# astaka-pe/SeMIGCN

Measured on NVIDIA B200. Metric: sgcn_gcnconv_train_edge_layers_per_s, higher is better.
Workload: dtype f32

## Files before the change

include/semigcn_b200.h:

```cpp
#ifndef SEMIGCN_B200_H
#define SEMIGCN_B200_H

#include <stddef.h>
#include <stdint.h>

#if defined(__GNUC__)
#define SGB_API __attribute__((visibility("default")))
#else
#define SGB_API
#endif

#ifdef __cplusplus
extern "C" {
#endif

#define SGB_VERSION 100

#define SGB_OK 0
#define SGB_EINVAL (-1)
#define SGB_ECUDA (-2)
#define SGB_ENOSPC (-3)
#define SGB_ENOTSUP (-4)

#define SGB_MODE_GCN 0
#define SGB_MODE_CHEB 1
#define SGB_MODE_ADJ 2

typedef struct sgb_edge {
    int32_t col;
    float w;
} sgb_edge_t;

SGB_API int sgb_version(void);
SGB_API const char* sgb_last_error(void);
SGB_API int sgb_num_sms(void);

SGB_API int sgb_fingerprint(const int64_t* values, int64_t count, uint64_t* out , void* stream);
SGB_API size_t sgb_graph_build_workspace_bytes(int64_t nnz, int64_t n);
SGB_API int sgb_graph_build(const int64_t* edge_index, int64_t nnz, int64_t n, int mode, int transpose,
                    int32_t* rowptr , int32_t* colidx , sgb_edge_t* edges ,
                    float* dis , int32_t* perm , int32_t* err_flag ,
                    void* workspace, size_t workspace_bytes, void* stream);

SGB_API int sgb_spmm_stat_rows(int64_t n, int c);
SGB_API int sgb_spmm(const int32_t* rowptr, const sgb_edge_t* edges, const float* dis, int mode,
             const float* x, int64_t ldx, int64_t n, int c,
             const float* in_mean, const float* in_scale, const float* in_shift, float slope,
             float alpha, const float* addend, int64_t ld_addend, float beta,
             const float* bias, float* y, int64_t ldy, float* stat_partials, float* amax_out, void* stream);

SGB_API int sgb_spmm_halo(const int32_t* rowptr, const sgb_edge_t* edges, const float* dis, int mode,
                  const float* x, int64_t ldx, int64_t n, int c, const float* x_ghost, int64_t ld_ghost, int64_t n_split,
                  const float* in_mean, const float* in_scale, const float* in_shift, float slope,
                  float alpha, const float* addend, int64_t ld_addend, float beta,
                  const float* bias, float* y, int64_t ldy, float* stat_partials, float* amax_out, void* stream);
SGB_API int sgb_spmm_range(const int32_t* rowptr, const sgb_edge_t* edges, const float* dis, int mode,
                   const float* x, int64_t ldx, int64_t row_begin, int64_t n, int c, const float* x_ghost, int64_t ld_ghost, int64_t n_split,
                   const float* in_mean, const float* in_scale, const float* in_shift, float slope,
                   float alpha, const float* addend, int64_t ld_addend, float beta,
                   const float* bias, float* y, int64_t ldy, float* stat_partials, float* amax_out, void* stream);
SGB_API int sgb_gather_rows(const float* x, int64_t ldx, const int32_t* idx, int64_t count, int c, float* out, int64_t ldo, void* stream);

SGB_API int sgb_gemm_stat_rows(int64_t m);
SGB_API size_t sgb_gemm_workspace_bytes(int64_t m, int n, int k, int engine);
SGB_API int sgb_gemm(int transb, const float* a, int64_t lda, const float* b, int64_t ldb,
             float* c, int64_t ldc, int64_t m, int n, int k,
             const float* a_mean, const float* a_scale, const float* a_shift, float slope,
             const float* bias, int accumulate, float* stat_partials, const float* a_amax,
             void* workspace, size_t workspace_bytes, int engine, void* stream);
SGB_API size_t sgb_gemm_tn_workspace_bytes(int64_t m, int n, int k);
SGB_API int sgb_gemm_tn(const float* g, int64_t ldg, const float* a, int64_t lda, float* d, int64_t ldd,
                int64_t m, int n, int k, int accumulate, const float* g_amax, const float* a_amax,
                void* workspace, size_t workspace_bytes, int engine, void* stream);
SGB_API size_t sgb_colsum_workspace_bytes(int64_t m, int n);
SGB_API int sgb_colsum(const float* g, int64_t ldg, int64_t m, int n, float* out, int accumulate,
               float* amax_out ,
               void* workspace, size_t workspace_bytes, void* stream);
SGB_API int sgb_amax(const float* x, int64_t ldx, int64_t m, int c, float* amax_out, void* stream);

SGB_API int sgb_col_stat_rows(int64_t m, int c);
SGB_API int sgb_col_stats(const float* y, int64_t ldy, int64_t m, int c, float* partials, void* stream);
SGB_API int sgb_bn_finalize(const float* partials, int rows, int c, int64_t count,
                    const float* gamma, const float* beta, float eps, float momentum,
                    float* running_mean, float* running_var,
                    float* mean, float* invstd, float* scale, float* shift, void* stream);
SGB_API int sgb_moments_merge(const float* partials, int rows, int c, float* merged , void* stream);
SGB_API int sgb_bn_act_apply(const float* y, int64_t ldy, int64_t m, int c, const float* mean, const float* scale,
                     const float* shift, float slope, float* z, int64_t ldz, float* amax_out , void* stream);
SGB_API int sgb_bn_act_bwd_reduce(const float* dz, int64_t lddz, const float* y, int64_t ldy, int64_t m, int c,
                          const float* scale, const float* shift, const float* mean, const float* invstd,
                          float slope, float* partials, void* stream);
SGB_API int sgb_bn_bwd_finalize(const float* partials, int rows, int c, float* sums, float* dgamma,
                        float* dbeta, int accumulate, void* stream);
SGB_API int sgb_bn_act_bwd_apply(const float* dz, int64_t lddz, const float* y, int64_t ldy, int64_t m, int c,
                         const float* scale, const float* shift, const float* mean, const float* invstd,
                         const float* sums, float slope, int training, float* dy, int64_t lddy,
                         float* amax_out , void* stream);

SGB_API int sgb_loss_partial_rows(void);
SGB_API size_t sgb_incidence_build_workspace_bytes(int64_t nf, int64_t n);
SGB_API int sgb_incidence_build(const int64_t* faces, int64_t nf, int64_t n, int32_t* rowptr , int32_t* inc ,
                        int32_t* err_flag, void* workspace, size_t workspace_bytes, void* stream);
SGB_API int sgb_step_loss_fwd(const float* pos, int64_t ldp, int64_t n, const void* target_pos, int target_f64, const uint8_t* vmask,
                      const int64_t* faces, int64_t nf, const void* target_fn, const uint8_t* fmask, float* fn_out,
                      double* partials, double* out , void* stream);
SGB_API int sgb_step_loss_bwd(const float* pos, int64_t ldp, int64_t n, const void* target_pos, int target_f64, const uint8_t* vmask,
                      const int64_t* faces, int64_t nf, const void* target_fn, const uint8_t* fmask,
                      const int32_t* inc_rowptr, const int32_t* inc, const double* out, const double* grads ,
                      float* dpos, int64_t lddpos, void* stream);
SGB_API int sgb_lap_loss_fwd(const float* pos, int64_t ldp, int64_t n, const int32_t* rowptr, const sgb_edge_t* edges, float* diff ,
                     double* partials, double* out , void* stream);
SGB_API int sgb_lap_loss_bwd(const float* diff, int64_t n, const int32_t* rowptr, const int32_t* rowptr_t, const sgb_edge_t* edges_t,
                     const double* out, const double* grad , float* dpos, int64_t lddpos, void* stream);

SGB_API size_t sgb_bnf_work_floats(int64_t nf);
SGB_API int sgb_bnf_partial_rows(void);
SGB_API int sgb_bnf_loss_fwd(const float* pos, int64_t ldp, int64_t n, const int64_t* faces, const int32_t* f2f, int64_t nf,
                     const float* fn, int loop, int ltype, float* work, double* partials, float* new_fn, double* out ,
                     void* stream);
SGB_API int sgb_bnf_loss_bwd(const float* fn, const float* new_fn, int64_t nf, int ltype, const double* out, const double* grad ,
                     float* dfn, void* stream);

SGB_API int sgb_input_prep(const float* z1, int64_t ldz, int64_t n, const float* dm, float* x, float* scratch , void* stream);

#ifdef __cplusplus
}
#endif
#endif
```

semigcn_b200/_lib.py:

```python
from __future__ import annotations

import ctypes as C
import os
import subprocess
from typing import Optional

import torch

_HERE = os.path.dirname(os.path.abspath(__file__))
CSRC = os.path.join(_HERE, "csrc")
LIB_PATH = os.environ.get("SGB_LIB_PATH") or os.path.join(CSRC, "libsemigcn_b200.so")

MODE_GCN, MODE_CHEB, MODE_ADJ = 0, 1, 2
ENGINE_AUTO, ENGINE_SIMT, ENGINE_TC = 0, 1, 2

_i64, _i32, _f32, _vp, _sz = C.c_int64, C.c_int, C.c_float, C.c_void_p, C.c_size_t
_f64 = C.c_double

SIGNATURES = {
    "sgb_version": (_i32, []),
    "sgb_last_error": (C.c_char_p, []),
    "sgb_num_sms": (_i32, []),
    "sgb_fingerprint": (_i32, [_vp, _i64, _vp, _vp]),
    "sgb_graph_build_workspace_bytes": (_sz, [_i64, _i64]),
    "sgb_graph_build": (_i32, [_vp, _i64, _i64, _i32, _i32, _vp, _vp, _vp, _vp, _vp, _vp, _vp, _sz, _vp]),
    "sgb_spmm_stat_rows": (_i32, [_i64, _i32]),
    "sgb_spmm": (_i32, [_vp, _vp, _vp, _i32, _vp, _i64, _i64, _i32, _vp, _vp, _vp, _f32, _f32, _vp, _i64, _f32,
                        _vp, _vp, _i64, _vp, _vp, _vp]),
    "sgb_spmm_halo": (_i32, [_vp, _vp, _vp, _i32, _vp, _i64, _i64, _i32, _vp, _i64, _i64, _vp, _vp, _vp, _f32, _f32, _vp, _i64, _f32,
                             _vp, _vp, _i64, _vp, _vp, _vp]),
    "sgb_spmm_range": (_i32, [_vp, _vp, _vp, _i32, _vp, _i64, _i64, _i64, _i32, _vp, _i64, _i64, _vp, _vp, _vp, _f32, _f32, _vp, _i64, _f32,
                              _vp, _vp, _i64, _vp, _vp, _vp]),
    "sgb_gather_rows": (_i32, [_vp, _i64, _vp, _i64, _i32, _vp, _i64, _vp]),
    "sgb_gemm_stat_rows": (_i32, [_i64]),
    "sgb_gemm_workspace_bytes": (_sz, [_i64, _i32, _i32, _i32]),
    "sgb_gemm": (_i32, [_i32, _vp, _i64, _vp, _i64, _vp, _i64, _i64, _i32, _i32, _vp, _vp, _vp, _f32, _vp, _i32,
                        _vp, _vp, _vp, _sz, _i32, _vp]),
    "sgb_gemm_tn_workspace_bytes": (_sz, [_i64, _i32, _i32]),
    "sgb_gemm_tn": (_i32, [_vp, _i64, _vp, _i64, _vp, _i64, _i64, _i32, _i32, _i32, _vp, _vp, _vp, _sz, _i32, _vp]),
    "sgb_colsum_workspace_bytes": (_sz, [_i64, _i32]),
    "sgb_colsum": (_i32, [_vp, _i64, _i64, _i32, _vp, _i32, _vp, _vp, _sz, _vp]),
    "sgb_amax": (_i32, [_vp, _i64, _i64, _i32, _vp, _vp]),
    "sgb_moments_merge": (_i32, [_vp, _i32, _i32, _vp, _vp]),
    "sgb_col_stat_rows": (_i32, [_i64, _i32]),
    "sgb_col_stats": (_i32, [_vp, _i64, _i64, _i32, _vp, _vp]),
    "sgb_bn_finalize": (_i32, [_vp, _i32, _i32, _i64, _vp, _vp, _f32, _f32, _vp, _vp, _vp, _vp, _vp, _vp, _vp]),
    "sgb_bn_act_apply": (_i32, [_vp, _i64, _i64, _i32, _vp, _vp, _vp, _f32, _vp, _i64, _vp, _vp]),
    "sgb_bn_act_bwd_reduce": (_i32, [_vp, _i64, _vp, _i64, _i64, _i32, _vp, _vp, _vp, _vp, _f32, _vp, _vp]),
    "sgb_bn_bwd_finalize": (_i32, [_vp, _i32, _i32, _vp, _vp, _vp, _i32, _vp]),
    "sgb_bn_act_bwd_apply": (_i32, [_vp, _i64, _vp, _i64, _i64, _i32, _vp, _vp, _vp, _vp, _vp, _f32, _i32,
                                    _vp, _i64, _vp, _vp]),
    "sgb_loss_partial_rows": (_i32, []),
    "sgb_incidence_build_workspace_bytes": (_sz, [_i64, _i64]),
    "sgb_incidence_build": (_i32, [_vp, _i64, _i64, _vp, _vp, _vp, _vp, _sz, _vp]),
    "sgb_step_loss_fwd": (_i32, [_vp, _i64, _i64, _vp, _i32, _vp, _vp, _i64, _vp, _vp, _vp, _vp, _vp, _vp]),
    "sgb_step_loss_bwd": (_i32, [_vp, _i64, _i64, _vp, _i32, _vp, _vp, _i64, _vp, _vp, _vp, _vp, _vp, _vp, _vp, _i64, _vp]),
    "sgb_lap_loss_fwd": (_i32, [_vp, _i64, _i64, _vp, _vp, _vp, _vp, _vp, _vp]),
    "sgb_input_prep": (_i32, [_vp, _i64, _i64, _vp, _vp, _vp, _vp]),
    "sgb_bnf_work_floats": (_sz, [_i64]),
    "sgb_bnf_partial_rows": (_i32, []),
    "sgb_bnf_loss_fwd": (_i32, [_vp, _i64, _i64, _vp, _vp, _i64, _vp, _i32, _i32, _vp, _vp, _vp, _vp, _vp]),
    "sgb_bnf_loss_bwd": (_i32, [_vp, _vp, _i64, _i32, _vp, _vp, _vp, _vp]),
    "sgb_lap_loss_bwd": (_i32, [_vp, _i64, _vp, _vp, _vp, _vp, _vp, _vp, _i64, _vp]),
}

_lib: Optional[C.CDLL] = None


class SgbError(RuntimeError):
    pass


def build_library(verbose: bool = False) -> str:
    out = subprocess.run(["make", "-C", CSRC, "-j", str(os.cpu_count() or 4)], capture_output=True, text=True)
    if verbose or out.returncode != 0:
        print(out.stdout[-4000:])
        print(out.stderr[-4000:])
    if out.returncode != 0:
        raise SgbError("building libsemigcn_b200.so failed")
    return LIB_PATH


def load() -> C.CDLL:
    global _lib
    if _lib is not None:
        return _lib
    if not os.path.exists(LIB_PATH):
        raise SgbError(
            f"{LIB_PATH} not found: the CUDA extension is required (no CPU fallback). "
            "Build it with `python -c 'import __graft_entry__ as g; g.build()'` or `make -C semigcn_b200/csrc`.")
    lib = C.CDLL(LIB_PATH)
    for name, (res, args) in SIGNATURES.items():
        fn = getattr(lib, name)
        fn.restype = res
        fn.argtypes = args
    _lib = lib
    return lib


# ... 27 lines not shown
```

semigcn_b200/csrc/bn.cu:

```cuda
#include "common.cuh"

namespace sgb {

constexpr int kColThreads = 256;

enum ColOp { COL_STATS = 0, COL_BN_BWD = 1, COL_SUM = 2 };

struct ColArgs {
    const float* y; int64_t ldy;
    const float* dz; int64_t lddz;
    int64_t m; int c;
    const float* scale; const float* shift; const float* mean; const float* invstd;
    float slope;
    float* partials;
    float* amax;
};

template <int OP, int VEC>
__global__ void __launch_bounds__(kColThreads) k_col_reduce(const ColArgs a, int tpr ) {
    __shared__ float red[2][kColThreads * VEC];
    __shared__ float redn[kColThreads];
    float amx = 0.f;
    const int cl = threadIdx.x % tpr;
    const int rl = threadIdx.x / tpr;
// ... 87 lines not shown
            }
        }
        __syncthreads();
    }
    if (OP == COL_SUM && a.amax) publish_amax(amx, reinterpret_cast<uint32_t*>(redn), a.amax);
}

static int col_tpr(int c, int vec) {
    int lanes = (c + vec - 1) / vec;
    int p = 1;
    while (p < lanes && p < kColThreads) p <<= 1;
    return p;
}

static int col_rows_cfg(int64_t m, int c, int vec) {
    int tpr = col_tpr(c, vec);
    int rpp = kColThreads / tpr;
    int64_t need = ceil_div(m > 0 ? m : 1, (int64_t)rpp * 4);
    int64_t cap = (int64_t)num_sms() * 4;
    int64_t g = need < cap ? need : cap;
    return (int)(g < 1 ? 1 : g);
}

static int col_rows(int64_t m, int c) {
    int g4 = col_rows_cfg(m, c, 4), g1 = col_rows_cfg(m, c, 1);
    return g4 > g1 ? g4 : g1;
}

template <int OP>
static int col_launch(const ColArgs& a, bool vec_ok, cudaStream_t stream) {
    int vec = (a.c % 4 == 0 && vec_ok) ? 4 : 1;
    int grid = col_rows_cfg(a.m, a.c, vec);
    int rows = col_rows(a.m, a.c);
    const int planes = OP == COL_STATS ? 3 : 2;
    if (rows > grid)
        if (cudaMemsetAsync(a.partials + (size_t)grid * planes * a.c, 0, (size_t)(rows - grid) * planes * a.c * sizeof(float), stream) != cudaSuccess) {
            set_error("col_reduce: memset failed");
            return SGB_ECUDA;
        }
    int tpr = col_tpr(a.c, vec);
    if (vec == 4) k_col_reduce<OP, 4><<<grid, kColThreads, 0, stream>>>(a, tpr);
    else k_col_reduce<OP, 1><<<grid, kColThreads, 0, stream>>>(a, tpr);
    SGB_CHECK_LAUNCH("k_col_reduce");
    return SGB_OK;
}

static bool al16(const void* p) { return (reinterpret_cast<uintptr_t>(p) & 15) == 0; }

struct FinArgs {
    const float* partials; int rows; int c; int64_t count;
    const float* gamma; const float* beta; float eps; float momentum;
    float* running_mean; float* running_var;
    float* mean; float* invstd; float* scale; float* shift;
    float* sums; float* dgamma; float* dbeta; int accumulate;
    int kind;
};

__global__ void __launch_bounds__(1024) k_finalize(const FinArgs f) {
    __shared__ double r1[32][33], r2[32][33], r3[32][33];
    const int ch = blockIdx.x * 32 + threadIdx.x;
    double s1 = 0.0, s2 = 0.0, s3 = 0.0;
    if (ch < f.c) {
        if (f.kind == 0 || f.kind == 3) {
            double p = 0.0;
            bool have = false;
            for (int r = threadIdx.y; r < f.rows; r += 32) {
                const double nb = (double)__ldg(f.partials + ((int64_t)r * 3 + 0) * f.c + ch);
                if (nb == 0.0) continue;
                const double mb = (double)__ldg(f.partials + ((int64_t)r * 3 + 1) * f.c + ch);
                const double qb = (double)__ldg(f.partials + ((int64_t)r * 3 + 2) * f.c + ch);
                if (!have) { p = mb; have = true; }
                const double d = mb - p;
                s1 += nb;
                s2 = fma(nb, d, s2);
                s3 += fma(nb * d, d, qb);
            }
            if (have) {
                const double dm = s2 / s1;
                s3 -= s2 * dm;
                if (s3 < 0.0) s3 = 0.0;
                s2 = p + dm;
            }
        } else {
            for (int r = threadIdx.y; r < f.rows; r += 32) {
                s1 += (double)__ldg(f.partials + ((int64_t)r * 2 + 0) * f.c + ch);
                s2 += (double)__ldg(f.partials + ((int64_t)r * 2 + 1) * f.c + ch);
            }
        }
    }
    r1[threadIdx.y][threadIdx.x] = s1;
    r2[threadIdx.y][threadIdx.x] = s2;
    r3[threadIdx.y][threadIdx.x] = s3;
    __syncthreads();
    if (threadIdx.y == 0 && ch < f.c) {
        if (f.kind == 0 || f.kind == 3) {
            double n = 0.0, mean = 0.0, m2 = 0.0;
            for (int r = 0; r < 32; ++r) {
                const double nb = r1[r][threadIdx.x];
                if (nb == 0.0) continue;
                const double nt = n + nb, d = r2[r][threadIdx.x] - mean;
                m2 += r3[r][threadIdx.x] + d * d * n * nb / nt;
                mean += d * nb / nt;
                n = nt;
            }
            if (f.kind == 3) {
                f.sums[ch] = (float)n;
                f.sums[f.c + ch] = (float)mean;
                f.sums[2 * f.c + ch] = (float)m2;
                return;
            }
            double var = n > 0.0 ? m2 / n : 0.0;
            if (var < 0.0) var = 0.0;
            const double invstd = 1.0 / sqrt(var + (double)f.eps);
            const double g = f.gamma ? (double)f.gamma[ch] : 1.0;
            const double b = f.beta ? (double)f.beta[ch] : 0.0;
            f.mean[ch] = (float)mean;
            f.invstd[ch] = (float)invstd;
            f.scale[ch] = (float)(g * invstd);
            f.shift[ch] = (float)b;
            if (f.running_mean) {
                const double unb = n > 1.0 ? m2 / (n - 1.0) : var;
                f.running_mean[ch] = (float)((1.0 - f.momentum) * (double)f.running_mean[ch] + f.momentum * mean);
                f.running_var[ch] = (float)((1.0 - f.momentum) * (double)f.running_var[ch] + f.momentum * unb);
            }
        } else {
            double t1 = 0.0, t2 = 0.0;
            for (int r = 0; r < 32; ++r) { t1 += r1[r][threadIdx.x]; t2 += r2[r][threadIdx.x]; }
            if (f.kind == 1) {
                f.sums[ch] = (float)t1;
                f.sums[f.c + ch] = (float)t2;
                if (f.dbeta) f.dbeta[ch] = f.accumulate ? f.dbeta[ch] + (float)t1 : (float)t1;
                if (f.dgamma) f.dgamma[ch] = f.accumulate ? f.dgamma[ch] + (float)t2 : (float)t2;
            } else {
                f.sums[ch] = f.accumulate ? f.sums[ch] + (float)t1 : (float)t1;
            }
        }
    }
}

constexpr int kEwThreads = 256;

static int ew_tpr(int c, int vec) {
    int lanes = (c + vec - 1) / vec;
    int p = 1;
    while (p < lanes && p < kEwThreads) p <<= 1;
    return p;
}

template <int VEC>
__global__ void __launch_bounds__(kEwThreads) k_bn_act_apply(const float* __restrict__ y, int64_t ldy, int64_t m, int c, const float* __restrict__ mean,
                                                             const float* __restrict__ scale, const float* __restrict__ shift, float slope,
                                                             float* __restrict__ z, int64_t ldz, float* __restrict__ amax, int tpr) {
    __shared__ uint32_t s_amax[32];
    float amx = 0.f;
    const int cl = threadIdx.x % tpr, rl = threadIdx.x / tpr, rpp = kEwThreads / tpr;
    for (int c0 = 0; c0 < c; c0 += tpr * VEC) {
        const int ch = c0 + cl * VEC;
        if (ch >= c) continue;
        float mu[VEC], sc[VEC], sh[VEC];
#pragma unroll
        for (int q = 0; q < VEC; ++q) { mu[q] = __ldg(mean + ch + q); sc[q] = __ldg(scale + ch + q); sh[q] = __ldg(shift + ch + q); }
        for (int64_t r = (int64_t)blockIdx.x * rpp + rl; r < m; r += (int64_t)gridDim.x * rpp) {
            if (VEC == 4) {
                const float4 v = ldg4(y + r * ldy + ch);
                float4 o;
                o.x = bn_lrelu(v.x, mu[0], sc[0], sh[0], slope); o.y = bn_lrelu(v.y, mu[1], sc[1], sh[1], slope);
                o.z = bn_lrelu(v.z, mu[2], sc[2], sh[2], slope); o.w = bn_lrelu(v.w, mu[3], sc[3], sh[3], slope);
                st4(z + r * ldz + ch, o);
                amx = fmaxf(amx, fmaxf(fmaxf(fabsf(o.x), fabsf(o.y)), fmaxf(fabsf(o.z), fabsf(o.w))));
            } else {
                const float o = bn_lrelu(__ldg(y + r * ldy + ch), mu[0], sc[0], sh[0], slope);
                z[r * ldz + ch] = o;
                amx = fmaxf(amx, fabsf(o));
            }
        }
    }
    if (amax) publish_amax(amx, s_amax, amax);
}

struct BwdArgs {
    const float* dz; int64_t lddz; const float* y; int64_t ldy; int64_t m; int c;
    const float* scale; const float* shift; const float* mean; const float* invstd; const float* sums;
    float slope; int training; float* dy; int64_t lddy; float* amax;
};

template <int VEC>
__global__ void __launch_bounds__(kEwThreads) k_bn_act_bwd_apply(const BwdArgs a, int tpr) {
    __shared__ uint32_t s_amax[32];
    float amx = 0.f;
// ... 19 lines not shown
                float4 t = ldg4(a.y + r * a.ldy + ch), u = ldg4(a.dz + r * a.lddz + ch);
                yv[0] = t.x; yv[1] = t.y; yv[2] = t.z; yv[3] = t.w;
                dv[0] = u.x; dv[1] = u.y; dv[2] = u.z; dv[3] = u.w;
            } else {
                yv[0] = __ldg(a.y + r * a.ldy + ch);
                dv[0] = __ldg(a.dz + r * a.lddz + ch);
            }
#pragma unroll
            for (int q = 0; q < VEC; ++q) {
                const float ctr = yv[q] - mu[q];
                const float pre = fmaf(ctr, sc[q], sh[q]);
                const float da = pre > 0.f ? dv[q] : dv[q] * a.slope;
                if (a.training) {
                    const float xh = ctr * is[q];
                    out[q] = sc[q] * (da - sb[q] - xh * sg[q]);
                } else {
                    out[q] = sc[q] * da;
                }
                amx = fmaxf(amx, fabsf(out[q]));
            }
            if (VEC == 4) st4(a.dy + r * a.lddy + ch, make_float4(out[0], out[1], out[2], out[3]));
            else a.dy[r * a.lddy + ch] = out[0];
        }
    }
    if (a.amax) publish_amax(amx, s_amax, a.amax);
}

static int ew_grid(int64_t m, int tpr) {
    const int rpp = kEwThreads / tpr;
    int64_t g = ceil_div(m > 0 ? m : 1, (int64_t)rpp * 4);
    int64_t cap = (int64_t)num_sms() * 8;
    g = g < cap ? g : cap;
    return (int)(g < 1 ? 1 : g);
}

}

using namespace sgb;

extern "C" int sgb_col_stat_rows(int64_t m, int c) {
    if (m < 0 || c <= 0) return 0;
    return col_rows(m, c);
}

extern "C" int sgb_col_stats(const float* y, int64_t ldy, int64_t m, int c, float* partials, void* stream) {
    SGB_CHECK_ARG(y && partials && m >= 0 && c > 0 && ldy >= c, "sgb_col_stats: bad argument");
    ColArgs a{};
    a.y = y; a.ldy = ldy; a.m = m; a.c = c; a.partials = partials;
    return col_launch<COL_STATS>(a, al16(y) && ldy % 4 == 0, (cudaStream_t)stream);
}

extern "C" int sgb_bn_finalize(const float* partials, int rows, int c, int64_t count, const float* gamma, const float* beta,
                               float eps, float momentum, float* running_mean, float* running_var, float* mean, float* invstd,
                               float* scale, float* shift, void* stream) {
    SGB_CHECK_ARG(partials && rows > 0 && c > 0 && count > 0 && mean && invstd && scale && shift, "sgb_bn_finalize: bad argument");
    SGB_CHECK_ARG((running_mean == nullptr) == (running_var == nullptr), "sgb_bn_finalize: running stats must come together");
    FinArgs f{};
    f.partials = partials; f.rows = rows; f.c = c; f.count = count; f.gamma = gamma; f.beta = beta; f.eps = eps;
    f.momentum = momentum; f.running_mean = running_mean; f.running_var = running_var;
    f.mean = mean; f.invstd = invstd; f.scale = scale; f.shift = shift; f.kind = 0;
    k_finalize<<<(c + 31) / 32, dim3(32, 32), 0, (cudaStream_t)stream>>>(f);
    SGB_CHECK_LAUNCH("k_finalize");
    return SGB_OK;
}

extern "C" int sgb_moments_merge(const float* partials, int rows, int c, float* merged, void* stream) {
    SGB_CHECK_ARG(partials && rows > 0 && c > 0 && merged, "sgb_moments_merge: bad argument");
    FinArgs f{};
    f.partials = partials; f.rows = rows; f.c = c; f.sums = merged; f.kind = 3;
    k_finalize<<<(c + 31) / 32, dim3(32, 32), 0, (cudaStream_t)stream>>>(f);
    SGB_CHECK_LAUNCH("k_finalize");
    return SGB_OK;
}

extern "C" int sgb_bn_act_apply(const float* y, int64_t ldy, int64_t m, int c, const float* mean, const float* scale,
                                const float* shift, float slope, float* z, int64_t ldz, float* amax_out, void* stream) {
    SGB_CHECK_ARG(y && z && mean && scale && shift && m >= 0 && c > 0 && ldy >= c && ldz >= c, "sgb_bn_act_apply: bad argument");
    if (m == 0) return SGB_OK;
    bool vec = c % 4 == 0 && al16(y) && al16(z) && al16(mean) && al16(scale) && al16(shift) && ldy % 4 == 0 && ldz % 4 == 0;
    const int tpr = ew_tpr(c, vec ? 4 : 1);
    if (vec) k_bn_act_apply<4><<<ew_grid(m, tpr), kEwThreads, 0, (cudaStream_t)stream>>>(y, ldy, m, c, mean, scale, shift, slope, z, ldz, amax_out, tpr);
    else k_bn_act_apply<1><<<ew_grid(m, tpr), kEwThreads, 0, (cudaStream_t)stream>>>(y, ldy, m, c, mean, scale, shift, slope, z, ldz, amax_out, tpr);
    SGB_CHECK_LAUNCH("k_bn_act_apply");
    return SGB_OK;
}

extern "C" int sgb_bn_act_bwd_reduce(const float* dz, int64_t lddz, const float* y, int64_t ldy, int64_t m, int c, const float* scale,
                                     const float* shift, const float* mean, const float* invstd, float slope, float* partials,
                                     void* stream) {
    SGB_CHECK_ARG(dz && y && scale && shift && mean && invstd && partials && m >= 0 && c > 0 && ldy >= c && lddz >= c,
                  "sgb_bn_act_bwd_reduce: bad argument");
    ColArgs a{};
    a.y = y; a.ldy = ldy; a.dz = dz; a.lddz = lddz; a.m = m; a.c = c;
    a.scale = scale; a.shift = shift; a.mean = mean; a.invstd = invstd; a.slope = slope; a.partials = partials;
    return col_launch<COL_BN_BWD>(a, al16(y) && al16(dz) && ldy % 4 == 0 && lddz % 4 == 0, (cudaStream_t)stream);
}

extern "C" int sgb_bn_bwd_finalize(const float* partials, int rows, int c, float* sums, float* dgamma, float* dbeta, int accumulate,
                                   void* stream) {
    SGB_CHECK_ARG(partials && rows > 0 && c > 0 && sums, "sgb_bn_bwd_finalize: bad argument");
    FinArgs f{};
    f.partials = partials; f.rows = rows; f.c = c; f.sums = sums; f.dgamma = dgamma; f.dbeta = dbeta; f.accumulate = accumulate;
    f.kind = 1;
    k_finalize<<<(c + 31) / 32, dim3(32, 32), 0, (cudaStream_t)stream>>>(f);
    SGB_CHECK_LAUNCH("k_finalize");
    return SGB_OK;
}

extern "C" int sgb_bn_act_bwd_apply(const float* dz, int64_t lddz, const float* y, int64_t ldy, int64_t m, int c, const float* scale,
                                    const float* shift, const float* mean, const float* invstd, const float* sums, float slope,
                                    int training, float* dy, int64_t lddy, float* amax_out, void* stream) {
    SGB_CHECK_ARG(dz && y && dy && scale && shift && m >= 0 && c > 0 && ldy >= c && lddz >= c && lddy >= c,
                  "sgb_bn_act_bwd_apply: bad argument");
// ... 36 lines not shown
```

semigcn_b200/csrc/common.cuh:

```cuda
#pragma once
#include <cuda_runtime.h>
#include <stdint.h>
#include <stdio.h>
#include <stdarg.h>
#include <atomic>
#include "../../include/semigcn_b200.h"

namespace sgb {

void set_error(const char* fmt, ...);
int num_sms();
int smem_optin(const void* func, int bytes, std::atomic<uint64_t>* done_mask);

#define SGB_CHECK_ARG(cond, ...)                 \
    do {                                         \
        if (!(cond)) {                           \
            sgb::set_error(__VA_ARGS__);         \
            return SGB_EINVAL;                   \
        }                                        \
    } while (0)

#define SGB_CHECK_LAUNCH(name)                                                        \
    do {                                                                              \
        cudaError_t e__ = cudaGetLastError();                                         \
        if (e__ != cudaSuccess) {                                                     \
            sgb::set_error("%s: launch failed: %s", name, cudaGetErrorString(e__));   \
            return SGB_ECUDA;                                                         \
        }                                                                             \
    } while (0)

#define SGB_CUDA(call)                                                                \
    do {                                                                              \
        cudaError_t e__ = (call);                                                     \
        if (e__ != cudaSuccess) {                                                     \
            sgb::set_error("%s failed: %s", #call, cudaGetErrorString(e__));          \
            return SGB_ECUDA;                                                         \
        }                                                                             \
    } while (0)

static inline int64_t ceil_div(int64_t a, int64_t b) { return (a + b - 1) / b; }
__host__ __device__ static inline int64_t min64(int64_t a, int64_t b) { return a < b ? a : b; }
static inline size_t align_up(size_t x, size_t a) { return (x + a - 1) / a * a; }

__device__ __forceinline__ float lrelu(float v, float slope) { return v > 0.f ? v : v * slope; }

__device__ __forceinline__ float bn_lrelu(float x, float mean, float scale, float beta, float slope) {
    return lrelu(fmaf(x - mean, scale, beta), slope);
}

struct Moments {
    float n, mean, m2;
};
__device__ __forceinline__ Moments merge(Moments a, Moments b) {
    if (b.n == 0.f) return a;
    if (a.n == 0.f) return b;
    Moments r;
    r.n = a.n + b.n;
    const float d = b.mean - a.mean;
    const float w = b.n / r.n;
    r.mean = fmaf(d, w, a.mean);
    r.m2 = a.m2 + b.m2 + d * d * a.n * w;
    return r;
}
__device__ __forceinline__ Moments from_shifted(float n, float p, float s1, float s2) {
    Moments r;
    r.n = n;
    if (n == 0.f) { r.mean = 0.f; r.m2 = 0.f; return r; }
    const float dm = s1 / n;
    r.mean = p + dm;
    r.m2 = fmaxf(s2 - s1 * dm, 0.f);
    return r;
}

__device__ __forceinline__ float4 ldg4(const float* p) { return __ldg(reinterpret_cast<const float4*>(p)); }
__device__ __forceinline__ void st4(float* p, float4 v) { *reinterpret_cast<float4*>(p) = v; }

__device__ __forceinline__ void publish_amax(float mx, uint32_t* scratch, float* slot) {
    uint32_t b = __reduce_max_sync(0xffffffffu, __float_as_uint(mx));
    const int warp = threadIdx.x >> 5, nw = (blockDim.x + 31) >> 5;
    if ((threadIdx.x & 31) == 0) scratch[warp] = b;
    __syncthreads();
    if (threadIdx.x == 0) {
        for (int w = 1; w < nw; ++w) b = max(b, scratch[w]);
        if (b) atomicMax(reinterpret_cast<uint32_t*>(slot), b);
    }
}

int gemm_stat_rows(int64_t m);

struct GemmArgs {
    int transb;
    const float* a; int64_t lda;
    const float* b; int64_t ldb;
    float* c; int64_t ldc;
    int64_t m; int n; int k;
    const float* a_mean; const float* a_scale; const float* a_shift; float slope;
    const float* bias; int accumulate; float* stat_partials;
};

}
```

semigcn_b200/csrc/gemm.cu:

```cuda
#include "common.cuh"

namespace sgb {
int gemm_simt_launch(const GemmArgs& g, cudaStream_t stream);
int gemm_tn_simt_launch(const float* g, int64_t ldg, const float* a, int64_t lda, float* d, int64_t ldd, int64_t m, int n, int k,
                        int accumulate, void* ws, size_t ws_bytes, cudaStream_t stream);
size_t gemm_tn_simt_workspace(int64_t m, int n, int k);
bool gemm_tc_supported(int64_t m, int n, int k, int64_t lda, int64_t ldc, const void* a, const void* c, const void* bias,
                       const void* a_scale);
size_t gemm_tc_workspace(int n, int k);
int gemm_tc_launch(const GemmArgs& g, void* ws, size_t ws_bytes, cudaStream_t stream);
bool gemm_tn_tc_supported(int64_t m, int n, int k, int64_t ldg, int64_t lda, const void* g, const void* a);
size_t gemm_tn_tc_workspace(int64_t m, int n, int k);
int gemm_tn_tc_launch(const float* g, int64_t ldg, const float* a, int64_t lda, float* d, int64_t ldd, int64_t m, int n, int k,
                      int accumulate, void* ws, size_t ws_bytes, cudaStream_t stream);
size_t gemm_f16_workspace(int n, int k);
int gemm_f16_launch(const GemmArgs& g, const float* a_amax, void* ws, size_t ws_bytes, cudaStream_t stream);
size_t gemm_tn_f16_workspace(int64_t m, int n, int k);
int gemm_tn_f16_launch(const float* g, int64_t ldg, const float* a, int64_t lda, const float* g_amax, const float* a_amax, float* d,
                       int64_t ldd, int64_t m, int n, int k, int accumulate, void* ws, size_t ws_bytes, cudaStream_t stream);
bool gemm_tn_pair_ok(int64_t m, int n, int k);
size_t gemm_tn_pair_workspace(int64_t m, int n, int k);
int gemm_tn_pair_launch(const float* g, int64_t ldg, const float* a, int64_t lda, const float* g_amax, const float* a_amax, float* d,
                        int64_t ldd, int64_t m, int n, int k, int accumulate, void* ws, size_t ws_bytes, cudaStream_t stream);
static bool tn_tc_worthwhile(int64_t m, int n, int k) { return n >= 32 && k >= 16 && m >= 4096; }

static bool tc_worthwhile(int64_t m, int n, int k) { return n >= 32 && k >= 16 && m >= 2048; }
}

using namespace sgb;

namespace sgb {
int gemm_stat_rows(int64_t m) {
    if (m <= 0) return 0;
    const int64_t tiles = ceil_div(m, 128);
    return 4 * (int)(tiles < num_sms() ? tiles : num_sms());
}
}

extern "C" int sgb_gemm_stat_rows(int64_t m) { return gemm_stat_rows(m); }

extern "C" size_t sgb_gemm_workspace_bytes(int64_t m, int n, int k, int engine) {
    if (m < 0 || n <= 0 || k <= 0 || engine == 1) return 0;
    if (engine == 0 && !tc_worthwhile(m, n, k)) return 0;
    if (n % 16 != 0 || k % 4 != 0) return 0;
    size_t w2 = gemm_tc_workspace(n, k), w3 = gemm_f16_workspace(n, k);
    return engine == 2 ? w2 : engine == 3 ? w3 : (w2 > w3 ? w2 : w3);
}

extern "C" int sgb_gemm(int transb, const float* a, int64_t lda, const float* b, int64_t ldb, float* c, int64_t ldc, int64_t m,
                        int n, int k, const float* a_mean, const float* a_scale, const float* a_shift, float slope, const float* bias,
                        int accumulate, float* stat_partials, const float* a_amax, void* workspace, size_t workspace_bytes, int engine,
                        void* stream) {
    SGB_CHECK_ARG(a && b && c && m >= 0 && n > 0 && k > 0, "sgb_gemm: bad argument m=%lld n=%d k=%d", (long long)m, n, k);
    SGB_CHECK_ARG(lda >= k && ldc >= n && ldb >= (transb ? k : n), "sgb_gemm: leading dimension too small");
    SGB_CHECK_ARG((a_scale == nullptr) == (a_shift == nullptr) && (a_scale == nullptr) == (a_mean == nullptr),
                  "sgb_gemm: a_mean / a_scale / a_shift must come together");
    SGB_CHECK_ARG(engine >= 0 && engine <= 3, "sgb_gemm: bad engine %d", engine);
    if (m == 0) return SGB_OK;
    GemmArgs g{transb, a, lda, b, ldb, c, ldc, m, n, k, a_mean, a_scale, a_shift, slope, bias, accumulate, stat_partials};
    const bool tc_ok = gemm_tc_supported(m, n, k, lda, ldc, a, c, bias, a_scale);
    if (engine == 2) {
        if (!tc_ok) {
            set_error("sgb_gemm: tcgen05 engine needs n %% 16 == 0, k %% 4 == 0 and 16-byte aligned operands (n=%d k=%d)", n, k);
            return SGB_ENOTSUP;
        }
        return gemm_tc_launch(g, workspace, workspace_bytes, (cudaStream_t)stream);
    }
    if (engine == 3) {
        if (!tc_ok || a_scale) {
            set_error("sgb_gemm: fp16-split engine needs n %% 16 == 0, k %% 4 == 0, 16-byte aligned operands and no A prologue (n=%d k=%d)", n, k);
            return SGB_ENOTSUP;
        }
        return gemm_f16_launch(g, a_amax, workspace, workspace_bytes, (cudaStream_t)stream);
    }
    if (engine == 0 && tc_ok && tc_worthwhile(m, n, k) && workspace) {
        if (!a_scale && workspace_bytes >= gemm_f16_workspace(n, k))
            return gemm_f16_launch(g, a_amax, workspace, workspace_bytes, (cudaStream_t)stream);
        if (workspace_bytes >= gemm_tc_workspace(n, k)) return gemm_tc_launch(g, workspace, workspace_bytes, (cudaStream_t)stream);
    }
    return gemm_simt_launch(g, (cudaStream_t)stream);
}

extern "C" size_t sgb_gemm_tn_workspace_bytes(int64_t m, int n, int k) {
    if (m < 0 || n <= 0 || k <= 0) return 0;
    size_t a = gemm_tn_simt_workspace(m, n, k), b = (n % 4 == 0 && k % 4 == 0) ? gemm_tn_tc_workspace(m, n, k) : 0;
    size_t c = (n % 4 == 0 && k % 4 == 0) ? gemm_tn_f16_workspace(m, n, k) : 0;
    size_t e = gemm_tn_pair_workspace(m, n, k);
    a = a > b ? a : b;
    a = a > c ? a : c;
    return a > e ? a : e;
}

extern "C" int sgb_gemm_tn(const float* g, int64_t ldg, const float* a, int64_t lda, float* d, int64_t ldd, int64_t m, int n, int k,
                           int accumulate, const float* g_amax, const float* a_amax, void* workspace, size_t workspace_bytes, int engine,
                           void* stream) {
    SGB_CHECK_ARG(g && a && d && m >= 0 && n > 0 && k > 0, "sgb_gemm_tn: bad argument");
    SGB_CHECK_ARG(ldg >= n && lda >= k && ldd >= k, "sgb_gemm_tn: leading dimension too small");
    SGB_CHECK_ARG(engine >= 0 && engine <= 4, "sgb_gemm_tn: bad engine %d", engine);
    const bool tc_ok = gemm_tn_tc_supported(m, n, k, ldg, lda, g, a);
    if (engine == 0 && tc_ok && gemm_tn_pair_ok(m, n, k) && m >= 32768) engine = 4;
    if (engine == 4) {
        if (!tc_ok || !gemm_tn_pair_ok(m, n, k)) {
            set_error("sgb_gemm_tn: the pair engine needs n %% 256 == 0, k %% 32 == 0 (k <= 256 or k %% 256 == 0), m >= 4096 and 16-byte aligned operands");
            return SGB_ENOTSUP;
        }
        return gemm_tn_pair_launch(g, ldg, a, lda, g_amax, a_amax, d, ldd, m, n, k, accumulate, workspace, workspace_bytes, (cudaStream_t)stream);
    }
    if (engine == 2) {
        if (!tc_ok) {
            set_error("sgb_gemm_tn: tcgen05 engine needs n %% 4 == 0, k %% 4 == 0 and 16-byte aligned operands");
            return SGB_ENOTSUP;
        }
        return gemm_tn_tc_launch(g, ldg, a, lda, d, ldd, m, n, k, accumulate, workspace, workspace_bytes, (cudaStream_t)stream);
    }
    if (engine == 3 || (engine == 0 && tc_ok && tn_tc_worthwhile(m, n, k))) {
        if (!tc_ok) {
            set_error("sgb_gemm_tn: fp16-split engine needs n %% 4 == 0, k %% 4 == 0 and 16-byte aligned operands");
            return SGB_ENOTSUP;
        }
        return gemm_tn_f16_launch(g, ldg, a, lda, g_amax, a_amax, d, ldd, m, n, k, accumulate, workspace, workspace_bytes, (cudaStream_t)stream);
    }
    if (engine == 0 && tc_ok && tn_tc_worthwhile(m, n, k))
        return gemm_tn_tc_launch(g, ldg, a, lda, d, ldd, m, n, k, accumulate, workspace, workspace_bytes, (cudaStream_t)stream);
    return gemm_tn_simt_launch(g, ldg, a, lda, d, ldd, m, n, k, accumulate, workspace, workspace_bytes, (cudaStream_t)stream);
}
```

semigcn_b200/csrc/gemm_f16.cu:

```cuda
#include "common.cuh"
#include "umma.cuh"
#include <cuda_fp16.h>
#include <stdlib.h>

#ifndef SGB_ABL
#define SGB_ABL 0
#endif
#define SGB_ABL_NO_BCOPY 1
#define SGB_ABL_NO_STORE 2
#define SGB_ABL_NO_EPI 4
#define SGB_ABL_NO_CONV 8
#define SGB_ABL_NO_TMA 16
#define SGB_ABL_NO_MMA 32
#define SGB_ABL_T_NO_MMA 64
#define SGB_ABL_T_NO_CONV 128
#define SGB_ABL_T_NO_DRAIN 256

namespace sgb {

__host__ __device__ __forceinline__ void f16_scale_from_amax(float amax, float& s, float& inv) {
    uint32_t bits;
#ifdef __CUDA_ARCH__
    bits = __float_as_uint(amax);
#else
    union { float f; uint32_t u; } cv; cv.f = amax; bits = cv.u;
#endif
    const int e = (int)((bits >> 23) & 0xff);
    int se = 127 + 14 - (e - 127);
    if (e == 0 || e == 255) se = 127;
    if (se < 2) se = 2;
    if (se > 252) se = 252;
#ifdef __CUDA_ARCH__
    s = __uint_as_float((uint32_t)se << 23);
    inv = __uint_as_float((uint32_t)(254 - se) << 23);
#else
    cv.u = (uint32_t)se << 23; s = cv.f;
    cv.u = (uint32_t)(254 - se) << 23; inv = cv.f;
#endif
}

__global__ void __launch_bounds__(256) k_amax(const float* __restrict__ x, int64_t ldx, int64_t m, int c, uint32_t* __restrict__ slot) {
    const int cv = c >> 2;
    const int64_t total = m * cv;
    float mx = 0.f;
    for (int64_t i = blockIdx.x * (int64_t)blockDim.x + threadIdx.x; i < total; i += (int64_t)gridDim.x * blockDim.x) {
        const int64_t r = i / cv;
        const int ch = (int)(i % cv) * 4;
        const float4 v = ldg4(x + r * ldx + ch);
        mx = fmaxf(mx, fmaxf(fmaxf(fabsf(v.x), fabsf(v.y)), fmaxf(fabsf(v.z), fabsf(v.w))));
    }
    uint32_t b = __float_as_uint(mx);
    b = __reduce_max_sync(0xffffffffu, b);
    __shared__ uint32_t sm[8];
    if ((threadIdx.x & 31) == 0) sm[threadIdx.x >> 5] = b;
    __syncthreads();
    if (threadIdx.x == 0) {
        for (int w = 1; w < 8; ++w) b = max(b, sm[w]);
        if (b) atomicMax(slot, b);
    }
}

int amax_launch(const float* x, int64_t ldx, int64_t m, int c, uint32_t* slot, cudaStream_t stream) {
    SGB_CUDA(cudaMemsetAsync(slot, 0, sizeof(uint32_t), stream));
    const int64_t total = m * (c / 4);
    const int grid = (int)min64(ceil_div(total > 0 ? total : 1, 256 * 8), (int64_t)num_sms() * 8);
    k_amax<<<grid, 256, 0, stream>>>(x, ldx, m, c, slot);
    SGB_CHECK_LAUNCH("k_amax");
    return SGB_OK;
}

__device__ __forceinline__ void split_f16x2(float x0, float x1, uint32_t& hi, uint32_t& lo) {
    const __half2 h = __floats2half2_rn(x0, x1);
    const float2 f = __half22float2(h);
    const __half2 l = __floats2half2_rn(x0 - f.x, x1 - f.y);
    hi = *reinterpret_cast<const uint32_t*>(&h);
    lo = *reinterpret_cast<const uint32_t*>(&l);
}

constexpr int kHBM = 128;
constexpr int kHBK = 32;
constexpr int kHCols = kHBK / 8;
constexpr int kHALbo = 128;
constexpr int kHASbo = kHCols * kHALbo;
constexpr int kHATile = (kHBM / 8) * kHASbo;
constexpr int kHBLbo = 128;
constexpr int kHBSbo = kHCols * kHBLbo;
constexpr int kHConvWarps = 4;
constexpr int kHEpiWarps = 8;
constexpr int kHWarpB = kHConvWarps + kHEpiWarps;
constexpr int kHWarpMma = kHWarpB + 1;
constexpr int kHWarpLoad = kHWarpB + 2;
constexpr int kHThreads = (kHWarpLoad + 1) * 32;
constexpr int kHRawBytes = kHBM * kHBK * 4;
constexpr int kHMaxRawStages = 6;
constexpr int kHBarBytes = 512;
constexpr int kHMaxStages = 6;
constexpr int kHEpiLd = 36;
constexpr int kHEpiBytes = kHEpiWarps * 32 * 32 * 4;
constexpr int kTEpiBytes = 4 * 32 * kHEpiLd * 4;
static const int kHSmemBudget = 227 * 1024;

__host__ __device__ constexpr int h_b_tile_bytes(int bn) { return (bn / 8) * kHBSbo; }
__host__ __device__ constexpr int h_stage_bytes(int bn) { return (2 * kHATile + 2 * h_b_tile_bytes(bn) + 1023) / 1024 * 1024; }
__host__ __device__ constexpr int h_stage_bytes_pair(int bn) { return (2 * kHATile + h_b_tile_bytes(bn) + 1023) / 1024 * 1024; }

struct HArgs {
    CUtensorMap a_map;
    const float* a; int64_t lda;
    const uint8_t* wp;
    const float* wscale;
    const float* a_amax;
    float* c; int64_t ldc;
    int64_t m; int n; int k;
    int bn; int n_tiles; int k_chunks; int stages; int raw_stages;
    const float* bias; int accumulate;
    float* stat_partials;
    uint32_t tmem_cols; int acc_stride;
};

__global__ void __launch_bounds__(256) k_prep_weights_f16(const float* __restrict__ w, int64_t ldw, int transb, int n, int k, int bn,
                                                          int n_tiles, int k_chunks, __half* __restrict__ wp, float* __restrict__ wscale) {
    __shared__ float sm[8];
    const int rows = transb ? n : k, cols = transb ? k : n;
    float mx = 0.f;
    if (ldw == cols && (reinterpret_cast<uintptr_t>(w) & 15) == 0 && ((rows * cols) & 3) == 0) {
        for (int i = threadIdx.x; i < (rows * cols) >> 2; i += blockDim.x) {
            const float4 v = ldg4(w + 4 * i);
            mx = fmaxf(mx, fmaxf(fmaxf(fabsf(v.x), fabsf(v.y)), fmaxf(fabsf(v.z), fabsf(v.w))));
        }
    } else {
        for (int r = 0; r < rows; ++r)
            for (int i = threadIdx.x; i < cols; i += blockDim.x) mx = fmaxf(mx, fabsf(w[(int64_t)r * ldw + i]));
    }
    mx = __uint_as_float(__reduce_max_sync(0xffffffffu, __float_as_uint(mx)));
    if ((threadIdx.x & 31) == 0) sm[threadIdx.x >> 5] = mx;
    __syncthreads();
    mx = sm[0];
    for (int i = 1; i < 8; ++i) mx = fmaxf(mx, sm[i]);
    float s, inv;
    f16_scale_from_amax(mx, s, inv);
    if (blockIdx.x == 0 && threadIdx.x == 0) { wscale[0] = s; wscale[1] = inv; }
    const int tile_halves = h_b_tile_bytes(bn) / 2;
    const int64_t total = (int64_t)n_tiles * k_chunks * tile_halves;
    for (int64_t i = blockIdx.x * (int64_t)blockDim.x + threadIdx.x; i < total; i += (int64_t)gridDim.x * blockDim.x) {
        const int h = (int)(i % tile_halves);
        const int64_t blk = i / tile_halves;
        const int q = (int)(blk % k_chunks), t = (int)(blk / k_chunks);
        const int core_n = h / (kHBSbo / 2);
        const int rem = h % (kHBSbo / 2);
        const int core_k = rem / 64, in_core = rem % 64;
        const int nl = core_n * 8 + in_core / 8, kl = core_k * 8 + in_core % 8;
        const int gn = t * bn + nl, gk = q * kHBK + kl;
        float v = 0.f;
        if (gn < n && gk < k) v = transb ? w[(int64_t)gn * ldw + gk] : w[(int64_t)gk * ldw + gn];
        v *= s;
        const __half hi = __float2half_rn(v);
        const __half lo = __float2half_rn(v - __half2float(hi));
        __half* base = wp + (blk * 2) * tile_halves;
        base[h] = hi;
        base[tile_halves + h] = lo;
    }
}

template <bool FULL>
__device__ __forceinline__ void h_epi_chunk(const HArgs& g, uint32_t taddr, float* __restrict__ stg, float* __restrict__ cp ,
                                            const float* __restrict__ bias_p, int lane, int grp, int cc, int nvalid, bool col_ok, float sc1, float sc2,
                                            bool stats, float inv_nb, float (&blk_mean)[4], float (&blk_m2)[4]) {
    float4 b = make_float4(0.f, 0.f, 0.f, 0.f);
    if (bias_p && (FULL || col_ok)) b = ldg4(bias_p);
    float v[32];
    tmem_ld_32x32(taddr, v);
    if (sc2 == 1.f) {
#pragma unroll
        for (int e = 0; e < 32; e += 4)
            *reinterpret_cast<float4*>(stg + lane * 32 + (((e >> 2) ^ (lane & 7)) << 2)) = make_float4(v[e] * sc1, v[e + 1] * sc1, v[e + 2] * sc1, v[e + 3] * sc1);
    } else {
#pragma unroll
        for (int e = 0; e < 32; e += 4)
            *reinterpret_cast<float4*>(stg + lane * 32 + (((e >> 2) ^ (lane & 7)) << 2)) =
                make_float4((v[e] * sc1) * sc2, (v[e + 1] * sc1) * sc2, (v[e + 2] * sc1) * sc2, (v[e + 3] * sc1) * sc2);
    }
    __syncwarp();
    const int64_t ld4 = 4 * g.ldc;
    float4 o[8];
#pragma unroll
    for (int i = 0; i < 8; ++i) {
        const bool on = FULL || (col_ok && i * 4 + grp < nvalid);
        o[i] = on ? *reinterpret_cast<const float4*>(stg + (i * 4 + grp) * 32 + ((((lane & 7) ^ ((i * 4 + grp) & 7))) << 2)) : make_float4(0.f, 0.f, 0.f, 0.f);
    }
    if (g.accumulate) {
        float4 old[8];
#pragma unroll
        for (int i = 0; i < 8; ++i) {
            const bool on = FULL || (col_ok && i * 4 + grp < nvalid);
            old[i] = on ? *reinterpret_cast<const float4*>(cp + i * ld4) : make_float4(0.f, 0.f, 0.f, 0.f);
        }
#pragma unroll
        for (int i = 0; i < 8; ++i) { o[i].x += old[i].x; o[i].y += old[i].y; o[i].z += old[i].z; o[i].w += old[i].w; }
    }
#pragma unroll
    for (int i = 0; i < 8; ++i) {
        const bool on = FULL || (col_ok && i * 4 + grp < nvalid);
        if (on) {
            o[i].x += b.x; o[i].y += b.y; o[i].z += b.z; o[i].w += b.w;
            if (!(SGB_ABL & SGB_ABL_NO_STORE)) *reinterpret_cast<float4*>(cp + i * ld4) = o[i];
        }
    }
    if (stats) {
        float sm[4] = {0.f, 0.f, 0.f, 0.f};
#pragma unroll
        for (int i = 0; i < 8; ++i) { sm[0] += o[i].x; sm[1] += o[i].y; sm[2] += o[i].z; sm[3] += o[i].w; }
#pragma unroll
        for (int q = 0; q < 4; ++q) {
            sm[q] += __shfl_xor_sync(0xffffffffu, sm[q], 8);
            sm[q] += __shfl_xor_sync(0xffffffffu, sm[q], 16);
            sm[q] *= inv_nb;
        }
        float d2[4] = {0.f, 0.f, 0.f, 0.f};
#pragma unroll
        for (int i = 0; i < 8; ++i) {
            if (FULL || i * 4 + grp < nvalid) {
                const float dx = o[i].x - sm[0], dy = o[i].y - sm[1], dz = o[i].z - sm[2], dw = o[i].w - sm[3];
                d2[0] = fmaf(dx, dx, d2[0]); d2[1] = fmaf(dy, dy, d2[1]); d2[2] = fmaf(dz, dz, d2[2]); d2[3] = fmaf(dw, dw, d2[3]);
            }
        }
#pragma unroll
        for (int q = 0; q < 4; ++q) {
            d2[q] += __shfl_xor_sync(0xffffffffu, d2[q], 8);
            d2[q] += __shfl_xor_sync(0xffffffffu, d2[q], 16);
            blk_mean[q] = sm[q];
            blk_m2[q] = d2[q];
        }
    }
    __syncwarp();
}

template <bool PAIR>
__global__ void __launch_bounds__(kHThreads, 1) k_gemm_f16(const __grid_constant__ HArgs g) {
    extern __shared__ __align__(1024) uint8_t smem[];
    const int warp = threadIdx.x >> 5, lane = threadIdx.x & 31;
    const uint32_t rank = PAIR ? cluster_ctarank() : 0u;
    const int stage_bytes = PAIR ? h_stage_bytes_pair(g.bn) : h_stage_bytes(g.bn);
    const int b_tile_bytes = h_b_tile_bytes(g.bn);
    const int b_smem_bytes = PAIR ? b_tile_bytes / 2 : b_tile_bytes;
    const uint32_t stages = (uint32_t)g.stages;
    uint8_t* const raw_base = smem;
    const uint32_t raw_stages = (uint32_t)g.raw_stages;
    uint8_t* const op_base = smem + raw_stages * kHRawBytes;
    uint64_t* full = reinterpret_cast<uint64_t*>(op_base + (size_t)g.stages * stage_bytes);
    uint64_t* empty = full + kHMaxStages;
    uint64_t* tfull = empty + kHMaxStages;
    uint64_t* tempty = tfull + 2;
    uint64_t* rfull = tempty + 2;
    uint64_t* rempty = rfull + kHMaxRawStages;
    uint64_t* bfull = rempty + kHMaxRawStages;
    uint32_t* tmem_slot = reinterpret_cast<uint32_t*>(bfull + kHMaxStages);

    if (threadIdx.x == 0) {
        for (int s = 0; s < g.stages; ++s) {
            mbar_init(&full[s], PAIR ? 2 * (kHConvWarps / 2) : kHConvWarps * 32 / 2 + 1);
            mbar_init(&empty[s], 1);
            mbar_init(&bfull[s], 1);
        }
        for (int b = 0; b < 2; ++b) {
            mbar_init(&tfull[b], 1);
            mbar_init(&tempty[b], PAIR ? 2 * kHEpiWarps : kHEpiWarps);
        }
        for (uint32_t s = 0; s < raw_stages; ++s) {
            mbar_init(&rfull[s], 1);
            mbar_init(&rempty[s], kHConvWarps * 32 / 2);
        }
        fence_barrier_init();
    }
    if (PAIR) {
        __syncthreads();
        cluster_sync_all();
        if (warp == kHWarpMma) tmem_alloc_pair(tmem_slot, g.tmem_cols);
    } else {
        if (warp == kHWarpMma) tmem_alloc(tmem_slot, g.tmem_cols);
    }
    tc_fence_before();
    __syncthreads();
    tc_fence_after();
    const uint32_t tmem_base = *tmem_slot;

    const uint32_t unit = PAIR ? blockIdx.x >> 1 : blockIdx.x, units = PAIR ? gridDim.x >> 1 : gridDim.x;
    const int64_t m_tiles = (g.m + kHBM - 1) / kHBM;
    const int64_t total_tiles = (PAIR ? (m_tiles + 1) / 2 : m_tiles) * g.n_tiles;
    const uint32_t my_tiles = total_tiles > unit ? (uint32_t)((total_tiles - 1 - unit) / units + 1) : 0u;
    const uint32_t k_chunks = (uint32_t)g.k_chunks;
    const int nt = (int)(unit % (uint32_t)g.n_tiles);
#define SGB_H_M0_OF(tile) ((PAIR ? ((tile) / g.n_tiles) * 2 + (int64_t)rank : (tile) / g.n_tiles) * kHBM)

    if (warp < kHConvWarps) {
        float sa, inva;
        f16_scale_from_amax(__ldg(g.a_amax), sa, inva);
        constexpr int GROUPS = 2, GTHREADS = kHConvWarps * 32 / GROUPS;
        const int grp = warp / (kHConvWarps / GROUPS);
        const int gt = threadIdx.x - grp * GTHREADS;
        const int cq = (gt >> 3) & (kHCols - 1), r0 = (gt & 7) + 8 * (gt >> 5);
        static_assert(kHCols == 4, "converter thread mapping assumes 4 core columns per stage");
        constexpr int RPT = kHBM * kHCols / GTHREADS;
        constexpr int RSTEP = GTHREADS / kHCols;
        constexpr int HALF = RPT / 2;
        const uint32_t total_it = my_tiles * k_chunks;
        uint32_t s = (uint32_t)grp % stages, ph = ((uint32_t)grp / stages) & 1u;
        uint32_t rs = (uint32_t)grp % raw_stages, rph = ((uint32_t)grp / raw_stages) & 1u;
        for (uint32_t it = (uint32_t)grp; it < total_it; it += GROUPS) {
            mbar_wait(&rempty[rs], rph ^ 1);
            mbar_wait(&rfull[rs], rph);
            const uint8_t* raw = raw_base + (size_t)rs * kHRawBytes;
            uint4 h[RPT], l[RPT];
#pragma unroll
            for (int hf = 0; hf < ((SGB_ABL & SGB_ABL_NO_CONV) ? 0 : 2); ++hf) {
                float4 v[HALF][2];
#pragma unroll
                for (int i = 0; i < HALF; ++i) {
                    const int r = r0 + RSTEP * (hf * HALF + i);
                    v[i][0] = *reinterpret_cast<const float4*>(raw + r * 128 + (((2 * cq) ^ (r & 7)) << 4));
                    v[i][1] = *reinterpret_cast<const float4*>(raw + r * 128 + (((2 * cq + 1) ^ (r & 7)) << 4));
                }
#pragma unroll
                for (int i = 0; i < HALF; ++i) {
                    const int k = hf * HALF + i;
                    split_f16x2(v[i][0].x * sa, v[i][0].y * sa, h[k].x, l[k].x);
                    split_f16x2(v[i][0].z * sa, v[i][0].w * sa, h[k].y, l[k].y);
                    split_f16x2(v[i][1].x * sa, v[i][1].y * sa, h[k].z, l[k].z);
                    split_f16x2(v[i][1].z * sa, v[i][1].w * sa, h[k].w, l[k].w);
                }
            }
            fence_proxy_async();
            mbar_arrive(&rempty[rs]);
            mbar_wait(&empty[s], ph ^ 1);
            uint8_t* a_hi = op_base + (size_t)s * stage_bytes;
            uint8_t* a_lo = a_hi + kHATile;
#pragma unroll
            for (int i = 0; i < ((SGB_ABL & SGB_ABL_NO_CONV) ? 0 : RPT); ++i) {
                const int r = r0 + RSTEP * i;
                const uint32_t off = (uint32_t)(r >> 3) * kHASbo + (uint32_t)cq * kHALbo + (uint32_t)(r & 7) * 16;
                *reinterpret_cast<uint4*>(a_hi + off) = h[i];
                *reinterpret_cast<uint4*>(a_lo + off) = l[i];
            }
            fence_proxy_async();
            if (PAIR) {
                __syncwarp();
                if (lane == 0) {
                    mbar_wait(&bfull[s], ph);
                    mbar_arrive_cluster(&full[s], 0);
                }
            } else {
                mbar_arrive(&full[s]);
            }
            s += GROUPS;
            if (s >= stages) { s -= stages; ph ^= 1; }
            rs += GROUPS;
            if (rs >= raw_stages) { rs -= raw_stages; rph ^= 1; }
        }
    } else if (warp == kHWarpLoad) {
        if (lane == 0) {
            tma_prefetch_desc(&g.a_map);
            uint32_t rs = 0, rph = 0;
            int64_t tile = unit;
            for (uint32_t t = 0; t < my_tiles; ++t, tile += units) {
                const int m0 = (int)SGB_H_M0_OF(tile);
                for (uint32_t q = 0; q < k_chunks; ++q) {
                    mbar_wait(&rempty[rs], rph ^ 1);
                    if (SGB_ABL & SGB_ABL_NO_TMA) { mbar_arrive(&rfull[rs]); }
                    else {
                        mbar_arrive_expect_tx(&rfull[rs], kHRawBytes);
                        tma_load_2d(raw_base + (size_t)rs * kHRawBytes, &g.a_map, (int)(q * kHBK), m0, &rfull[rs]);
                    }
                    if (++rs == raw_stages) { rs = 0; rph ^= 1; }
                }
// ... 32 lines not shown
                const uint32_t acc = tcount & 1;
                if (PAIR) mbar_wait_cluster(&tempty[acc], ((tcount >> 1) & 1) ^ 1);
                else mbar_wait(&tempty[acc], ((tcount >> 1) & 1) ^ 1);
                tc_fence_after();
                const uint32_t d_tmem = tmem_base + acc * (uint32_t)g.acc_stride;
                for (uint32_t q = 0; q < k_chunks; ++q) {
                    if (PAIR) mbar_wait_cluster(&full[s], ph);
                    else mbar_wait(&full[s], ph);
                    tc_fence_after();
                    const uint32_t a_hi = smem_u32(op_base + (size_t)s * stage_bytes);
                    const uint32_t a_lo = a_hi + kHATile;
                    const uint32_t b_hi = a_hi + 2 * kHATile;
                    const uint32_t b_lo = b_hi + b_smem_bytes;
#pragma unroll
                    for (int j = 0; j < ((SGB_ABL & SGB_ABL_NO_MMA) ? 0 : kHBK / 16); ++j) {
                        const uint64_t dah = make_desc(a_hi + j * 2 * kHALbo, kHALbo, kHASbo);
                        const uint64_t dal = make_desc(a_lo + j * 2 * kHALbo, kHALbo, kHASbo);
                        const uint64_t dbh = make_desc(b_hi + j * 2 * kHBLbo, kHBLbo, kHBSbo);
                        const uint64_t dbl = make_desc(b_lo + j * 2 * kHBLbo, kHBLbo, kHBSbo);
                        if (PAIR) {
                            umma_f16_pair(d_tmem, dal, dbh, idesc, (q | (uint32_t)j) ? 1u : 0u);
                            umma_f16_pair(d_tmem, dah, dbl, idesc, 1u);
                            umma_f16_pair(d_tmem, dah, dbh, idesc, 1u);
                        } else {
                            umma_f16(d_tmem, dal, dbh, idesc, (q | (uint32_t)j) ? 1u : 0u);
                            umma_f16(d_tmem, dah, dbl, idesc, 1u);
                            umma_f16(d_tmem, dah, dbh, idesc, 1u);
                        }
                    }
                    if (PAIR) umma_commit_pair(&empty[s]);
                    else umma_commit(&empty[s]);
                    if (++s == stages) { s = 0; ph ^= 1; }
                }
                if (PAIR) umma_commit_pair(&tfull[acc]);
                else umma_commit(&tfull[acc]);
            }
        }
    } else {
        float sa, inva;
        f16_scale_from_amax(__ldg(g.a_amax), sa, inva);
        const float invw = __ldg(g.wscale + 1);
        float sc1 = inva * invw, sc2 = 1.f;
        if (!(fabsf(sc1) >= 1.1754944e-38f && fabsf(sc1) <= 3.4028235e38f)) { sc1 = inva; sc2 = invw; }
        const int ew = warp - kHConvWarps;
        const int quarter = warp & 3;
        const int half = ew >> 2;
        float* stg = reinterpret_cast<float*>(op_base + (size_t)g.stages * stage_bytes + kHBarBytes) + ew * 32 * 32;
        const int grp = lane >> 3;
        const int cc = (lane & 7) * 4;
        const bool stats = g.stat_partials != nullptr;
        const int n0 = nt * g.bn;
        const int ncols = min(g.bn, g.n - n0);
        float st_mean[4] = {0.f, 0.f, 0.f, 0.f}, st_m2[4] = {0.f, 0.f, 0.f, 0.f}, st_n = 0.f;
        int64_t tile = unit;
        for (uint32_t tcount = 0; tcount < my_tiles; ++tcount, tile += units) {
            const int64_t m0 = SGB_H_M0_OF(tile);
            const uint32_t acc = tcount & 1;
            mbar_wait(&tfull[acc], (tcount >> 1) & 1);
            tc_fence_after();
            const uint32_t taddr = tmem_base + ((uint32_t)(quarter * 32) << 16) + acc * (uint32_t)g.acc_stride;
            const int64_t rows_left = g.m - (m0 + quarter * 32);
            const int nvalid = rows_left >= 32 ? 32 : (rows_left > 0 ? (int)rows_left : 0);
            const float nb = (float)nvalid;
            const float inv_nb = nvalid ? 1.f / nb : 0.f;
            const float wgt = nvalid ? nb / (st_n + nb) : 0.f;
            float* crow = g.c + (m0 + quarter * 32 + grp) * g.ldc + n0 + cc;
#pragma unroll
            for (int t = 0; t < 4; ++t) {
                const int c0 = (2 * t + half) * 32;
                if (c0 < ncols && !(SGB_ABL & SGB_ABL_NO_EPI)) {
                    float bm[4], bq[4];
                    const bool col_ok = c0 + cc < ncols;
                    const float* bias_p = g.bias ? g.bias + n0 + c0 + cc : nullptr;
                    if (nvalid == 32 && c0 + 32 <= ncols)
                        h_epi_chunk<true>(g, taddr + c0, stg, crow + c0, bias_p, lane, grp, cc, nvalid, col_ok, sc1, sc2, stats, inv_nb, bm, bq);
                    else
                        h_epi_chunk<false>(g, taddr + c0, stg, crow + c0, bias_p, lane, grp, cc, nvalid, col_ok, sc1, sc2, stats && nvalid > 0, inv_nb, bm, bq);
                    if (stats && nvalid > 0 && grp == t) {
#pragma unroll
                        for (int q = 0; q < 4; ++q) {
                            const float delta = bm[q] - st_mean[q];
                            st_mean[q] = fmaf(delta, wgt, st_mean[q]);
                            st_m2[q] += bq[q] + delta * delta * st_n * wgt;
                        }
                    }
                }
            }
            st_n += nb;
            tc_fence_before();
            __syncwarp();
            if (lane == 0) {
                if (PAIR) mbar_arrive_cluster(&tempty[acc], 0);
                else mbar_arrive(&tempty[acc]);
            }
        }
        if (stats) {
            const int64_t group = PAIR ? (int64_t)(unit / (uint32_t)g.n_tiles) * 2 + rank : (int64_t)(blockIdx.x / g.n_tiles);
            float* row = g.stat_partials + (group * 4 + quarter) * 3 * g.n;
            const int c0 = (2 * grp + half) * 32;
            if (c0 + cc < ncols) {
                st4(row + 0 * (int64_t)g.n + n0 + c0 + cc, make_float4(st_n, st_n, st_n, st_n));
                st4(row + 1 * (int64_t)g.n + n0 + c0 + cc, make_float4(st_mean[0], st_mean[1], st_mean[2], st_mean[3]));
                st4(row + 2 * (int64_t)g.n + n0 + c0 + cc, make_float4(st_m2[0], st_m2[1], st_m2[2], st_m2[3]));
            }
        }
    }
    tc_fence_before();
    __syncthreads();
    if (PAIR) cluster_sync_all();
    if (warp == kHWarpMma) {
        tc_fence_after();
        if (PAIR) tmem_dealloc_pair(tmem_base, g.tmem_cols);
        else tmem_dealloc(tmem_base, g.tmem_cols);
    }
#undef SGB_H_M0_OF
}

int reduce_splits_launch(const float* partial, int splits, int n, int k, float* d, int64_t ldd, int accumulate, cudaStream_t stream);

constexpr int kTBM = 128;
constexpr int kTBV = 32;
constexpr int kTCols = kTBV / 8;
constexpr int kTLbo = 128;
constexpr int kTSbo = kTCols * kTLbo + 16;
constexpr int kTGTile = (kTBM / 8) * kTSbo;
constexpr int kTProducerWarps = 12;
constexpr int kTDrainWarps = 4;
constexpr int kTThreads = (kTProducerWarps + 1 + kTDrainWarps + 1) * 32;
constexpr int kTRawStages = 2;
constexpr int kTMaxRawStages = 8;
constexpr int kTBarBytes = 512;
constexpr int kTSegChunks = 16;

__host__ __device__ constexpr int t_a_tile_bytes(int bk) { return (bk / 8) * kTSbo; }
__host__ __device__ constexpr int t_stage_bytes(int bk) { return 2 * kTGTile + 2 * t_a_tile_bytes(bk); }

struct TArgs {
    CUtensorMap g_map, a_map;
    int gbox, abox;
    const float* g; int64_t ldg;
    const float* a; int64_t lda;
    const float* g_amax; const float* a_amax;
    float* partial;
    int64_t m; int n; int k;
    int bk;
    int k_tiles; int stages; int raw_stages;
    int conv_groups;
    int64_t m_per_split;
    uint32_t tmem_cols; int acc_stride;
};

__global__ void __launch_bounds__(kTThreads, 1) k_gemm_tn_f16(const __grid_constant__ TArgs t) {
    extern __shared__ __align__(1024) uint8_t smem[];
    const int warp = threadIdx.x >> 5, lane = threadIdx.x & 31;
    const int stage_bytes = t_stage_bytes(t.bk);
    const int a_tile_bytes = t_a_tile_bytes(t.bk);
    const int raw_g_bytes = kTBV * t.gbox * 4, raw_a_bytes = kTBV * t.abox * 4;
    const int raw_bytes = (raw_g_bytes + raw_a_bytes + 127) / 128 * 128;
    uint8_t* const raw_base = smem;
    const uint32_t raw_stages = (uint32_t)t.raw_stages;
    uint8_t* const op_base = smem + (size_t)raw_stages * raw_bytes;
    uint64_t* full = reinterpret_cast<uint64_t*>(op_base + (size_t)t.stages * stage_bytes);
    uint64_t* empty = full + kHMaxStages;
    uint64_t* tfull = empty + kHMaxStages;
    uint64_t* tempty = tfull + 2;
    uint64_t* rfull = tempty + 2;
    uint64_t* rempty = rfull + kTMaxRawStages;
    uint32_t* tmem_slot = reinterpret_cast<uint32_t*>(rempty + kTMaxRawStages);

    if (threadIdx.x == 0) {
        for (int s = 0; s < t.stages; ++s) {
            mbar_init(&full[s], kTProducerWarps * 32 / t.conv_groups);
            mbar_init(&empty[s], 1);
        }
        for (int b = 0; b < 2; ++b) {
            mbar_init(&tfull[b], 1);
            mbar_init(&tempty[b], kTDrainWarps);
        }
        for (uint32_t s = 0; s < raw_stages; ++s) {
            mbar_init(&rfull[s], 1);
            mbar_init(&rempty[s], kTProducerWarps * 32 / t.conv_groups);
        }
        fence_barrier_init();
    }
    if (warp == kTProducerWarps) tmem_alloc(tmem_slot, t.tmem_cols);
    tc_fence_before();
    __syncthreads();
    tc_fence_after();
    const uint32_t tmem_base = *tmem_slot;

    const int n0 = (blockIdx.x / t.k_tiles) * kTBM;
    const int k0 = (blockIdx.x % t.k_tiles) * t.bk;
    const int64_t ms = (int64_t)blockIdx.y * t.m_per_split;
    const int64_t me = min64(t.m, ms + t.m_per_split);
    const int chunks = me > ms ? (int)((me - ms + kTBV - 1) / kTBV) : 0;
    const int segments = (chunks + kTSegChunks - 1) / kTSegChunks;
    float sg, invg, sa, inva;
    f16_scale_from_amax(__ldg(t.g_amax), sg, invg);
    f16_scale_from_amax(__ldg(t.a_amax), sa, inva);

    if (warp < kTProducerWarps) {
        const int tid = threadIdx.x;
        const int groups = t.conv_groups, gthreads = kTProducerWarps * 32 / groups;
        const int grp = tid / gthreads, lt = tid - grp * gthreads;
        bool is_g, active = true;
        int mg, c4;
        if (groups == 1) {
            is_g = tid < 128;
            const int idx = is_g ? tid : tid - 128;
            const int per_mg = is_g ? 32 : 64;
            mg = idx / per_mg; c4 = idx % per_mg;
        } else {
            const int qg = t.gbox >> 2, qa = t.abox >> 2;
            is_g = lt < 4 * qg;
            const int la = is_g ? lt : lt - 4 * qg;
            const int q = is_g ? qg : qa;
            active = la < 4 * q;
            mg = active ? la / q : 0; c4 = active ? la % q : 0;
        }
        const int box = is_g ? t.gbox : t.abox;
        const bool col_ok = active && c4 * 4 < box;
        const bool in_tile = active && c4 * 4 < (is_g ? kTBM : t.bk);
        const float sc = is_g ? sg : sa;
        const uint32_t raw_off = (is_g ? 0u : (uint32_t)raw_g_bytes) + (uint32_t)(mg * 8) * (uint32_t)box * 4u + (uint32_t)c4 * 16u;
        const uint32_t tile_off = is_g ? 0u : (uint32_t)(2 * kTGTile);
        const uint32_t lo_off = is_g ? (uint32_t)kTGTile : (uint32_t)a_tile_bytes;
        const uint32_t base_off = tile_off + (uint32_t)((c4 * 4) >> 3) * kTSbo + (uint32_t)mg * kTLbo + (uint32_t)((c4 * 4) & 7) * 16;
        const uint32_t ug = (uint32_t)groups, ustages = (uint32_t)t.stages;
        uint32_t s = (uint32_t)grp % ustages, ph = ((uint32_t)grp / ustages) & 1u, rs = (uint32_t)grp % raw_stages, rph = ((uint32_t)grp / raw_stages) & 1u;
        for (int it = grp; it < chunks; it += groups) {
            if (groups == 2) mbar_wait(&rempty[rs], rph ^ 1);
            mbar_wait(&rfull[rs], rph);
            const uint8_t* raw = raw_base + (size_t)rs * raw_bytes + raw_off;
            uint4 h[4], l[4];
            if (SGB_ABL & SGB_ABL_T_NO_CONV) {
#pragma unroll
                for (int q = 0; q < 4; ++q) { h[q] = make_uint4(0u, 0u, 0u, 0u); l[q] = make_uint4(0u, 0u, 0u, 0u); }
            } else if (col_ok) {
                float4 v[8];
#pragma unroll
                for (int r = 0; r < 8; ++r) v[r] = *reinterpret_cast<const float4*>(raw + (size_t)r * box * 4);
#pragma unroll
                for (int q = 0; q < 4; ++q) {
                    const float x0 = (&v[0].x)[q], x1 = (&v[1].x)[q], x2 = (&v[2].x)[q], x3 = (&v[3].x)[q];
                    const float x4 = (&v[4].x)[q], x5 = (&v[5].x)[q], x6 = (&v[6].x)[q], x7 = (&v[7].x)[q];
                    split_f16x2(x0 * sc, x1 * sc, h[q].x, l[q].x);
                    split_f16x2(x2 * sc, x3 * sc, h[q].y, l[q].y);
                    split_f16x2(x4 * sc, x5 * sc, h[q].z, l[q].z);
                    split_f16x2(x6 * sc, x7 * sc, h[q].w, l[q].w);
                }
            } else {
#pragma unroll
                for (int q = 0; q < 4; ++q) { h[q] = make_uint4(0u, 0u, 0u, 0u); l[q] = make_uint4(0u, 0u, 0u, 0u); }
            }
            fence_proxy_async();
            mbar_arrive(&rempty[rs]);
            mbar_wait(&empty[s], ph ^ 1);
            if (in_tile && !(SGB_ABL & SGB_ABL_T_NO_CONV)) {
                uint8_t* st = op_base + (size_t)s * stage_bytes + base_off;
#pragma unroll
                for (int q = 0; q < 4; ++q) {
                    *reinterpret_cast<uint4*>(st + q * 16) = h[q];
                    *reinterpret_cast<uint4*>(st + lo_off + q * 16) = l[q];
                }
            }
            fence_proxy_async();
            mbar_arrive(&full[s]);
            s += ug;
            if (s >= ustages) { s -= ustages; ph ^= 1; }
            rs += ug;
            if (rs >= raw_stages) { rs -= raw_stages; rph ^= 1; }
        }
    } else if (warp == kTProducerWarps + 1 + kTDrainWarps) {
        if (lane == 0) {
            tma_prefetch_desc(&t.g_map);
            tma_prefetch_desc(&t.a_map);
            const uint64_t stream_policy = l2_policy_evict_first();
            uint32_t rs = 0, rph = 0;
            for (int it = 0; it < chunks; ++it) {
                mbar_wait(&rempty[rs], rph ^ 1);
                mbar_arrive_expect_tx(&rfull[rs], (uint32_t)(raw_g_bytes + raw_a_bytes));
                uint8_t* dst = raw_base + (size_t)rs * raw_bytes;
                const int row = (int)(ms + (int64_t)it * kTBV);
                tma_load_2d_hint(dst, &t.g_map, n0, row, &rfull[rs], stream_policy);
                tma_load_2d_hint(dst + raw_g_bytes, &t.a_map, k0, row, &rfull[rs], stream_policy);
                if (++rs == raw_stages) { rs = 0; rph ^= 1; }
            }
        }
    } else if (warp == kTProducerWarps) {
        if (lane == 0) {
            const uint32_t idesc = make_idesc_f16(kTBM, t.bk, 0, 0);
            uint32_t s = 0, ph = 0;
            for (int it = 0; it < chunks; ++it) {
                const int seg = it / kTSegChunks, in_seg = it % kTSegChunks;
// ... 57 lines not shown
                        float4 old[8];
                        if (seg != 0) {
#pragma unroll
                            for (int i = 0; i < 8; ++i)
                                old[i] = (4 * i < nrows) ? ldcg_hint(reinterpret_cast<const float4*>(op0 + (int64_t)(4 * i) * t.k), keep_policy) : make_float4(0.f, 0.f, 0.f, 0.f);
                        }
#pragma unroll
                        for (int i = 0; i < 8; ++i) {
                            if (4 * i < nrows) {
                                float4 o = *reinterpret_cast<const float4*>(stg + (i * 4 + (lane >> 3)) * kHEpiLd + cc);
                                if (seg != 0) { o.x += old[i].x; o.y += old[i].y; o.z += old[i].z; o.w += old[i].w; }
                                stcg_hint(reinterpret_cast<float4*>(op0 + (int64_t)(4 * i) * t.k), o, keep_policy);
                            }
                        }
                    }
                    __syncwarp();
                } else if (gn < t.n) {
                    float* op = out + (int64_t)gn * t.k + k0 + c0;
#pragma unroll
                    for (int e = 0; e < 32; ++e)
                        if (c0 + e < kcols) op[e] = seg == 0 ? v[e] : op[e] + v[e];
                }
            }
            tc_fence_before();
            __syncwarp();
            if (lane == 0) mbar_arrive(&tempty[acc]);
        }
    }
    tc_fence_before();
    __syncthreads();
    if (warp == kTProducerWarps) {
        tc_fence_after();
        tmem_dealloc(tmem_base, t.tmem_cols);
    }
}

constexpr int kPConvWarps = 8;
constexpr int kPWarpMma = kPConvWarps;
constexpr int kPWarpDrain0 = kPConvWarps + 1;
constexpr int kPWarpLoad = kPWarpDrain0 + kTDrainWarps;
constexpr int kPThreads = (kPWarpLoad + 1) * 32;
constexpr int kPMaxRawStages = 4;

struct TPArgs {
    CUtensorMap g_map, a_map;
    int ah;
    const float* g_amax; const float* a_amax;
    float* partial;
    int64_t m; int n; int k;
    int bk;
    int k_tiles; int stages; int raw_stages;
    int64_t m_per_split;
    uint32_t tmem_cols; int acc_stride;
};

__global__ void __cluster_dims__(2, 1, 1) __launch_bounds__(kPThreads, 1) k_gemm_tn_f16_pair(const __grid_constant__ TPArgs t) {
    extern __shared__ __align__(1024) uint8_t smem[];
    const int warp = threadIdx.x >> 5, lane = threadIdx.x & 31;
    const uint32_t rank = cluster_ctarank();
    const int a_tile_bytes = t_a_tile_bytes(t.ah);
    const int stage_bytes = 2 * kTGTile + 2 * a_tile_bytes;
    constexpr int raw_g_bytes = kTBV * kTBM * 4;
    const int raw_a_bytes = kTBV * t.ah * 4;
    const int raw_bytes = (raw_g_bytes + raw_a_bytes + 127) / 128 * 128;
    uint8_t* const raw_base = smem;
    uint8_t* const op_base = smem + (size_t)t.raw_stages * raw_bytes;
    uint64_t* full = reinterpret_cast<uint64_t*>(op_base + (size_t)t.stages * stage_bytes);
    uint64_t* empty = full + kHMaxStages;
    uint64_t* tfull = empty + kHMaxStages;
    uint64_t* tempty = tfull + 2;
    uint64_t* rfull = tempty + 2;
    uint64_t* rempty = rfull + kPMaxRawStages;
    uint32_t* tmem_slot = reinterpret_cast<uint32_t*>(rempty + kPMaxRawStages);

    if (threadIdx.x == 0) {
        for (int s = 0; s < t.stages; ++s) {
            mbar_init(&full[s], 2 * kPConvWarps);
            mbar_init(&empty[s], 1);
        }
        for (int b = 0; b < 2; ++b) {
            mbar_init(&tfull[b], 1);
            mbar_init(&tempty[b], 2 * kTDrainWarps);
        }
        for (int s = 0; s < t.raw_stages; ++s) {
            mbar_init(&rfull[s], 1);
            mbar_init(&rempty[s], kPConvWarps * 32);
        }
        fence_barrier_init();
    }
    __syncthreads();
    cluster_sync_all();
    if (warp == kPWarpMma) tmem_alloc_pair(tmem_slot, t.tmem_cols);
    tc_fence_before();
    __syncthreads();
    tc_fence_after();
    const uint32_t tmem_base = *tmem_slot;

    const int pair = blockIdx.x >> 1;
    const int n0 = (pair / t.k_tiles) * 2 * kTBM + (int)rank * kTBM;
    const int k0 = (pair % t.k_tiles) * t.bk;
    const int ka = k0 + (int)rank * t.ah;
    const int64_t ms = (int64_t)blockIdx.y * t.m_per_split;
    const int64_t me = min64(t.m, ms + t.m_per_split);
    const int chunks = me > ms ? (int)((me - ms + kTBV - 1) / kTBV) : 0;
    const int segments = (chunks + kTSegChunks - 1) / kTSegChunks;
    float sg, invg, sa, inva;
    f16_scale_from_amax(__ldg(t.g_amax), sg, invg);
    f16_scale_from_amax(__ldg(t.a_amax), sa, inva);

    if (warp < kPConvWarps) {
        const int tid = threadIdx.x;
        const bool is_g = tid < 128;
        const int idx = tid & 127;
        const int mg = idx >> 5, c4 = idx & 31;
        const int box = is_g ? kTBM : t.ah;
        const bool in_tile = c4 * 4 < box;
        const float sc = is_g ? sg : sa;
        const uint32_t raw_off = (is_g ? 0u : (uint32_t)raw_g_bytes) + (uint32_t)(mg * 8) * (uint32_t)box * 4u + (uint32_t)c4 * 16u;
        const uint32_t tile_off = is_g ? 0u : (uint32_t)(2 * kTGTile);
        const uint32_t lo_off = is_g ? (uint32_t)kTGTile : (uint32_t)a_tile_bytes;
        const uint32_t base_off = tile_off + (uint32_t)((c4 * 4) >> 3) * kTSbo + (uint32_t)mg * kTLbo + (uint32_t)((c4 * 4) & 7) * 16;
        uint32_t s = 0, ph = 0, rs = 0, rph = 0;
        for (int it = 0; it < chunks; ++it) {
            mbar_wait(&rfull[rs], rph);
            const uint8_t* raw = raw_base + (size_t)rs * raw_bytes + raw_off;
            uint4 h[4], l[4];
            if (SGB_ABL & SGB_ABL_T_NO_CONV) {
#pragma unroll
                for (int q = 0; q < 4; ++q) { h[q] = make_uint4(0u, 0u, 0u, 0u); l[q] = make_uint4(0u, 0u, 0u, 0u); }
            } else if (in_tile) {
                float4 v[8];
#pragma unroll
                for (int r = 0; r < 8; ++r) v[r] = *reinterpret_cast<const float4*>(raw + (size_t)r * box * 4);
#pragma unroll
                for (int q = 0; q < 4; ++q) {
                    const float x0 = (&v[0].x)[q], x1 = (&v[1].x)[q], x2 = (&v[2].x)[q], x3 = (&v[3].x)[q];
                    const float x4 = (&v[4].x)[q], x5 = (&v[5].x)[q], x6 = (&v[6].x)[q], x7 = (&v[7].x)[q];
                    split_f16x2(x0 * sc, x1 * sc, h[q].x, l[q].x);
                    split_f16x2(x2 * sc, x3 * sc, h[q].y, l[q].y);
                    split_f16x2(x4 * sc, x5 * sc, h[q].z, l[q].z);
                    split_f16x2(x6 * sc, x7 * sc, h[q].w, l[q].w);
                }
            }
            fence_proxy_async();
            mbar_arrive(&rempty[rs]);
            mbar_wait(&empty[s], ph ^ 1);
            if (in_tile && !(SGB_ABL & SGB_ABL_T_NO_CONV)) {
                uint8_t* st = op_base + (size_t)s * stage_bytes + base_off;
#pragma unroll
                for (int q = 0; q < 4; ++q) {
                    *reinterpret_cast<uint4*>(st + q * 16) = h[q];
                    *reinterpret_cast<uint4*>(st + lo_off + q * 16) = l[q];
                }
            }
            fence_proxy_async();
            __syncwarp();
            if (lane == 0) mbar_arrive_cluster(&full[s], 0);
            if (++s == (uint32_t)t.stages) { s = 0; ph ^= 1; }
            if (++rs == (uint32_t)t.raw_stages) { rs = 0; rph ^= 1; }
        }
    } else if (warp == kPWarpLoad) {
        if (lane == 0) {
            tma_prefetch_desc(&t.g_map);
            tma_prefetch_desc(&t.a_map);
            const uint64_t stream_policy = l2_policy_evict_first();
            uint32_t rs = 0, rph = 0;
            for (int it = 0; it < chunks; ++it) {
                mbar_wait(&rempty[rs], rph ^ 1);
                mbar_arrive_expect_tx(&rfull[rs], (uint32_t)(raw_g_bytes + raw_a_bytes));
                uint8_t* dst = raw_base + (size_t)rs * raw_bytes;
                const int row = (int)(ms + (int64_t)it * kTBV);
                tma_load_2d_hint(dst, &t.g_map, n0, row, &rfull[rs], stream_policy);
                tma_load_2d_hint(dst + raw_g_bytes, &t.a_map, ka, row, &rfull[rs], stream_policy);
                if (++rs == (uint32_t)t.raw_stages) { rs = 0; rph ^= 1; }
            }
        }
    } else if (warp == kPWarpMma) {
        if (lane == 0 && rank == 0) {
            const uint32_t idesc = make_idesc_f16(2 * kTBM, t.bk, 0, 0);
            uint32_t s = 0, ph = 0;
            for (int it = 0; it < chunks; ++it) {
                const int seg = it / kTSegChunks, in_seg = it % kTSegChunks;
                const int acc = seg & 1;
                if (in_seg == 0) {
                    mbar_wait_cluster(&tempty[acc], ((seg >> 1) & 1) ^ 1);
                    tc_fence_after();
// ... 39 lines not shown
            mbar_wait(&tfull[acc], (seg >> 1) & 1);
            tc_fence_after();
            const uint32_t taddr = tmem_base + ((uint32_t)(quarter * 32) << 16) + (uint32_t)(acc * t.acc_stride);
            for (int c0 = 0; c0 < ((SGB_ABL & SGB_ABL_T_NO_DRAIN) ? 0 : kcols); c0 += 32) {
                float v[32];
                tmem_ld_32x32(taddr + (uint32_t)c0, v);
#pragma unroll
                for (int e = 0; e < 32; e += 4)
                    *reinterpret_cast<float4*>(stg + lane * kHEpiLd + e) =
                        make_float4((v[e] * invg) * inva, (v[e + 1] * invg) * inva, (v[e + 2] * invg) * inva, (v[e + 3] * invg) * inva);
                __syncwarp();
                if (c0 + cc < kcols) {
                    float4 old[8];
                    if (seg != 0) {
#pragma unroll
                        for (int i = 0; i < 8; ++i) old[i] = ldcg_hint(reinterpret_cast<const float4*>(orow + (int64_t)(4 * i) * t.k + c0), keep_policy);
                    }
#pragma unroll
                    for (int i = 0; i < 8; ++i) {
                        float4 o = *reinterpret_cast<const float4*>(stg + (i * 4 + (lane >> 3)) * kHEpiLd + cc);
                        if (seg != 0) { o.x += old[i].x; o.y += old[i].y; o.z += old[i].z; o.w += old[i].w; }
                        stcg_hint(reinterpret_cast<float4*>(orow + (int64_t)(4 * i) * t.k + c0), o, keep_policy);
                    }
                }
                __syncwarp();
            }
            tc_fence_before();
            __syncwarp();
            if (lane == 0) mbar_arrive_cluster(&tempty[acc], 0);
        }
    }
    tc_fence_before();
    __syncthreads();
    cluster_sync_all();
    if (warp == kPWarpMma) {
        tc_fence_after();
        tmem_dealloc_pair(tmem_base, t.tmem_cols);
    }
}

struct HPlan {
    int bn, n_tiles, k_chunks, stages, raw_stages, acc_stride;
    size_t smem_bytes, img_bytes;
    uint32_t tmem_cols;
    bool pair;
};

static bool h_pair_wanted(int64_t m, int n) {
    if (m <= kHBM) return false;
    if (const char* e = getenv("SGB_F16_PAIR")) return atoi(e) != 0 && n % 16 == 0 && n >= 32;
    return n % 32 == 0 && m >= 32768;
}

static HPlan h_plan(int n, int k, bool pair = false) {
    HPlan p;
    p.pair = pair;
    p.bn = n <= 256 ? n : 256;
    p.n_tiles = (n + p.bn - 1) / p.bn;
    p.k_chunks = (k + kHBK - 1) / kHBK;
    int sb = pair ? h_stage_bytes_pair(p.bn) : h_stage_bytes(p.bn);
    p.raw_stages = 3;
    if (const char* e = getenv("SGB_F16_RAW")) { int v = atoi(e); if (v >= 2 && v <= kHMaxRawStages) p.raw_stages = v; }
    int st = (kHSmemBudget - kHBarBytes - kHEpiBytes - p.raw_stages * kHRawBytes - 1024) / sb;
    p.stages = st > kHMaxStages ? kHMaxStages : st;
    if (const char* e = getenv("SGB_F16_STAGES")) { int v = atoi(e); if (v >= 2 && v <= p.stages) p.stages = v; }
    p.smem_bytes = (size_t)p.raw_stages * kHRawBytes + (size_t)p.stages * sb + kHBarBytes + kHEpiBytes;
    p.img_bytes = (size_t)p.n_tiles * p.k_chunks * 2 * h_b_tile_bytes(p.bn);
    p.acc_stride = (p.bn + 31) / 32 * 32;
    uint32_t cols = 32;
    while (cols < (uint32_t)(2 * p.acc_stride)) cols <<= 1;
    p.tmem_cols = cols;
    return p;
}

size_t gemm_f16_workspace(int n, int k) { return h_plan(n, k).img_bytes + 512; }

int gemm_f16_launch(const GemmArgs& g, const float* a_amax, void* ws, size_t ws_bytes, cudaStream_t stream) {
    HPlan p = h_plan(g.n, g.k, h_pair_wanted(g.m, g.n));
    if (!ws || ws_bytes < p.img_bytes + 512) {
        set_error("sgb_gemm: fp16-split engine needs %zu bytes of workspace, got %zu", p.img_bytes + 512, ws_bytes);
        return SGB_ENOSPC;
    }
    if (p.stages < 2) {
        set_error("sgb_gemm: tile does not fit shared memory");
        return SGB_ENOTSUP;
    }
    uint8_t* base = reinterpret_cast<uint8_t*>((reinterpret_cast<uintptr_t>(ws) + 255) & ~(uintptr_t)255);
    float* hdr = reinterpret_cast<float*>(base);
    uint8_t* img = base + 256;
    if (!a_amax) {
        int rc = amax_launch(g.a, g.lda, g.m, g.k, reinterpret_cast<uint32_t*>(hdr + 2), stream);
        if (rc != SGB_OK) return rc;
        a_amax = hdr + 2;
    }
    k_prep_weights_f16<<<num_sms(), 256, 0, stream>>>(g.b, g.ldb, g.transb, g.n, g.k, p.bn, p.n_tiles, p.k_chunks, reinterpret_cast<__half*>(img), hdr);
    SGB_CHECK_LAUNCH("k_prep_weights_f16");
    {
        static std::atomic<uint64_t> optin{0}, optin_pair{0};
        int rc = p.pair ? smem_optin(reinterpret_cast<const void*>(k_gemm_f16<true>), kHSmemBudget, &optin_pair)
                        : smem_optin(reinterpret_cast<const void*>(k_gemm_f16<false>), kHSmemBudget, &optin);
        if (rc != SGB_OK) return rc;
    }
    HArgs t{};
    {
        int rc = make_tmap_2d(&t.a_map, g.a, g.m, g.k, g.lda, kHBK, kHBM, true);
        if (rc != SGB_OK) return rc;
    }
    t.a = g.a; t.lda = g.lda; t.wp = img; t.wscale = hdr; t.a_amax = a_amax; t.c = g.c; t.ldc = g.ldc; t.m = g.m; t.n = g.n; t.k = g.k;
    t.bn = p.bn; t.n_tiles = p.n_tiles; t.k_chunks = p.k_chunks; t.stages = p.stages; t.raw_stages = p.raw_stages;
    t.bias = g.bias; t.accumulate = g.accumulate; t.stat_partials = g.stat_partials; t.tmem_cols = p.tmem_cols; t.acc_stride = p.acc_stride;
    const int64_t m_tiles = ceil_div(g.m, kHBM);
    int groups = num_sms() / p.n_tiles;
    if (groups < 1) groups = 1;
    if (groups > m_tiles) groups = (int)m_tiles;
    if (p.pair) groups = groups / 2 * 2;
    if (p.pair && groups < 2) {
        set_error("sgb_gemm: too few rows for CTA pairs");
        return SGB_ENOTSUP;
    }
    const int grid = groups * p.n_tiles;
    if (g.stat_partials) {
        SGB_CHECK_ARG((reinterpret_cast<uintptr_t>(g.stat_partials) & 15) == 0, "sgb_gemm: stat_partials must be 16-byte aligned");
        const int rows = gemm_stat_rows(g.m), written = 4 * groups;
        if (rows > written)
            SGB_CUDA(cudaMemsetAsync(g.stat_partials + (size_t)written * 3 * g.n, 0, (size_t)(rows - written) * 3 * g.n * sizeof(float), stream));
    }
    if (p.pair) {
        cudaLaunchConfig_t cfg{};
        cfg.gridDim = dim3((unsigned)grid);
        cfg.blockDim = dim3(kHThreads);
        cfg.dynamicSmemBytes = p.smem_bytes;
        cfg.stream = stream;
        cudaLaunchAttribute attr[1];
        attr[0].id = cudaLaunchAttributeClusterDimension;
        attr[0].val.clusterDim.x = 2; attr[0].val.clusterDim.y = 1; attr[0].val.clusterDim.z = 1;
        cfg.attrs = attr;
        cfg.numAttrs = 1;
        SGB_CUDA(cudaLaunchKernelEx(&cfg, k_gemm_f16<true>, t));
    } else {
        k_gemm_f16<false><<<grid, kHThreads, p.smem_bytes, stream>>>(t);
    }
    SGB_CHECK_LAUNCH("k_gemm_f16");
    return SGB_OK;
}

struct TPlan {
    int bk, k_tiles, n_tiles, stages, raw_stages, conv_groups, splits, acc_stride, gbox, abox;
    int64_t m_per_split;
    size_t smem_bytes, ws_bytes;
    uint32_t tmem_cols;
};

static TPlan t_plan(int64_t m, int n, int k) {
    TPlan p;
    int kpad = (k + 15) / 16 * 16;
    p.bk = kpad <= 256 ? kpad : 256;
    p.k_tiles = (k + p.bk - 1) / p.bk;
    p.n_tiles = (n + kTBM - 1) / kTBM;
    int sb = t_stage_bytes(p.bk);
    p.gbox = n < kTBM ? n : kTBM;
    p.abox = k < p.bk ? k : p.bk;
    int raw = (kTBV * (p.gbox + p.abox) * 4 + 127) / 128 * 128;
    int st = (kHSmemBudget - kTBarBytes - kTEpiBytes - kTRawStages * raw) / sb;
    p.stages = st > 4 ? 4 : st;
    int rs = (kHSmemBudget - kTBarBytes - kTEpiBytes - p.stages * sb) / raw;
    p.raw_stages = rs > kTMaxRawStages ? kTMaxRawStages : (rs < kTRawStages ? kTRawStages : rs);
    if (const char* e = getenv("SGB_TN_RAW")) { int v = atoi(e); if (v >= 2 && v <= p.raw_stages) p.raw_stages = v; }
    p.conv_groups = (p.gbox + p.abox <= kTProducerWarps * 32 / 2 && p.stages >= 2 && p.raw_stages >= 2) ? 2 : 1;
    if (const char* e = getenv("SGB_TN_GROUPS")) { if (atoi(e) == 1) p.conv_groups = 1; }
    p.smem_bytes = (size_t)p.raw_stages * raw + (size_t)p.stages * sb + kTBarBytes + kTEpiBytes;
    int tiles = p.k_tiles * p.n_tiles;
    int64_t want = num_sms() / tiles;
    if (want < 1) want = 1;
    int64_t maxs = ceil_div(m > 0 ? m : 1, 1024);
    p.splits = (int)(want < maxs ? want : maxs);
    p.m_per_split = ceil_div(ceil_div(m, p.splits), kTBV) * kTBV;
    p.ws_bytes = (size_t)p.splits * n * k * sizeof(float) + 512;
    p.acc_stride = (p.bk + 31) / 32 * 32;
    uint32_t cols = 32;
    while (cols < (uint32_t)(2 * p.acc_stride)) cols <<= 1;
    p.tmem_cols = cols;
    return p;
}

size_t gemm_tn_f16_workspace(int64_t m, int n, int k) { return t_plan(m, n, k).ws_bytes; }

int gemm_tn_f16_launch(const float* g, int64_t ldg, const float* a, int64_t lda, const float* g_amax, const float* a_amax, float* d,
                       int64_t ldd, int64_t m, int n, int k, int accumulate, void* ws, size_t ws_bytes, cudaStream_t stream) {
    TPlan p = t_plan(m, n, k);
    if (!ws || ws_bytes < p.ws_bytes) {
        set_error("sgb_gemm_tn: fp16-split engine needs %zu bytes of workspace, got %zu", p.ws_bytes, ws_bytes);
        return SGB_ENOSPC;
    }
    if (p.stages < 2) {
        set_error("sgb_gemm_tn: tile does not fit shared memory");
        return SGB_ENOTSUP;
    }
    uint8_t* base = reinterpret_cast<uint8_t*>((reinterpret_cast<uintptr_t>(ws) + 255) & ~(uintptr_t)255);
    float* hdr = reinterpret_cast<float*>(base);
    float* partial = reinterpret_cast<float*>(base + 256);
    if (!g_amax) {
        int rc = amax_launch(g, ldg, m, n, reinterpret_cast<uint32_t*>(hdr + 0), stream);
        if (rc != SGB_OK) return rc;
        g_amax = hdr + 0;
    }
    if (!a_amax) {
        int rc = amax_launch(a, lda, m, k, reinterpret_cast<uint32_t*>(hdr + 1), stream);
        if (rc != SGB_OK) return rc;
        a_amax = hdr + 1;
    }
    {
        static std::atomic<uint64_t> optin{0};
        int rc = smem_optin(reinterpret_cast<const void*>(k_gemm_tn_f16), kHSmemBudget, &optin);
        if (rc != SGB_OK) return rc;
    }
    TArgs t{};
    {
        int rc = make_tmap_2d(&t.g_map, g, m, n, ldg, p.gbox, kTBV, false);
        if (rc == SGB_OK) rc = make_tmap_2d(&t.a_map, a, m, k, lda, p.abox, kTBV, false);
        if (rc != SGB_OK) return rc;
        t.gbox = p.gbox; t.abox = p.abox;
    }
    t.g = g; t.ldg = ldg; t.a = a; t.lda = lda; t.g_amax = g_amax; t.a_amax = a_amax; t.partial = partial; t.m = m; t.n = n; t.k = k;
    t.bk = p.bk; t.k_tiles = p.k_tiles; t.stages = p.stages; t.raw_stages = p.raw_stages; t.conv_groups = p.conv_groups; t.m_per_split = p.m_per_split; t.tmem_cols = p.tmem_cols; t.acc_stride = p.acc_stride;
    dim3 grid((unsigned)(p.n_tiles * p.k_tiles), (unsigned)p.splits);
    k_gemm_tn_f16<<<grid, kTThreads, p.smem_bytes, stream>>>(t);
    SGB_CHECK_LAUNCH("k_gemm_tn_f16");
    return reduce_splits_launch(partial, p.splits, n, k, d, ldd, accumulate, stream);
}

bool gemm_tn_pair_ok(int64_t m, int n, int k) { return n % 256 == 0 && k % 32 == 0 && (k <= 256 || k % 256 == 0) && m >= 4096; }

struct PPlan {
    int bk, ah, k_tiles, pairs, stages, raw_stages, splits, acc_stride;
    int64_t m_per_split;
    size_t smem_bytes, ws_bytes;
    uint32_t tmem_cols;
};

static PPlan p_plan(int64_t m, int n, int k) {
    PPlan p;
    p.bk = k <= 256 ? k : 256;
    p.ah = p.bk / 2;
    p.k_tiles = k / p.bk;
    p.pairs = (n / 256) * p.k_tiles;
    const int sb = 2 * kTGTile + 2 * t_a_tile_bytes(p.ah);
    const int raw = (kTBV * (kTBM + p.ah) * 4 + 127) / 128 * 128;
    p.raw_stages = 3;
    if (const char* e = getenv("SGB_PAIR_RAW")) { int v = atoi(e); if (v >= 2 && v <= kPMaxRawStages) p.raw_stages = v; }
    int st = (kHSmemBudget - 256 - kTEpiBytes - p.raw_stages * raw) / sb;
    p.stages = st > kHMaxStages ? kHMaxStages : st;
    p.smem_bytes = (size_t)p.raw_stages * raw + (size_t)p.stages * sb + 256 + kTEpiBytes;
    int64_t want = num_sms() / (2 * p.pairs);
    if (want < 1) want = 1;
    const int64_t maxs = ceil_div(m > 0 ? m : 1, 1024);
    p.splits = (int)(want < maxs ? want : maxs);
    p.m_per_split = ceil_div(ceil_div(m, p.splits), kTBV) * kTBV;
    p.ws_bytes = (size_t)p.splits * n * k * sizeof(float) + 512;
    p.acc_stride = (p.bk + 31) / 32 * 32;
    uint32_t cols = 32;
    while (cols < (uint32_t)(2 * p.acc_stride)) cols <<= 1;
    p.tmem_cols = cols;
    return p;
}

size_t gemm_tn_pair_workspace(int64_t m, int n, int k) { return gemm_tn_pair_ok(m, n, k) ? p_plan(m, n, k).ws_bytes : 0; }

int gemm_tn_pair_launch(const float* g, int64_t ldg, const float* a, int64_t lda, const float* g_amax, const float* a_amax, float* d,
                        int64_t ldd, int64_t m, int n, int k, int accumulate, void* ws, size_t ws_bytes, cudaStream_t stream) {
    PPlan p = p_plan(m, n, k);
    if (!ws || ws_bytes < p.ws_bytes) {
        set_error("sgb_gemm_tn: pair engine needs %zu bytes of workspace, got %zu", p.ws_bytes, ws_bytes);
        return SGB_ENOSPC;
    }
    if (p.stages < 2) {
        set_error("sgb_gemm_tn: pair tile does not fit shared memory");
        return SGB_ENOTSUP;
    }
    uint8_t* base = reinterpret_cast<uint8_t*>((reinterpret_cast<uintptr_t>(ws) + 255) & ~(uintptr_t)255);
    float* hdr = reinterpret_cast<float*>(base);
    float* partial = reinterpret_cast<float*>(base + 256);
    if (!g_amax) {
        int rc = amax_launch(g, ldg, m, n, reinterpret_cast<uint32_t*>(hdr + 0), stream);
        if (rc != SGB_OK) return rc;
        g_amax = hdr + 0;
    }
    if (!a_amax) {
        int rc = amax_launch(a, lda, m, k, reinterpret_cast<uint32_t*>(hdr + 1), stream);
        if (rc != SGB_OK) return rc;
        a_amax = hdr + 1;
    }
    {
        static std::atomic<uint64_t> optin{0};
        int rc = smem_optin(reinterpret_cast<const void*>(k_gemm_tn_f16_pair), kHSmemBudget, &optin);
        if (rc != SGB_OK) return rc;
    }
    TPArgs t{};
    {
        int rc = make_tmap_2d(&t.g_map, g, m, n, ldg, kTBM, kTBV, false);
        if (rc == SGB_OK) rc = make_tmap_2d(&t.a_map, a, m, k, lda, p.ah, kTBV, false);
        if (rc != SGB_OK) return rc;
    }
    t.ah = p.ah; t.g_amax = g_amax; t.a_amax = a_amax; t.partial = partial; t.m = m; t.n = n; t.k = k;
    t.bk = p.bk; t.k_tiles = p.k_tiles; t.stages = p.stages; t.raw_stages = p.raw_stages; t.m_per_split = p.m_per_split; t.tmem_cols = p.tmem_cols; t.acc_stride = p.acc_stride;
    dim3 grid((unsigned)(2 * p.pairs), (unsigned)p.splits);
    k_gemm_tn_f16_pair<<<grid, kPThreads, p.smem_bytes, stream>>>(t);
    SGB_CHECK_LAUNCH("k_gemm_tn_f16_pair");
    return reduce_splits_launch(partial, p.splits, n, k, d, ldd, accumulate, stream);
}

}

extern "C" int sgb_amax(const float* x, int64_t ldx, int64_t m, int c, float* amax_out, void* stream) {
    SGB_CHECK_ARG(x && amax_out && m >= 0 && c > 0 && ldx >= c, "sgb_amax: bad argument");
    SGB_CHECK_ARG(c % 4 == 0 && ldx % 4 == 0 && (reinterpret_cast<uintptr_t>(x) & 15) == 0, "sgb_amax: needs c %% 4 == 0 and 16-byte aligned rows");
    return sgb::amax_launch(x, ldx, m, c, reinterpret_cast<uint32_t*>(amax_out), (cudaStream_t)stream);
}
```

semigcn_b200/networks.py:

```python
from __future__ import annotations

import numpy as np
import torch
import torch.nn as nn

from . import ops
from . import profile as _prof
from .nn import ChebConv, GCNConv, Sequential

SGCN_WIDTHS = [4, 16, 32, 64, 128, 256, 256, 512, 256, 256, 128, 64, 32, 16, 3]


class SingleScaleGCN(nn.Module):
    def __init__(self, device, activation: str = "lrelu", skip: bool = False, conv: str = "chebconv", widths=None):
        super().__init__()
        self.device, self.skip = device, skip
        self.comm = None
        h = list(widths) if widths is not None else list(SGCN_WIDTHS)
        self.h = h
        act = {"relu": nn.ReLU(), "lrelu": nn.LeakyReLU()}[activation]

        def mk(i):
            if conv == "gcnconv":
                return GCNConv(h[i], h[i + 1])
            if conv == "chebconv":
                return ChebConv(h[i], h[i + 1], K=3)
            raise ValueError(conv)

        nb = len(h) - 2
        blocks = []
        for i in range(nb - 1):
            blocks.append(Sequential("x, edge_index", [(mk(i), "x, edge_index -> x"), nn.BatchNorm1d(h[i + 1]), act]))
        blocks.append(Sequential("x, edge_index", [(mk(nb - 1), "x, edge_index -> x"), nn.BatchNorm1d(h[nb]), act,
                                                   (nn.Linear(h[nb], h[nb + 1]), "x -> x")]))
        self.blocks = nn.ModuleList(blocks)
        self.skip_blocks = nn.ModuleList([nn.Linear(h[i + 1] * 2, h[i + 1]) for i in range(min(6, nb))])

    def forward(self, data, dm=None):
        z1, x_pos, edge_index = data.z1.to(self.device), data.x_pos.to(self.device), data.edge_index.to(self.device)
        if type(dm) == np.ndarray:
            dm = torch.from_numpy(dm)
        elif type(dm) != torch.Tensor:
            dm = torch.ones([z1.shape[0], 1])
        dm = dm.to(self.device)
        if self.comm is None and z1.is_cuda and not z1.requires_grad and dm.numel() == z1.shape[0]:
            x = ops.input_prep(z1, dm)
        else:
            prep = _prof.span("input_prep", 4.0 * 11 * z1.shape[0]) if _prof.ACTIVE is not None else None
            z_min, z_max = torch.min(z1, dim=0, keepdim=True)[0], torch.max(z1, dim=0, keepdim=True)[0]
            if self.comm is not None:
                z_min, z_max = self.comm.all_reduce_min(z_min.clone()), self.comm.all_reduce_max(z_max.clone())
            z_sc = torch.max(z_max - z_min)
            zc = (z_min + z_max) * 0.5
            z1 = (z1 - zc) / z_sc
            z1 = dm * z1
            x = torch.cat([z1, dm], dim=1)
            if prep is not None:
                prep.close()
        skip_in = []
        nblk = len(self.blocks)
        for i, b in enumerate(self.blocks):
            if i <= 5:
                x = b(x, edge_index)
                skip_in.append(x)
            elif i <= 7:
                x = b(x, edge_index)
            else:
                if self.skip:
                    lin = self.skip_blocks[nblk - i]
                    x = ops.linear(torch.cat([skip_in[nblk - i], x], dim=1), lin.weight, lin.bias)
                x = b(x, edge_index)
        return x_pos + x
```

semigcn_b200/nn.py:

```python
from __future__ import annotations

import math
from typing import List, Optional, Tuple

import torch
import torch.nn as nn
from torch import Tensor

from . import ops
from ._lib import MODE_CHEB, MODE_GCN, SgbError, require_cuda


def _glorot_(w: Tensor) -> None:
    a = math.sqrt(6.0 / (w.size(-2) + w.size(-1)))
    w.data.uniform_(-a, a)


class _PygLinear(nn.Module):

    def __init__(self, in_channels: int, out_channels: int):
        super().__init__()
        self.in_channels, self.out_channels = in_channels, out_channels
        self.weight = nn.Parameter(torch.empty(out_channels, in_channels))
        self.register_parameter("bias", None)
        self.reset_parameters()

    def reset_parameters(self) -> None:
        _glorot_(self.weight)

    def forward(self, x: Tensor) -> Tensor:
        return ops.linear(x, self.weight, None)


def _check_inputs(x: Tensor, edge_index: Tensor, in_channels: int) -> None:
    require_cuda(x, edge_index)
    if x.dim() != 2 or x.shape[1] != in_channels:
        raise SgbError(f"expected x of shape [N, {in_channels}], got {tuple(x.shape)}")
    if x.dtype != torch.float32:
        raise SgbError("x must be float32")


class GCNConv(nn.Module):

    def __init__(self, in_channels: int, out_channels: int, improved: bool = False, cached: bool = False,
                 add_self_loops: bool = True, normalize: bool = True, bias: bool = True, **kwargs):
        super().__init__()
        if improved or not add_self_loops or not normalize:
            raise SgbError("GCNConv: only improved=False, add_self_loops=True, normalize=True are supported")
        if kwargs:
            raise SgbError(f"GCNConv: unsupported arguments {sorted(kwargs)}")
        self.in_channels, self.out_channels = in_channels, out_channels
        self.improved, self.cached, self.add_self_loops, self.normalize = improved, cached, add_self_loops, normalize
        self.lin = _PygLinear(in_channels, out_channels)
        if bias:
            self.bias = nn.Parameter(torch.empty(out_channels))
        else:
            self.register_parameter("bias", None)
        self.reset_parameters()

    def reset_parameters(self) -> None:
        self.lin.reset_parameters()
        if self.bias is not None:
            self.bias.data.zero_()

    def forward(self, x: Tensor, edge_index: Tensor, edge_weight: Optional[Tensor] = None) -> Tensor:
        if edge_weight is not None:
            raise SgbError("GCNConv: edge_weight is not supported (the reference never passes one)")
        _check_inputs(x, edge_index, self.in_channels)
        g = ops.graph_for(edge_index, x.shape[0], MODE_GCN)
        return ConvBlockFn.apply(x, g, _BlockCfg("gcn", None, 1.0), self.bias, None, None, self.lin.weight)

    def __repr__(self) -> str:
        return f"GCNConv({self.in_channels}, {self.out_channels})"


class ChebConv(nn.Module):

    def __init__(self, in_channels: int, out_channels: int, K: int, normalization: Optional[str] = "sym",
                 bias: bool = True, **kwargs):
        super().__init__()
        if K <= 0:
            raise SgbError("ChebConv: K must be positive")
        if normalization != "sym":
            raise SgbError("ChebConv: only normalization='sym' is supported")
        if kwargs:
            raise SgbError(f"ChebConv: unsupported arguments {sorted(kwargs)}")
        self.in_channels, self.out_channels, self.normalization = in_channels, out_channels, normalization
        self.lins = nn.ModuleList([_PygLinear(in_channels, out_channels) for _ in range(K)])
        if bias:
            self.bias = nn.Parameter(torch.empty(out_channels))
        else:
            self.register_parameter("bias", None)
        self.reset_parameters()

    def reset_parameters(self) -> None:
        for lin in self.lins:
            lin.reset_parameters()
        if self.bias is not None:
            self.bias.data.zero_()

    def forward(self, x: Tensor, edge_index: Tensor, edge_weight: Optional[Tensor] = None,
                batch: Optional[Tensor] = None, lambda_max: Optional[Tensor] = None) -> Tensor:
        if edge_weight is not None or batch is not None or lambda_max is not None:
            raise SgbError("ChebConv: edge_weight / batch / lambda_max are not supported (lambda_max is 2.0 for 'sym')")
        _check_inputs(x, edge_index, self.in_channels)
        g = ops.graph_for(edge_index, x.shape[0], MODE_CHEB)
        return ConvBlockFn.apply(x, g, _BlockCfg("cheb", None, 1.0), self.bias, None, None, *[l.weight for l in self.lins])

    def __repr__(self) -> str:
        return f"ChebConv({self.in_channels}, {self.out_channels}, K={len(self.lins)}, normalization={self.normalization})"


class _BlockCfg:
    def __init__(self, kind: str, bn: Optional[nn.BatchNorm1d], slope: float, x_amax: Optional[Tensor] = None):
        self.kind, self.bn, self.slope = kind, bn, slope
        self.x_amax = x_amax
        self.out_amax = None


class ConvBlockFn(torch.autograd.Function):

    @staticmethod
    def forward(ctx, x, graph, cfg, bias, gamma, beta, *weights):
        x = ops._f32c(x, "x")
        bn = cfg.bn
        training = bn is not None and (bn.training or bn.running_mean is None)
        want_stats = training
        saved_ops: List[Tensor] = []
        am = ops.new_amax(x.device, 4)
        x_amax = cfg.x_amax
        if cfg.kind == "gcn":
            (w,) = weights
            cout, cin = w.shape
            agg_first = cin <= cout
            if agg_first:
                p = ops.spmm(graph, x, amax_out=am[0:1])
                r = ops.gemm(p, w, transb=True, bias=bias, want_stats=want_stats, a_amax=am[0:1])
                saved_ops = [p]
                ctx.op_amax = [am[0:1]]
            else:
                h = ops.gemm(x, w, transb=True, a_amax=x_amax)
                r = ops.spmm(graph, h, bias=bias, want_stats=want_stats)
                saved_ops = [x]
                ctx.op_amax = [x_amax]
            ctx.agg_first = agg_first
        else:
            nw = len(weights)
            cin = x.shape[1]
            tcat = None
            if nw > 1:
                tcat = torch.empty((x.shape[0], (nw - 1) * cin), dtype=torch.float32, device=x.device)
                tk = [x] + [tcat[:, (k - 1) * cin:k * cin] for k in range(1, nw)]
                ops.spmm(graph, x, out=tk[1], amax_out=am[0:1])
                for k in range(2, nw):
                    ops.spmm(graph, tk[k - 1], alpha=2.0, addend=tk[k - 2], beta=-1.0, out=tk[k], amax_out=am[0:1])
            one = nw == 1
            r = ops.gemm(x, weights[0], transb=True, bias=bias if one else None, want_stats=want_stats and one, a_amax=x_amax)
            if not one:
                wcat = weights[1] if nw == 2 else torch.cat(list(weights[1:]), dim=1)
                r = ops.gemm(tcat, wcat, transb=True, bias=bias, out=r, accumulate=True, want_stats=want_stats, a_amax=am[0:1])
            saved_ops = [x] if one else [x, tcat]
            ctx.op_amax = [x_amax, am[0:1]]
        y, partials = r if want_stats else (r, None)

        ctx.graph, ctx.cfg, ctx.nw, ctx.has_bias = graph, cfg, len(weights), bias is not None
        if bn is None:
            ctx.bn_mode = 0
            ctx.save_for_backward(*weights, *saved_ops)
            return y
        if training:
            momentum = 0.1 if bn.momentum is None else bn.momentum
            if bn.track_running_stats and bn.num_batches_tracked is not None:
                bn.num_batches_tracked.add_(1)
                if bn.momentum is None:
                    momentum = 1.0 / float(bn.num_batches_tracked)
            rm = bn.running_mean if bn.track_running_stats else None
            rv = bn.running_var if bn.track_running_stats else None
            mean, invstd, scale, shift = ops.bn_finalize(partials, graph.n_global, gamma, beta, bn.eps, momentum, rm, rv,
                                                         comm=graph.comm)
        else:
            mean, invstd, scale, shift = ops.eval_affine(bn.running_mean, bn.running_var, gamma, beta, bn.eps)
        z = ops.bn_act_apply(y, mean, scale, shift, cfg.slope, amax_out=am[3:4])
        cfg.out_amax = am[3:4]
        ctx.bn_mode = 2 if training else 1
        ctx.has_affine = gamma is not None
        ctx.save_for_backward(*weights, *saved_ops, y, scale, shift, mean, invstd)
        return z

    @staticmethod
    def backward(ctx, dz):
        cfg, graph, nw = ctx.cfg, ctx.graph, ctx.nw
        saved = ctx.saved_tensors
        weights = saved[:nw]
        dgamma = dbeta = None
        dz = dz.contiguous()
        am = ops.new_amax(dz.device, 2)
        dy_amax = None
        if ctx.bn_mode == 0:
            saved_ops = saved[nw:]
            dy = dz
        else:
            saved_ops = saved[nw:-5]
            y, scale, shift, mean, invstd = saved[-5:]
            dy_amax = am[0:1]
            dy, dgamma, dbeta = ops.bn_act_bwd(dz, y, scale, shift, mean, invstd, cfg.slope, ctx.bn_mode == 2,
                                               comm=graph.comm, n_global=graph.n_global, amax_out=dy_amax)
            if not ctx.has_affine:
                dgamma = dbeta = None
        need_x = ctx.needs_input_grad[0]
        db = None
        want_db = ctx.has_bias and ctx.needs_input_grad[3]
        dy_used_by_gemm = cfg.kind != "gcn" or ctx.agg_first
        if dy_amax is None and dy_used_by_gemm:
            if want_db and ctx.bn_mode != 2:
                dy_amax = am[0:1]
                db = ops.colsum(dy, amax_out=dy_amax)
                want_db = False
            elif ops.tensor_core_likely(dy.shape[0], weights[0].shape[1], dy.shape[1]):
                dy_amax = ops.amax(dy)
        if want_db:
            if ctx.bn_mode == 2:
                db = torch.zeros(dy.shape[1], dtype=dy.dtype, device=dy.device)
            else:
                db = ops.colsum(dy)
        dws: List[Optional[Tensor]] = [None] * nw
        dx = None
        if cfg.kind == "gcn":
            (w,) = weights
            if ctx.agg_first:
                (p,) = saved_ops
                dws[0] = ops.gemm_tn(dy, p, g_amax=dy_amax, a_amax=ctx.op_amax[0])
                if need_x:
                    dp = ops.gemm(dy, w, transb=False, a_amax=dy_amax)
                    dx = ops.spmm(graph, dp, transpose=True)
            else:
                (x,) = saved_ops
                dh = ops.spmm(graph, dy, transpose=True, amax_out=am[1:2])
                dws[0] = ops.gemm_tn(dh, x, g_amax=am[1:2], a_amax=ctx.op_amax[0])
                if need_x:
                    dx = ops.gemm(dh, w, transb=False, a_amax=am[1:2])
        else:
            x = saved_ops[0]
            cin = x.shape[1]
            dws[0] = ops.gemm_tn(dy, x, g_amax=dy_amax, a_amax=ctx.op_amax[0])
            if nw > 1:
                tcat = saved_ops[1]
                dwcat = ops.gemm_tn(dy, tcat, g_amax=dy_amax, a_amax=ctx.op_amax[1])
                for k in range(1, nw):
                    dws[k] = dwcat[:, (k - 1) * cin:k * cin]
            if need_x:
                ds: List[Optional[Tensor]] = [ops.gemm(dy, weights[0], transb=False, a_amax=dy_amax)]
                if nw > 1:
                    wcat = weights[1] if nw == 2 else torch.cat(list(weights[1:]), dim=1)
                    dcat = ops.gemm(dy, wcat, transb=False, a_amax=dy_amax)
                    ds += [dcat[:, (k - 1) * cin:k * cin] for k in range(1, nw)]
                gs: List[Optional[Tensor]] = [None] * nw
                for k in range(nw - 1, -1, -1):
                    d = ds[k]
                    if k + 2 <= nw - 1:
                        d = torch.sub(d, gs[k + 2], out=d)
                    if k + 1 <= nw - 1:
                        d = ops.spmm(graph, gs[k + 1], transpose=True, alpha=2.0 if k >= 1 else 1.0, addend=d, beta=1.0)
                    gs[k] = d
                dx = gs[0]
        return (dx, None, None, db, dgamma, dbeta, *dws)


class _SparseHashModule(nn.Module):

    _buffer_name = "hash"

    def __init__(self, hash_matrix: Tensor):
        super().__init__()
        self.register_buffer(self._buffer_name, hash_matrix)
        self._op = None
        self._op_key = None

    def _row_scale(self, mat: Tensor) -> Optional[Tensor]:
        return None

    def _operator(self, device) -> "ops.SparseOp":
        mat = getattr(self, self._buffer_name)
        key = (str(device), mat._version if not mat.is_sparse else id(mat))
        if self._op is None or self._op_key != key:
            m = mat.to(device)
            self._op = ops.SparseOp(m, self._row_scale(m))
            self._op_key = key
        return self._op

    def forward(self, input: Tensor) -> Tensor:
        require_cuda(input)
        if input.dtype != torch.float32 or input.dim() != 2:
            raise SgbError(f"{type(self).__name__}: expected a float32 [N, C] tensor")
        return ops.sparse_mm(self._operator(input.device), input)


class MeshPool(_SparseHashModule):

    _buffer_name = "pool_hash"

    def __init__(self, pool_hash: Tensor):
        super().__init__(pool_hash)

    def _row_scale(self, mat: Tensor) -> Tensor:
        m = mat if mat.is_sparse else mat.to_sparse()
        v_sum = torch.sparse.sum(m, dim=1).to_dense().to(torch.float32)
        return torch.where(v_sum != 0, 1.0 / v_sum, torch.zeros_like(v_sum))


class MeshUnpool(_SparseHashModule):

    _buffer_name = "unpool_hash"

    def __init__(self, unpool_hash: Tensor):
        super().__init__(unpool_hash)


class Sequential(nn.Module):

    def __init__(self, input_args: str, modules: list):
        super().__init__()
        self._in_names = [a.strip() for a in input_args.split(",")]
        self._descs: List[Tuple[List[str], List[str]]] = []
        for i, entry in enumerate(modules):
            if isinstance(entry, (tuple, list)):
                mod, desc = entry
                lhs, rhs = desc.split("->")
                ins = [a.strip() for a in lhs.split(",")]
                outs = [a.strip() for a in rhs.split(",")]
            else:
                mod = entry
                prev = self._descs[-1][1] if self._descs else self._in_names[:1]
                ins, outs = list(prev), list(prev)
            if isinstance(mod, nn.Module):
                setattr(self, f"module_{i}", mod)
            else:
                object.__setattr__(self, f"module_{i}", mod)
            self._descs.append((ins, outs))

    def __len__(self) -> int:
        return len(self._descs)

    def __getitem__(self, i: int):
        return getattr(self, f"module_{i}")

    def _fusable(self, i: int) -> Optional[Tuple[int, float]]:
        conv = self[i]
        if not isinstance(conv, (GCNConv, ChebConv)) or i + 1 >= len(self):
            return None
        ins, outs = self._descs[i]
        if len(ins) != 2 or len(outs) != 1:
            return None
        bn = self[i + 1]
        if type(bn) is not nn.BatchNorm1d or self._descs[i + 1][0] != outs:
            return None
        if i + 2 < len(self) and self._descs[i + 2][0] == outs:
            act = self[i + 2]
            if type(act) is nn.LeakyReLU:
                return 3, float(act.negative_slope)
            if type(act) is nn.ReLU:
                return 3, 0.0
        return 2, 1.0

    def forward(self, *args):
        env = dict(zip(self._in_names, args))
        out = None
        i = 0
        while i < len(self):
            ins, outs = self._descs[i]
            mod = self[i]
            fuse = self._fusable(i)
            if fuse is not None:
                consumed, slope = fuse
                x, edge_index = env[ins[0]], env[ins[1]]
                bn = self[i + 1]
                _check_inputs(x, edge_index, mod.in_channels)
                if isinstance(mod, GCNConv):
                    g = ops.graph_for(edge_index, x.shape[0], MODE_GCN)
                    cfg = _BlockCfg("gcn", bn, slope, ops.amax_of(x))
                    out = ConvBlockFn.apply(x, g, cfg, mod.bias, bn.weight, bn.bias, mod.lin.weight)
                else:
                    g = ops.graph_for(edge_index, x.shape[0], MODE_CHEB)
                    cfg = _BlockCfg("cheb", bn, slope, ops.amax_of(x))
                    out = ConvBlockFn.apply(x, g, cfg, mod.bias, bn.weight, bn.bias, *[l.weight for l in mod.lins])
                if cfg.out_amax is not None:
                    ops.tag_amax(out, cfg.out_amax)
                env[outs[0]] = out
                i += consumed
                continue
            vals = [env[k] for k in ins]
            if type(mod) is nn.Linear and len(vals) == 1 and vals[0].is_cuda and vals[0].dim() == 2:
                out = ops.linear(vals[0], mod.weight, mod.bias)
            elif (type(mod) is nn.BatchNorm1d and len(vals) == 1 and vals[0].is_cuda and vals[0].dim() == 2
                  and vals[0].dtype == torch.float32 and len(outs) == 1):
                slope, consumed = 1.0, 1
                if i + 1 < len(self) and self._descs[i + 1][0] == outs:
                    act = self[i + 1]
                    if type(act) is nn.LeakyReLU:
                        slope, consumed = float(act.negative_slope), 2
                    elif type(act) is nn.ReLU:
                        slope, consumed = 0.0, 2
                out = ops.bn_act(vals[0], mod, slope)
                env[outs[0]] = out
                i += consumed
                continue
            else:
                out = mod(*vals)
            if len(outs) == 1:
                env[outs[0]] = out
            else:
                for k, v in zip(outs, out):
                    env[k] = v
            i += 1
        return out
```

semigcn_b200/ops.py:

```python
from __future__ import annotations

import os
import weakref
from collections import OrderedDict
from typing import Optional, Tuple

import torch
from torch import Tensor

from . import _lib as L
from . import profile as _prof
from ._lib import MODE_ADJ, MODE_CHEB, MODE_GCN, SgbError, check, ptr, require_cuda, stream_ptr

Affine = Optional[Tuple[Tensor, Tensor, Tensor, float]]


def _f32c(t: Tensor, name: str) -> Tensor:
    if t.dtype != torch.float32:
        raise SgbError(f"{name}: expected float32, got {t.dtype}")
    if t.dim() == 2 and t.stride(1) != 1:
        t = t.contiguous()
    elif t.dim() != 2 and not t.is_contiguous():
        t = t.contiguous()
    return t
# ... 126 lines not shown

def clear_graph_cache() -> None:
    _GRAPH_CACHE.clear()
    _GRAPH_CACHE_PINNED.clear()
    _GRAPH_BY_CONTENT.clear()
    _GRAPH_ALIAS.clear()


def spmm(g: MeshGraph, x: Tensor, transpose: bool = False, in_affine: Affine = None, alpha: float = 1.0,
         addend: Optional[Tensor] = None, beta: float = 0.0, bias: Optional[Tensor] = None,
         want_stats: bool = False, out: Optional[Tensor] = None, amax_out: Optional[Tensor] = None):
    lib = L.load()
    require_cuda(x, addend, bias)
    x = _f32c(x, "x")
    n, c = x.shape
    if n != g.n:
        raise SgbError(f"x has {n} rows but the graph has {g.n} vertices")
    y = out if out is not None else torch.empty((n, c), dtype=torch.float32, device=x.device)
    if addend is not None:
        addend = _f32c(addend, "addend")
    rowptr, edges = g.csr(transpose)
    mu, sc, sh, slope = (in_affine if in_affine is not None else (None, None, None, 0.0))
    nnz_eff = int(g.nnz) + (n if g.mode == MODE_GCN else 0)
    sp = _prof.span(f"spmm_c{c}", 4.0 * (2 * n * c + nnz_eff + 2 * n + 1 + (n * c if addend is not None else 0)),
                    2.0 * nnz_eff * c) if _prof.ACTIVE is not None else None
    n_int = int(getattr(g, "n_interior", 0)) if g.halo is not None else 0
    ranges = [(0, n, True)] if not (0 < n_int < n) else [(0, n_int, False), (n_int, n - n_int, True)]
    pending = g.halo.start(x) if g.halo is not None else None
    partials, row_off = None, 0
    if want_stats:
        rows = sum(lib.sgb_spmm_stat_rows(cnt, c) for (_, cnt, _) in ranges)
        partials = torch.empty((rows, 3, c), dtype=torch.float32, device=x.device)
    xg = None
    with torch.cuda.device(x.device):
        for (r0, cnt, needs_ghosts) in ranges:
            if needs_ghosts and pending is not None:
                xg = g.halo.finish(pending)
            part = partials[row_off:] if partials is not None else None
            check(lib.sgb_spmm_range(ptr(rowptr), ptr(edges), ptr(g.dis), g.mode, ptr(x), x.stride(0), r0, cnt, c,
                                     ptr(xg) if needs_ghosts else None, xg.stride(0) if (needs_ghosts and xg is not None) else 0, n,
                                     ptr(mu), ptr(sc), ptr(sh), float(slope), float(alpha), ptr(addend),
                                     addend.stride(0) if addend is not None else 0, float(beta), ptr(bias),
                                     ptr(y), y.stride(0), ptr(part), ptr(amax_out), stream_ptr(x.device)), "sgb_spmm")
            if partials is not None:
                row_off += lib.sgb_spmm_stat_rows(cnt, c)
            L.count(1)
    if sp is not None:
        sp.close()
    return (y, partials) if want_stats else y


def gemm(a: Tensor, b: Tensor, transb: bool = True, a_affine: Affine = None, bias: Optional[Tensor] = None,
         out: Optional[Tensor] = None, accumulate: bool = False, want_stats: bool = False, engine: int = 0,
         a_amax: Optional[Tensor] = None):
    lib = L.load()
    require_cuda(a, b, bias)
    a, b = _f32c(a, "a"), _f32c(b, "b")
    m, k = a.shape
    n = b.shape[0] if transb else b.shape[1]
    if (b.shape[1] if transb else b.shape[0]) != k:
        raise SgbError(f"gemm: inner dimensions differ ({a.shape} x {b.shape}, transb={transb})")
    c = out if out is not None else torch.empty((m, n), dtype=torch.float32, device=a.device)
    partials = None
    if want_stats:
        partials = torch.empty((lib.sgb_gemm_stat_rows(m), 3, n), dtype=torch.float32, device=a.device)
    mu, sc, sh, slope = (a_affine if a_affine is not None else (None, None, None, 0.0))
    sp = _prof.span(f"gemm_n{n}_k{k}", 4.0 * (m * (k + n) + k * n + (m * n if accumulate else 0)), 2.0 * m * n * k) \
        if _prof.ACTIVE is not None else None
    wsb = lib.sgb_gemm_workspace_bytes(m, n, k, engine)
    ws = _ws(wsb, a.device) if wsb else None
    with torch.cuda.device(a.device):
        check(lib.sgb_gemm(1 if transb else 0, ptr(a), a.stride(0), ptr(b), b.stride(0), ptr(c), c.stride(0), m, n, k,
                           ptr(mu), ptr(sc), ptr(sh), float(slope), ptr(bias), 1 if accumulate else 0, ptr(partials),
                           ptr(a_amax), ptr(ws), wsb, engine, stream_ptr(a.device)), "sgb_gemm")
    if sp is not None:
        sp.close()
    L.count(1)
    return (c, partials) if want_stats else c


def gemm_tn(gmat: Tensor, a: Tensor, out: Optional[Tensor] = None, accumulate: bool = False, engine: int = 0,
            g_amax: Optional[Tensor] = None, a_amax: Optional[Tensor] = None) -> Tensor:
    lib = L.load()
    require_cuda(gmat, a)
    gmat, a = _f32c(gmat, "g"), _f32c(a, "a")
    m, n = gmat.shape
    k = a.shape[1]
    if a.shape[0] != m:
        raise SgbError("gemm_tn: row counts differ")
    d = out if out is not None else torch.empty((n, k), dtype=torch.float32, device=a.device)
    wsb = lib.sgb_gemm_tn_workspace_bytes(m, n, k)
    ws = _ws(wsb, a.device)
    sp = _prof.span(f"gemm_tn_n{n}_k{k}", 4.0 * (m * (k + n) + k * n), 2.0 * m * n * k) if _prof.ACTIVE is not None else None
    with torch.cuda.device(a.device):
        check(lib.sgb_gemm_tn(ptr(gmat), gmat.stride(0), ptr(a), a.stride(0), ptr(d), d.stride(0), m, n, k,
                              1 if accumulate else 0, ptr(g_amax), ptr(a_amax), ptr(ws), wsb, engine, stream_ptr(a.device)), "sgb_gemm_tn")
    if sp is not None:
        sp.close()
    L.count(2)
    return d


def colsum(gmat: Tensor, out: Optional[Tensor] = None, accumulate: bool = False, amax_out: Optional[Tensor] = None) -> Tensor:
    lib = L.load()
    require_cuda(gmat)
    gmat = _f32c(gmat, "g")
    m, n = gmat.shape
    o = out if out is not None else torch.empty(n, dtype=torch.float32, device=gmat.device)
    wsb = lib.sgb_colsum_workspace_bytes(m, n)
    ws = _ws(wsb, gmat.device)
    sp = _prof.span(f"colsum_c{n}", 4.0 * m * n) if _prof.ACTIVE is not None else None
    with torch.cuda.device(gmat.device):
        check(lib.sgb_colsum(ptr(gmat), gmat.stride(0), m, n, ptr(o), 1 if accumulate else 0, ptr(amax_out), ptr(ws), wsb,
                             stream_ptr(gmat.device)), "sgb_colsum")
    if sp is not None:
        sp.close()
    L.count(2)
    return o


def tensor_core_likely(m: int, cin: int, cout: int) -> bool:
    return m >= 2048 and ((cin >= 32 and cout >= 16) or (cout >= 32 and cin >= 16))


def amax(x: Tensor) -> Optional[Tensor]:
    lib = L.load()
    require_cuda(x)
    x = _f32c(x, "x")
    m, c = x.shape
    if c % 4 != 0 or x.stride(0) % 4 != 0 or x.data_ptr() % 16 != 0:
        return None
    out = torch.empty(1, dtype=torch.float32, device=x.device)
    with torch.cuda.device(x.device):
        check(lib.sgb_amax(ptr(x), x.stride(0), m, c, ptr(out), stream_ptr(x.device)), "sgb_amax")
    L.count(1)
    return out


def input_prep(z1: Tensor, dm: Optional[Tensor]) -> Tensor:
    lib = L.load()
    require_cuda(z1, dm)
    z1 = _f32c(z1.detach(), "z1")
    n = int(z1.shape[0])
    if z1.dim() != 2 or z1.shape[1] != 3:
        raise SgbError("input_prep: z1 must be [N, 3]")
    if dm is not None:
        dm = dm.detach().to(torch.float32).reshape(-1).contiguous()
        if dm.numel() != n:
            raise SgbError("input_prep: mask must have one entry per vertex")
    x = torch.empty((n, 4), dtype=torch.float32, device=z1.device)
    scratch = torch.empty(16, dtype=torch.float32, device=z1.device)
    sp = _prof.span("input_prep", 4.0 * 11 * n) if _prof.ACTIVE is not None else None
    with torch.cuda.device(z1.device):
        check(lib.sgb_input_prep(ptr(z1), z1.stride(0), n, ptr(dm), ptr(x), ptr(scratch), stream_ptr(z1.device)), "sgb_input_prep")
    if sp is not None:
        sp.close()
    L.count(3)
    return x


def col_stats(y: Tensor) -> Tensor:
    lib = L.load()
    y = _f32c(y, "y")
    m, c = y.shape
    partials = torch.empty((lib.sgb_col_stat_rows(m, c), 3, c), dtype=torch.float32, device=y.device)
    sp = _prof.span(f"col_stats_c{c}", 4.0 * m * c) if _prof.ACTIVE is not None else None
    with torch.cuda.device(y.device):
        check(lib.sgb_col_stats(ptr(y), y.stride(0), m, c, ptr(partials), stream_ptr(y.device)), "sgb_col_stats")
    if sp is not None:
        sp.close()
    L.count(1)
    return partials


def gather_rows(x: Tensor, idx: Tensor, out: Optional[Tensor] = None) -> Tensor:
    lib = L.load()
    require_cuda(x, idx)
    x = _f32c(x, "x")
    count, c = int(idx.numel()), int(x.shape[1])
    o = out if out is not None else torch.empty((count, c), dtype=torch.float32, device=x.device)
    with torch.cuda.device(x.device):
        check(lib.sgb_gather_rows(ptr(x), x.stride(0), ptr(idx), count, c, ptr(o), o.stride(0), stream_ptr(x.device)), "sgb_gather_rows")
    L.count(1)
    return o


def merge_moment_rows(partials: Tensor) -> Tensor:
    if partials.is_cuda:
        lib = L.load()
        partials = partials.contiguous()
        rows, _, c = partials.shape
        out = torch.empty((1, 3, c), dtype=torch.float32, device=partials.device)
        with torch.cuda.device(partials.device):
            check(lib.sgb_moments_merge(ptr(partials), rows, c, ptr(out), stream_ptr(partials.device)), "sgb_moments_merge")
        L.count(1)
        return out
    p = partials.to(torch.float64)
    n_r, mean_r, m2_r = p[:, 0, :], p[:, 1, :], p[:, 2, :]
    n = n_r.sum(dim=0)
    safe = torch.where(n > 0, n, torch.ones_like(n))
    mean = (n_r * mean_r).sum(dim=0) / safe
    d = mean_r - mean.unsqueeze(0)
    m2 = (m2_r + n_r * d * d).sum(dim=0)
    return torch.stack([n, mean, m2]).unsqueeze(0).to(torch.float32).contiguous()


def bn_finalize(partials: Tensor, count: int, gamma: Optional[Tensor], beta: Optional[Tensor], eps: float,
                momentum: float, running_mean: Optional[Tensor], running_var: Optional[Tensor], comm=None):
    lib = L.load()
    if comm is not None:
        partials = comm.all_gather_cat(merge_moment_rows(partials).contiguous())
    rows, _, c = partials.shape
    dev = partials.device
    sp = _prof.span("bn_finalize", 12.0 * rows * c) if _prof.ACTIVE is not None else None
    st = torch.empty((4, c), dtype=torch.float32, device=dev)
    with torch.cuda.device(dev):
        check(lib.sgb_bn_finalize(ptr(partials), rows, c, count, ptr(gamma), ptr(beta), float(eps), float(momentum),
                                  ptr(running_mean), ptr(running_var), ptr(st[0]), ptr(st[1]), ptr(st[2]), ptr(st[3]),
                                  stream_ptr(dev)), "sgb_bn_finalize")
    if sp is not None:
        sp.close()
    L.count(1)
    return st[0], st[1], st[2], st[3]


def bn_act_apply(y: Tensor, mean: Tensor, scale: Tensor, shift: Tensor, slope: float, out: Optional[Tensor] = None,
                 amax_out: Optional[Tensor] = None) -> Tensor:
    lib = L.load()
    y = _f32c(y, "y")
    m, c = y.shape
    z = out if out is not None else torch.empty_like(y)
    sp = _prof.span(f"bn_act_apply_c{c}", 8.0 * m * c) if _prof.ACTIVE is not None else None
    with torch.cuda.device(y.device):
        check(lib.sgb_bn_act_apply(ptr(y), y.stride(0), m, c, ptr(mean), ptr(scale), ptr(shift), float(slope), ptr(z), z.stride(0),
                                   ptr(amax_out), stream_ptr(y.device)), "sgb_bn_act_apply")
    if sp is not None:
        sp.close()
    L.count(1)
    return z


def bn_act_bwd(dz: Tensor, y: Tensor, scale: Tensor, shift: Tensor, mean: Optional[Tensor], invstd: Optional[Tensor],
               slope: float, training: bool, want_param_grads: bool = True, comm=None, n_global: Optional[int] = None,
               amax_out: Optional[Tensor] = None):
    lib = L.load()
    dz, y = _f32c(dz, "dz"), _f32c(y, "y")
    m, c = y.shape
    dev = y.device
    dy = torch.empty_like(y)
    dgamma = dbeta = sums = None
    sp = _prof.span(f"bn_act_bwd_c{c}", 4.0 * m * c * (5 if training else 3)) if _prof.ACTIVE is not None else None
    with torch.cuda.device(dev):
        if training or want_param_grads:
            if mean is None:
                raise SgbError("bn_act_bwd: mean/invstd required")
            rows = lib.sgb_col_stat_rows(m, c)
            partials = torch.empty((rows, 2, c), dtype=torch.float32, device=dev)
            check(lib.sgb_bn_act_bwd_reduce(ptr(dz), dz.stride(0), ptr(y), y.stride(0), m, c, ptr(scale), ptr(shift),
                                            ptr(mean), ptr(invstd), float(slope), ptr(partials), stream_ptr(dev)),
                  "sgb_bn_act_bwd_reduce")
            sums = torch.empty((2, c), dtype=torch.float32, device=dev)
            dgamma = torch.empty(c, dtype=torch.float32, device=dev)
            dbeta = torch.empty(c, dtype=torch.float32, device=dev)
            check(lib.sgb_bn_bwd_finalize(ptr(partials), rows, c, ptr(sums), ptr(dgamma), ptr(dbeta), 0, stream_ptr(dev)),
                  "sgb_bn_bwd_finalize")
            L.count(2)
            if comm is not None and training:
                sums = comm.all_reduce_sum(sums.clone()) * (float(m) / float(n_global))
        check(lib.sgb_bn_act_bwd_apply(ptr(dz), dz.stride(0), ptr(y), y.stride(0), m, c, ptr(scale), ptr(shift), ptr(mean),
                                       ptr(invstd), ptr(sums), float(slope), 1 if training else 0, ptr(dy), dy.stride(0),
                                       ptr(amax_out), stream_ptr(dev)), "sgb_bn_act_bwd_apply")
        L.count(1)
# ... 166 lines not shown
```

Measured before the change: 2.559 billion.

## Defer BatchNorm+LeakyReLU into next GCN block's tensor-core GEMM prologue

Instead of materialising the BN+activation output between blocks, the producing block returns a deferred object, and the next GCNConv applies the affine+LeakyReLU inside its fp16-split GEMM prologue, forward and backward (gemm_tn). The GEMM epilogue records per-column min/max order keys, so bn_finalize can bound the post-activation amax without a separate amax pass. This removes one full elementwise read/write pass and an amax kernel per deferred layer. In exchange it adds API surface, engine restrictions and more complex autograd plumbing, and relies on monotonic-bound reasoning for the fp16 scaling.

After: 2.592 billion, median of 6. 1.3% higher.

```diff
diff --git a/include/semigcn_b200.h b/include/semigcn_b200.h
--- a/include/semigcn_b200.h
+++ b/include/semigcn_b200.h
@@ -66,11 +66,13 @@
 SGB_API int sgb_gemm(int transb, const float* a, int64_t lda, const float* b, int64_t ldb,
              float* c, int64_t ldc, int64_t m, int n, int k,
              const float* a_mean, const float* a_scale, const float* a_shift, float slope,
-             const float* bias, int accumulate, float* stat_partials, const float* a_amax,
-             void* workspace, size_t workspace_bytes, int engine, void* stream);
+             const float* bias, int accumulate, float* stat_partials,
+             int32_t* stat_extremes ,
+             const float* a_amax, void* workspace, size_t workspace_bytes, int engine, void* stream);
 SGB_API size_t sgb_gemm_tn_workspace_bytes(int64_t m, int n, int k);
 SGB_API int sgb_gemm_tn(const float* g, int64_t ldg, const float* a, int64_t lda, float* d, int64_t ldd,
                 int64_t m, int n, int k, int accumulate, const float* g_amax, const float* a_amax,
+                const float* a_mean, const float* a_scale, const float* a_shift, float slope,
                 void* workspace, size_t workspace_bytes, int engine, void* stream);
 SGB_API size_t sgb_colsum_workspace_bytes(int64_t m, int n);
 SGB_API int sgb_colsum(const float* g, int64_t ldg, int64_t m, int n, float* out, int accumulate,
@@ -83,7 +85,10 @@
 SGB_API int sgb_bn_finalize(const float* partials, int rows, int c, int64_t count,
                     const float* gamma, const float* beta, float eps, float momentum,
                     float* running_mean, float* running_var,
-                    float* mean, float* invstd, float* scale, float* shift, void* stream);
+                    float* mean, float* invstd, float* scale, float* shift,
+                    const int32_t* extremes, float slope,
+                    float* amax_out ,
+                    void* stream);
 SGB_API int sgb_moments_merge(const float* partials, int rows, int c, float* merged , void* stream);
 SGB_API int sgb_bn_act_apply(const float* y, int64_t ldy, int64_t m, int c, const float* mean, const float* scale,
                      const float* shift, float slope, float* z, int64_t ldz, float* amax_out , void* stream);
diff --git a/semigcn_b200/_lib.py b/semigcn_b200/_lib.py
--- a/semigcn_b200/_lib.py
+++ b/semigcn_b200/_lib.py
@@ -35,16 +35,16 @@
     "sgb_gemm_stat_rows": (_i32, [_i64]),
     "sgb_gemm_workspace_bytes": (_sz, [_i64, _i32, _i32, _i32]),
     "sgb_gemm": (_i32, [_i32, _vp, _i64, _vp, _i64, _vp, _i64, _i64, _i32, _i32, _vp, _vp, _vp, _f32, _vp, _i32,
-                        _vp, _vp, _vp, _sz, _i32, _vp]),
+                        _vp, _vp, _vp, _vp, _sz, _i32, _vp]),
     "sgb_gemm_tn_workspace_bytes": (_sz, [_i64, _i32, _i32]),
-    "sgb_gemm_tn": (_i32, [_vp, _i64, _vp, _i64, _vp, _i64, _i64, _i32, _i32, _i32, _vp, _vp, _vp, _sz, _i32, _vp]),
+    "sgb_gemm_tn": (_i32, [_vp, _i64, _vp, _i64, _vp, _i64, _i64, _i32, _i32, _i32, _vp, _vp, _vp, _vp, _vp, _f32, _vp, _sz, _i32, _vp]),
     "sgb_colsum_workspace_bytes": (_sz, [_i64, _i32]),
     "sgb_colsum": (_i32, [_vp, _i64, _i64, _i32, _vp, _i32, _vp, _vp, _sz, _vp]),
     "sgb_amax": (_i32, [_vp, _i64, _i64, _i32, _vp, _vp]),
     "sgb_moments_merge": (_i32, [_vp, _i32, _i32, _vp, _vp]),
     "sgb_col_stat_rows": (_i32, [_i64, _i32]),
     "sgb_col_stats": (_i32, [_vp, _i64, _i64, _i32, _vp, _vp]),
-    "sgb_bn_finalize": (_i32, [_vp, _i32, _i32, _i64, _vp, _vp, _f32, _f32, _vp, _vp, _vp, _vp, _vp, _vp, _vp]),
+    "sgb_bn_finalize": (_i32, [_vp, _i32, _i32, _i64, _vp, _vp, _f32, _f32, _vp, _vp, _vp, _vp, _vp, _vp, _vp, _f32, _vp, _vp]),
     "sgb_bn_act_apply": (_i32, [_vp, _i64, _i64, _i32, _vp, _vp, _vp, _f32, _vp, _i64, _vp, _vp]),
     "sgb_bn_act_bwd_reduce": (_i32, [_vp, _i64, _vp, _i64, _i64, _i32, _vp, _vp, _vp, _vp, _f32, _vp, _vp]),
     "sgb_bn_bwd_finalize": (_i32, [_vp, _i32, _i32, _vp, _vp, _vp, _i32, _vp]),
diff --git a/semigcn_b200/csrc/bn.cu b/semigcn_b200/csrc/bn.cu
--- a/semigcn_b200/csrc/bn.cu
+++ b/semigcn_b200/csrc/bn.cu
@@ -163,6 +163,8 @@
     const float* gamma; const float* beta; float eps; float momentum;
     float* running_mean; float* running_var;
     float* mean; float* invstd; float* scale; float* shift;
+    const int32_t* ext; float slope;
+    float* amax;
     float* sums; float* dgamma; float* dbeta; int accumulate;
     int kind;
 };
@@ -203,6 +205,7 @@
     r2[threadIdx.y][threadIdx.x] = s2;
     r3[threadIdx.y][threadIdx.x] = s3;
     __syncthreads();
+    float bound = 0.f;
     if (threadIdx.y == 0 && ch < f.c) {
         if (f.kind == 0 || f.kind == 3) {
             double n = 0.0, mean = 0.0, m2 = 0.0;
@@ -229,6 +232,11 @@
             f.invstd[ch] = (float)invstd;
             f.scale[ch] = (float)(g * invstd);
             f.shift[ch] = (float)b;
+            if (f.amax) {
+                const float mu = f.mean[ch], sc = f.scale[ch], sh = f.shift[ch];
+                const float hi = float_from_order_key(f.ext[ch]), lo = -float_from_order_key(f.ext[f.c + ch]);
+                bound = fmaxf(fabsf(bn_lrelu(hi, mu, sc, sh, f.slope)), fabsf(bn_lrelu(lo, mu, sc, sh, f.slope)));
+            }
             if (f.running_mean) {
                 const double unb = n > 1.0 ? m2 / (n - 1.0) : var;
                 f.running_mean[ch] = (float)((1.0 - f.momentum) * (double)f.running_mean[ch] + f.momentum * mean);
@@ -246,6 +254,10 @@
                 f.sums[ch] = f.accumulate ? f.sums[ch] + (float)t1 : (float)t1;
             }
         }
+    }
+    if (f.amax && threadIdx.y == 0) {
+        const uint32_t b = __reduce_max_sync(0xffffffffu, __float_as_uint(bound));
+        if (threadIdx.x == 0 && b) atomicMax(reinterpret_cast<uint32_t*>(f.amax), b);
     }
 }
 
@@ -371,13 +383,14 @@
 
 extern "C" int sgb_bn_finalize(const float* partials, int rows, int c, int64_t count, const float* gamma, const float* beta,
                                float eps, float momentum, float* running_mean, float* running_var, float* mean, float* invstd,
-                               float* scale, float* shift, void* stream) {
+                               float* scale, float* shift, const int32_t* extremes, float slope, float* amax_out, void* stream) {
     SGB_CHECK_ARG(partials && rows > 0 && c > 0 && count > 0 && mean && invstd && scale && shift, "sgb_bn_finalize: bad argument");
     SGB_CHECK_ARG((running_mean == nullptr) == (running_var == nullptr), "sgb_bn_finalize: running stats must come together");
     FinArgs f{};
     f.partials = partials; f.rows = rows; f.c = c; f.count = count; f.gamma = gamma; f.beta = beta; f.eps = eps;
     f.momentum = momentum; f.running_mean = running_mean; f.running_var = running_var;
-    f.mean = mean; f.invstd = invstd; f.scale = scale; f.shift = shift; f.kind = 0;
+    SGB_CHECK_ARG(!amax_out || (extremes && slope >= 0.f), "sgb_bn_finalize: amax_out needs the column extremes and slope >= 0");
+    f.mean = mean; f.invstd = invstd; f.scale = scale; f.shift = shift; f.ext = extremes; f.slope = slope; f.amax = amax_out; f.kind = 0;
     k_finalize<<<(c + 31) / 32, dim3(32, 32), 0, (cudaStream_t)stream>>>(f);
     SGB_CHECK_LAUNCH("k_finalize");
     return SGB_OK;
diff --git a/semigcn_b200/csrc/common.cuh b/semigcn_b200/csrc/common.cuh
--- a/semigcn_b200/csrc/common.cuh
+++ b/semigcn_b200/csrc/common.cuh
@@ -3,6 +3,7 @@
 #include <stdint.h>
 #include <stdio.h>
 #include <stdarg.h>
+#include <string.h>
 #include <atomic>
 #include "../../include/semigcn_b200.h"
 
@@ -96,6 +97,23 @@
     int64_t m; int n; int k;
     const float* a_mean; const float* a_scale; const float* a_shift; float slope;
     const float* bias; int accumulate; float* stat_partials;
+    int32_t* stat_ext;
+};
+
+__host__ __device__ __forceinline__ int32_t float_order_key(float v) {
+    int32_t b;
+    memcpy(&b, &v, 4);
+    return b >= 0 ? b : b ^ 0x7fffffff;
+}
+__host__ __device__ __forceinline__ float float_from_order_key(int32_t k) {
+    const int32_t b = k >= 0 ? k : k ^ 0x7fffffff;
+    float v;
+    memcpy(&v, &b, 4);
+    return v;
+}
+
+struct AffinePrologue {
+    const float* mean = nullptr; const float* scale = nullptr; const float* shift = nullptr; float slope = 0.f;
 };
 
 }
diff --git a/semigcn_b200/csrc/gemm.cu b/semigcn_b200/csrc/gemm.cu
--- a/semigcn_b200/csrc/gemm.cu
+++ b/semigcn_b200/csrc/gemm.cu
@@ -14,14 +14,15 @@
 int gemm_tn_tc_launch(const float* g, int64_t ldg, const float* a, int64_t lda, float* d, int64_t ldd, int64_t m, int n, int k,
                       int accumulate, void* ws, size_t ws_bytes, cudaStream_t stream);
 size_t gemm_f16_workspace(int n, int k);
+bool gemm_f16_prologue_ok(int k);
 int gemm_f16_launch(const GemmArgs& g, const float* a_amax, void* ws, size_t ws_bytes, cudaStream_t stream);
 size_t gemm_tn_f16_workspace(int64_t m, int n, int k);
-int gemm_tn_f16_launch(const float* g, int64_t ldg, const float* a, int64_t lda, const float* g_amax, const float* a_amax, float* d,
-                       int64_t ldd, int64_t m, int n, int k, int accumulate, void* ws, size_t ws_bytes, cudaStream_t stream);
+int gemm_tn_f16_launch(const float* g, int64_t ldg, const float* a, int64_t lda, const float* g_amax, const float* a_amax, const AffinePrologue& pro,
+                       float* d, int64_t ldd, int64_t m, int n, int k, int accumulate, void* ws, size_t ws_bytes, cudaStream_t stream);
 bool gemm_tn_pair_ok(int64_t m, int n, int k);
 size_t gemm_tn_pair_workspace(int64_t m, int n, int k);
-int gemm_tn_pair_launch(const float* g, int64_t ldg, const float* a, int64_t lda, const float* g_amax, const float* a_amax, float* d,
-                        int64_t ldd, int64_t m, int n, int k, int accumulate, void* ws, size_t ws_bytes, cudaStream_t stream);
+int gemm_tn_pair_launch(const float* g, int64_t ldg, const float* a, int64_t lda, const float* g_amax, const float* a_amax, const AffinePrologue& pro,
+                        float* d, int64_t ldd, int64_t m, int n, int k, int accumulate, void* ws, size_t ws_bytes, cudaStream_t stream);
 static bool tn_tc_worthwhile(int64_t m, int n, int k) { return n >= 32 && k >= 16 && m >= 4096; }
 
 static bool tc_worthwhile(int64_t m, int n, int k) { return n >= 32 && k >= 16 && m >= 2048; }
@@ -49,16 +50,23 @@
 
 extern "C" int sgb_gemm(int transb, const float* a, int64_t lda, const float* b, int64_t ldb, float* c, int64_t ldc, int64_t m,
                         int n, int k, const float* a_mean, const float* a_scale, const float* a_shift, float slope, const float* bias,
-                        int accumulate, float* stat_partials, const float* a_amax, void* workspace, size_t workspace_bytes, int engine,
-                        void* stream) {
+                        int accumulate, float* stat_partials, int32_t* stat_extremes, const float* a_amax, void* workspace,
+                        size_t workspace_bytes, int engine, void* stream) {
     SGB_CHECK_ARG(a && b && c && m >= 0 && n > 0 && k > 0, "sgb_gemm: bad argument m=%lld n=%d k=%d", (long long)m, n, k);
     SGB_CHECK_ARG(lda >= k && ldc >= n && ldb >= (transb ? k : n), "sgb_gemm: leading dimension too small");
     SGB_CHECK_ARG((a_scale == nullptr) == (a_shift == nullptr) && (a_scale == nullptr) == (a_mean == nullptr),
                   "sgb_gemm: a_mean / a_scale / a_shift must come together");
     SGB_CHECK_ARG(engine >= 0 && engine <= 3, "sgb_gemm: bad engine %d", engine);
     if (m == 0) return SGB_OK;
-    GemmArgs g{transb, a, lda, b, ldb, c, ldc, m, n, k, a_mean, a_scale, a_shift, slope, bias, accumulate, stat_partials};
+    SGB_CHECK_ARG(!stat_extremes || stat_partials, "sgb_gemm: stat_extremes come with stat_partials");
+    GemmArgs g{transb, a, lda, b, ldb, c, ldc, m, n, k, a_mean, a_scale, a_shift, slope, bias, accumulate, stat_partials, stat_extremes};
     const bool tc_ok = gemm_tc_supported(m, n, k, lda, ldc, a, c, bias, a_scale);
+    const bool f16_auto = engine == 0 && tc_ok && tc_worthwhile(m, n, k) && workspace && (!a_scale || gemm_f16_prologue_ok(k)) &&
+                          workspace_bytes >= gemm_f16_workspace(n, k);
+    if (stat_extremes && !((engine == 3 && tc_ok) || f16_auto)) {
+        set_error("sgb_gemm: stat_extremes are written by the fp16-split engine only (n=%d k=%d)", n, k);
+        return SGB_ENOTSUP;
+    }
     if (engine == 2) {
         if (!tc_ok) {
             set_error("sgb_gemm: tcgen05 engine needs n %% 16 == 0, k %% 4 == 0 and 16-byte aligned operands (n=%d k=%d)", n, k);
@@ -67,14 +75,14 @@
         return gemm_tc_launch(g, workspace, workspace_bytes, (cudaStream_t)stream);
     }
     if (engine == 3) {
-        if (!tc_ok || a_scale) {
-            set_error("sgb_gemm: fp16-split engine needs n %% 16 == 0, k %% 4 == 0, 16-byte aligned operands and no A prologue (n=%d k=%d)", n, k);
+        if (!tc_ok) {
+            set_error("sgb_gemm: fp16-split engine needs n %% 16 == 0, k %% 4 == 0 and 16-byte aligned operands (n=%d k=%d)", n, k);
             return SGB_ENOTSUP;
         }
         return gemm_f16_launch(g, a_amax, workspace, workspace_bytes, (cudaStream_t)stream);
     }
     if (engine == 0 && tc_ok && tc_worthwhile(m, n, k) && workspace) {
-        if (!a_scale && workspace_bytes >= gemm_f16_workspace(n, k))
+        if (f16_auto)
             return gemm_f16_launch(g, a_amax, workspace, workspace_bytes, (cudaStream_t)stream);
         if (workspace_bytes >= gemm_tc_workspace(n, k)) return gemm_tc_launch(g, workspace, workspace_bytes, (cudaStream_t)stream);
     }
@@ -92,11 +100,16 @@
 }
 
 extern "C" int sgb_gemm_tn(const float* g, int64_t ldg, const float* a, int64_t lda, float* d, int64_t ldd, int64_t m, int n, int k,
-                           int accumulate, const float* g_amax, const float* a_amax, void* workspace, size_t workspace_bytes, int engine,
-                           void* stream) {
+                           int accumulate, const float* g_amax, const float* a_amax, const float* a_mean, const float* a_scale,
+                           const float* a_shift, float slope, void* workspace, size_t workspace_bytes, int engine, void* stream) {
     SGB_CHECK_ARG(g && a && d && m >= 0 && n > 0 && k > 0, "sgb_gemm_tn: bad argument");
     SGB_CHECK_ARG(ldg >= n && lda >= k && ldd >= k, "sgb_gemm_tn: leading dimension too small");
     SGB_CHECK_ARG(engine >= 0 && engine <= 4, "sgb_gemm_tn: bad engine %d", engine);
+    SGB_CHECK_ARG((a_scale == nullptr) == (a_shift == nullptr) && (a_scale == nullptr) == (a_mean == nullptr),
+                  "sgb_gemm_tn: a_mean / a_scale / a_shift must come together");
+    SGB_CHECK_ARG(!a_scale || ((reinterpret_cast<uintptr_t>(a_mean) | reinterpret_cast<uintptr_t>(a_scale) | reinterpret_cast<uintptr_t>(a_shift)) & 15) == 0,
+                  "sgb_gemm_tn: a_mean / a_scale / a_shift must be 16-byte aligned");
+    const AffinePrologue pro{a_mean, a_scale, a_shift, slope};
     const bool tc_ok = gemm_tn_tc_supported(m, n, k, ldg, lda, g, a);
     if (engine == 0 && tc_ok && gemm_tn_pair_ok(m, n, k) && m >= 32768) engine = 4;
     if (engine == 4) {
@@ -104,7 +117,12 @@
             set_error("sgb_gemm_tn: the pair engine needs n %% 256 == 0, k %% 32 == 0 (k <= 256 or k %% 256 == 0), m >= 4096 and 16-byte aligned operands");
             return SGB_ENOTSUP;
         }
-        return gemm_tn_pair_launch(g, ldg, a, lda, g_amax, a_amax, d, ldd, m, n, k, accumulate, workspace, workspace_bytes, (cudaStream_t)stream);
+        return gemm_tn_pair_launch(g, ldg, a, lda, g_amax, a_amax, pro, d, ldd, m, n, k, accumulate, workspace, workspace_bytes, (cudaStream_t)stream);
+    }
+    if (a_scale && engine != 3 && !(engine == 0 && tc_ok && tn_tc_worthwhile(m, n, k))) {
+        set_error("sgb_gemm_tn: the BatchNorm prologue runs on the fp16-split engines (3, 4) only: n >= 32, k >= 16, m >= 4096, "
+                  "n %% 4 == 0, k %% 4 == 0 and 16-byte aligned operands for engine 0");
+        return SGB_ENOTSUP;
     }
     if (engine == 2) {
         if (!tc_ok) {
@@ -118,7 +136,7 @@
             set_error("sgb_gemm_tn: fp16-split engine needs n %% 4 == 0, k %% 4 == 0 and 16-byte aligned operands");
             return SGB_ENOTSUP;
         }
-        return gemm_tn_f16_launch(g, ldg, a, lda, g_amax, a_amax, d, ldd, m, n, k, accumulate, workspace, workspace_bytes, (cudaStream_t)stream);
+        return gemm_tn_f16_launch(g, ldg, a, lda, g_amax, a_amax, pro, d, ldd, m, n, k, accumulate, workspace, workspace_bytes, (cudaStream_t)stream);
     }
     if (engine == 0 && tc_ok && tn_tc_worthwhile(m, n, k))
         return gemm_tn_tc_launch(g, ldg, a, lda, d, ldd, m, n, k, accumulate, workspace, workspace_bytes, (cudaStream_t)stream);
diff --git a/semigcn_b200/csrc/gemm_f16.cu b/semigcn_b200/csrc/gemm_f16.cu
--- a/semigcn_b200/csrc/gemm_f16.cu
+++ b/semigcn_b200/csrc/gemm_f16.cu
@@ -39,14 +39,22 @@
 #endif
 }
 
-__global__ void __launch_bounds__(256) k_amax(const float* __restrict__ x, int64_t ldx, int64_t m, int c, uint32_t* __restrict__ slot) {
+__global__ void __launch_bounds__(256) k_amax(const float* __restrict__ x, int64_t ldx, int64_t m, int c, const float* __restrict__ mean,
+                                              const float* __restrict__ scale, const float* __restrict__ shift, float slope,
+                                              uint32_t* __restrict__ slot) {
     const int cv = c >> 2;
     const int64_t total = m * cv;
     float mx = 0.f;
     for (int64_t i = blockIdx.x * (int64_t)blockDim.x + threadIdx.x; i < total; i += (int64_t)gridDim.x * blockDim.x) {
         const int64_t r = i / cv;
         const int ch = (int)(i % cv) * 4;
-        const float4 v = ldg4(x + r * ldx + ch);
+        float4 v = ldg4(x + r * ldx + ch);
+        if (mean) {
+            v.x = bn_lrelu(v.x, __ldg(mean + ch), __ldg(scale + ch), __ldg(shift + ch), slope);
+            v.y = bn_lrelu(v.y, __ldg(mean + ch + 1), __ldg(scale + ch + 1), __ldg(shift + ch + 1), slope);
+            v.z = bn_lrelu(v.z, __ldg(mean + ch + 2), __ldg(scale + ch + 2), __ldg(shift + ch + 2), slope);
+            v.w = bn_lrelu(v.w, __ldg(mean + ch + 3), __ldg(scale + ch + 3), __ldg(shift + ch + 3), slope);
+        }
         mx = fmaxf(mx, fmaxf(fmaxf(fabsf(v.x), fabsf(v.y)), fmaxf(fabsf(v.z), fabsf(v.w))));
     }
     uint32_t b = __float_as_uint(mx);
@@ -60,13 +68,18 @@
     }
 }
 
-int amax_launch(const float* x, int64_t ldx, int64_t m, int c, uint32_t* slot, cudaStream_t stream) {
+int amax_launch(const float* x, int64_t ldx, int64_t m, int c, uint32_t* slot, cudaStream_t stream, const AffinePrologue& pro = AffinePrologue{}) {
     SGB_CUDA(cudaMemsetAsync(slot, 0, sizeof(uint32_t), stream));
     const int64_t total = m * (c / 4);
     const int grid = (int)min64(ceil_div(total > 0 ? total : 1, 256 * 8), (int64_t)num_sms() * 8);
-    k_amax<<<grid, 256, 0, stream>>>(x, ldx, m, c, slot);
+    k_amax<<<grid, 256, 0, stream>>>(x, ldx, m, c, pro.mean, pro.scale, pro.shift, pro.slope, slot);
     SGB_CHECK_LAUNCH("k_amax");
     return SGB_OK;
+}
+
+__device__ __forceinline__ float4 bn_lrelu4(float4 v, float4 mu, float4 sc, float4 sh, float slope) {
+    return make_float4(bn_lrelu(v.x, mu.x, sc.x, sh.x, slope), bn_lrelu(v.y, mu.y, sc.y, sh.y, slope), bn_lrelu(v.z, mu.z, sc.z, sh.z, slope),
+                       bn_lrelu(v.w, mu.w, sc.w, sh.w, slope));
 }
 
 __device__ __forceinline__ void split_f16x2(float x0, float x1, uint32_t& hi, uint32_t& lo) {
@@ -99,6 +112,7 @@
 constexpr int kHEpiBytes = kHEpiWarps * 32 * 32 * 4;
 constexpr int kTEpiBytes = 4 * 32 * kHEpiLd * 4;
 static const int kHSmemBudget = 227 * 1024;
+constexpr int kHMaxAffK = 512;
 
 __host__ __device__ constexpr int h_b_tile_bytes(int bn) { return (bn / 8) * kHBSbo; }
 __host__ __device__ constexpr int h_stage_bytes(int bn) { return (2 * kHATile + 2 * h_b_tile_bytes(bn) + 1023) / 1024 * 1024; }
@@ -115,7 +129,9 @@
     int bn; int n_tiles; int k_chunks; int stages; int raw_stages;
     const float* bias; int accumulate;
     float* stat_partials;
+    int32_t* stat_ext;
     uint32_t tmem_cols; int acc_stride;
+    AffinePrologue pro;
 };
 
 __global__ void __launch_bounds__(256) k_prep_weights_f16(const float* __restrict__ w, int64_t ldw, int transb, int n, int k, int bn,
@@ -165,7 +181,8 @@
 template <bool FULL>
 __device__ __forceinline__ void h_epi_chunk(const HArgs& g, uint32_t taddr, float* __restrict__ stg, float* __restrict__ cp ,
                                             const float* __restrict__ bias_p, int lane, int grp, int cc, int nvalid, bool col_ok, float sc1, float sc2,
-                                            bool stats, float inv_nb, float (&blk_mean)[4], float (&blk_m2)[4]) {
+                                            bool stats, float inv_nb, float (&blk_mean)[4], float (&blk_m2)[4], float (&blk_max)[4],
+                                            float (&blk_nmax)[4]) {
     float4 b = make_float4(0.f, 0.f, 0.f, 0.f);
     if (bias_p && (FULL || col_ok)) b = ldg4(bias_p);
     float v[32];
@@ -231,11 +248,30 @@
             blk_mean[q] = sm[q];
             blk_m2[q] = d2[q];
         }
+        if (g.stat_ext) {
+            float mx[4] = {-INFINITY, -INFINITY, -INFINITY, -INFINITY}, nx[4] = {-INFINITY, -INFINITY, -INFINITY, -INFINITY};
+#pragma unroll
+            for (int i = 0; i < 8; ++i) {
+                if (FULL || i * 4 + grp < nvalid) {
+                    mx[0] = fmaxf(mx[0], o[i].x); mx[1] = fmaxf(mx[1], o[i].y); mx[2] = fmaxf(mx[2], o[i].z); mx[3] = fmaxf(mx[3], o[i].w);
+                    nx[0] = fmaxf(nx[0], -o[i].x); nx[1] = fmaxf(nx[1], -o[i].y); nx[2] = fmaxf(nx[2], -o[i].z); nx[3] = fmaxf(nx[3], -o[i].w);
+                }
+            }
+#pragma unroll
+            for (int q = 0; q < 4; ++q) {
+                mx[q] = fmaxf(mx[q], __shfl_xor_sync(0xffffffffu, mx[q], 8));
+                mx[q] = fmaxf(mx[q], __shfl_xor_sync(0xffffffffu, mx[q], 16));
+                nx[q] = fmaxf(nx[q], __shfl_xor_sync(0xffffffffu, nx[q], 8));
+                nx[q] = fmaxf(nx[q], __shfl_xor_sync(0xffffffffu, nx[q], 16));
+                blk_max[q] = mx[q];
+                blk_nmax[q] = nx[q];
+            }
+        }
     }
     __syncwarp();
 }
 
-template <bool PAIR>
+template <bool PAIR, bool AFF>
 __global__ void __launch_bounds__(kHThreads, 1) k_gemm_f16(const __grid_constant__ HArgs g) {
     extern __shared__ __align__(1024) uint8_t smem[];
     const int warp = threadIdx.x >> 5, lane = threadIdx.x & 31;
@@ -255,6 +291,16 @@
     uint64_t* rempty = rfull + kHMaxRawStages;
     uint64_t* bfull = rempty + kHMaxRawStages;
     uint32_t* tmem_slot = reinterpret_cast<uint32_t*>(bfull + kHMaxStages);
+    float* const aff = reinterpret_cast<float*>(op_base + (size_t)g.stages * stage_bytes + kHBarBytes + kHEpiBytes);
+    const int aff_ld = g.k_chunks * kHBK;
+    if (AFF) {
+        for (int i = threadIdx.x; i < aff_ld; i += blockDim.x) {
+            const bool in = i < g.k;
+            aff[i] = in ? __ldg(g.pro.mean + i) : 0.f;
+            aff[aff_ld + i] = in ? __ldg(g.pro.scale + i) : 0.f;
+            aff[2 * aff_ld + i] = in ? __ldg(g.pro.shift + i) : 0.f;
+        }
+    }
 
     if (threadIdx.x == 0) {
         for (int s = 0; s < g.stages; ++s) {
@@ -308,6 +354,12 @@
         uint32_t rs = (uint32_t)grp % raw_stages, rph = ((uint32_t)grp / raw_stages) & 1u;
         for (uint32_t it = (uint32_t)grp; it < total_it; it += GROUPS) {
             mbar_wait(&rempty[rs], rph ^ 1);
+            int aff_col = 0, rows_left = kHBM;
+            if (AFF) {
+                const uint32_t tl = it / k_chunks, q = it - tl * k_chunks;
+                aff_col = (int)q * kHBK + cq * 8;
+                rows_left = (int)min64(g.m - SGB_H_M0_OF((int64_t)unit + (int64_t)tl * units), (int64_t)kHBM);
+            }
             mbar_wait(&rfull[rs], rph);
             const uint8_t* raw = raw_base + (size_t)rs * kHRawBytes;
             uint4 h[RPT], l[RPT];
@@ -319,6 +371,21 @@
                     const int r = r0 + RSTEP * (hf * HALF + i);
                     v[i][0] = *reinterpret_cast<const float4*>(raw + r * 128 + (((2 * cq) ^ (r & 7)) << 4));
                     v[i][1] = *reinterpret_cast<const float4*>(raw + r * 128 + (((2 * cq + 1) ^ (r & 7)) << 4));
+                }
+                if (AFF) {
+                    const float4 mu0 = *reinterpret_cast<const float4*>(aff + aff_col), mu1 = *reinterpret_cast<const float4*>(aff + aff_col + 4);
+                    const float4 sc0 = *reinterpret_cast<const float4*>(aff + aff_ld + aff_col), sc1 = *reinterpret_cast<const float4*>(aff + aff_ld + aff_col + 4);
+                    const float4 sh0 = *reinterpret_cast<const float4*>(aff + 2 * aff_ld + aff_col), sh1 = *reinterpret_cast<const float4*>(aff + 2 * aff_ld + aff_col + 4);
+#pragma unroll
+                    for (int i = 0; i < HALF; ++i) {
+                        v[i][0] = bn_lrelu4(v[i][0], mu0, sc0, sh0, g.pro.slope);
+                        v[i][1] = bn_lrelu4(v[i][1], mu1, sc1, sh1, g.pro.slope);
+                    }
+                    if (rows_left < kHBM) {
+#pragma unroll
+                        for (int i = 0; i < HALF; ++i)
+                            if (r0 + RSTEP * (hf * HALF + i) >= rows_left) v[i][0] = v[i][1] = make_float4(0.f, 0.f, 0.f, 0.f);
+                    }
                 }
 #pragma unroll
                 for (int i = 0; i < HALF; ++i) {
@@ -457,6 +524,7 @@
         const int n0 = nt * g.bn;
         const int ncols = min(g.bn, g.n - n0);
         float st_mean[4] = {0.f, 0.f, 0.f, 0.f}, st_m2[4] = {0.f, 0.f, 0.f, 0.f}, st_n = 0.f;
+        float st_max[4] = {-INFINITY, -INFINITY, -INFINITY, -INFINITY}, st_nmax[4] = {-INFINITY, -INFINITY, -INFINITY, -INFINITY};
         int64_t tile = unit;
         for (uint32_t tcount = 0; tcount < my_tiles; ++tcount, tile += units) {
             const int64_t m0 = SGB_H_M0_OF(tile);
@@ -474,19 +542,20 @@
             for (int t = 0; t < 4; ++t) {
                 const int c0 = (2 * t + half) * 32;
                 if (c0 < ncols && !(SGB_ABL & SGB_ABL_NO_EPI)) {
-                    float bm[4], bq[4];
+                    float bm[4], bq[4], bx[4], bnx[4];
                     const bool col_ok = c0 + cc < ncols;
                     const float* bias_p = g.bias ? g.bias + n0 + c0 + cc : nullptr;
                     if (nvalid == 32 && c0 + 32 <= ncols)
-                        h_epi_chunk<true>(g, taddr + c0, stg, crow + c0, bias_p, lane, grp, cc, nvalid, col_ok, sc1, sc2, stats, inv_nb, bm, bq);
+                        h_epi_chunk<true>(g, taddr + c0, stg, crow + c0, bias_p, lane, grp, cc, nvalid, col_ok, sc1, sc2, stats, inv_nb, bm, bq, bx, bnx);
                     else
-                        h_epi_chunk<false>(g, taddr + c0, stg, crow + c0, bias_p, lane, grp, cc, nvalid, col_ok, sc1, sc2, stats && nvalid > 0, inv_nb, bm, bq);
+                        h_epi_chunk<false>(g, taddr + c0, stg, crow + c0, bias_p, lane, grp, cc, nvalid, col_ok, sc1, sc2, stats && nvalid > 0, inv_nb, bm, bq, bx, bnx);
                     if (stats && nvalid > 0 && grp == t) {
 #pragma unroll
                         for (int q = 0; q < 4; ++q) {
                             const float delta = bm[q] - st_mean[q];
                             st_mean[q] = fmaf(delta, wgt, st_mean[q]);
                             st_m2[q] += bq[q] + delta * delta * st_n * wgt;
+                            if (g.stat_ext) { st_max[q] = fmaxf(st_max[q], bx[q]); st_nmax[q] = fmaxf(st_nmax[q], bnx[q]); }
                         }
                     }
                 }
@@ -507,6 +576,13 @@
                 st4(row + 0 * (int64_t)g.n + n0 + c0 + cc, make_float4(st_n, st_n, st_n, st_n));
                 st4(row + 1 * (int64_t)g.n + n0 + c0 + cc, make_float4(st_mean[0], st_mean[1], st_mean[2], st_mean[3]));
                 st4(row + 2 * (int64_t)g.n + n0 + c0 + cc, make_float4(st_m2[0], st_m2[1], st_m2[2], st_m2[3]));
+                if (g.stat_ext && st_n > 0.f) {
+#pragma unroll
+                    for (int q = 0; q < 4; ++q) {
+                        atomicMax(g.stat_ext + n0 + c0 + cc + q, float_order_key(st_max[q]));
+                        atomicMax(g.stat_ext + g.n + n0 + c0 + cc + q, float_order_key(st_nmax[q]));
+                    }
+                }
             }
         }
     }
@@ -553,8 +629,25 @@
     int conv_groups;
     int64_t m_per_split;
     uint32_t tmem_cols; int acc_stride;
+    AffinePrologue pro;
 };
 
+__device__ __forceinline__ void tn_load_affine(const AffinePrologue& pro, int col, int k, float4& mu, float4& sc, float4& sh) {
+    mu = sc = sh = make_float4(0.f, 0.f, 0.f, 0.f);
+    if (col < k) { mu = ldg4(pro.mean + col); sc = ldg4(pro.scale + col); sh = ldg4(pro.shift + col); }
+}
+
+__device__ __forceinline__ void tn_apply_affine(float4 (&v)[8], float4 mu, float4 sc, float4 sh, float slope, int64_t row0, int64_t m) {
+#pragma unroll
+    for (int r = 0; r < 8; ++r) v[r] = bn_lrelu4(v[r], mu, sc, sh, slope);
+    if (row0 + 8 > m) {
+#pragma unroll
+        for (int r = 0; r < 8; ++r)
+            if (row0 + r >= m) v[r] = make_float4(0.f, 0.f, 0.f, 0.f);
+    }
+}
+
+template <bool AFF>
 __global__ void __launch_bounds__(kTThreads, 1) k_gemm_tn_f16(const __grid_constant__ TArgs t) {
     extern __shared__ __align__(1024) uint8_t smem[];
     const int warp = threadIdx.x >> 5, lane = threadIdx.x & 31;
@@ -631,6 +724,8 @@
         const uint32_t tile_off = is_g ? 0u : (uint32_t)(2 * kTGTile);
         const uint32_t lo_off = is_g ? (uint32_t)kTGTile : (uint32_t)a_tile_bytes;
         const uint32_t base_off = tile_off + (uint32_t)((c4 * 4) >> 3) * kTSbo + (uint32_t)mg * kTLbo + (uint32_t)((c4 * 4) & 7) * 16;
+        float4 pmu, psc, psh;
+        if (AFF) tn_load_affine(t.pro, k0 + c4 * 4, t.k, pmu, psc, psh);
         const uint32_t ug = (uint32_t)groups, ustages = (uint32_t)t.stages;
         uint32_t s = (uint32_t)grp % ustages, ph = ((uint32_t)grp / ustages) & 1u, rs = (uint32_t)grp % raw_stages, rph = ((uint32_t)grp / raw_stages) & 1u;
         for (int it = grp; it < chunks; it += groups) {
@@ -645,6 +740,7 @@
                 float4 v[8];
 #pragma unroll
                 for (int r = 0; r < 8; ++r) v[r] = *reinterpret_cast<const float4*>(raw + (size_t)r * box * 4);
+                if (AFF && !is_g) tn_apply_affine(v, pmu, psc, psh, t.pro.slope, ms + (int64_t)it * kTBV + mg * 8, t.m);
 #pragma unroll
                 for (int q = 0; q < 4; ++q) {
                     const float x0 = (&v[0].x)[q], x1 = (&v[1].x)[q], x2 = (&v[2].x)[q], x3 = (&v[3].x)[q];
@@ -808,8 +904,10 @@
     int k_tiles; int stages; int raw_stages;
     int64_t m_per_split;
     uint32_t tmem_cols; int acc_stride;
+    AffinePrologue pro;
 };
 
+template <bool AFF>
 __global__ void __cluster_dims__(2, 1, 1) __launch_bounds__(kPThreads, 1) k_gemm_tn_f16_pair(const __grid_constant__ TPArgs t) {
     extern __shared__ __align__(1024) uint8_t smem[];
     const int warp = threadIdx.x >> 5, lane = threadIdx.x & 31;
@@ -876,6 +974,8 @@
         const uint32_t tile_off = is_g ? 0u : (uint32_t)(2 * kTGTile);
         const uint32_t lo_off = is_g ? (uint32_t)kTGTile : (uint32_t)a_tile_bytes;
         const uint32_t base_off = tile_off + (uint32_t)((c4 * 4) >> 3) * kTSbo + (uint32_t)mg * kTLbo + (uint32_t)((c4 * 4) & 7) * 16;
+        float4 pmu, psc, psh;
+        if (AFF) tn_load_affine(t.pro, ka + c4 * 4, t.k, pmu, psc, psh);
         uint32_t s = 0, ph = 0, rs = 0, rph = 0;
         for (int it = 0; it < chunks; ++it) {
             mbar_wait(&rfull[rs], rph);
@@ -888,6 +988,7 @@
                 float4 v[8];
 #pragma unroll
                 for (int r = 0; r < 8; ++r) v[r] = *reinterpret_cast<const float4*>(raw + (size_t)r * box * 4);
+                if (AFF && !is_g) tn_apply_affine(v, pmu, psc, psh, t.pro.slope, ms + (int64_t)it * kTBV + mg * 8, t.m);
 #pragma unroll
                 for (int q = 0; q < 4; ++q) {
                     const float x0 = (&v[0].x)[q], x1 = (&v[1].x)[q], x2 = (&v[2].x)[q], x3 = (&v[3].x)[q];
@@ -1033,7 +1134,7 @@
     return n % 32 == 0 && m >= 32768;
 }
 
-static HPlan h_plan(int n, int k, bool pair = false) {
+static HPlan h_plan(int n, int k, bool pair = false, bool aff = false) {
     HPlan p;
     p.pair = pair;
     p.bn = n <= 256 ? n : 256;
@@ -1042,10 +1143,11 @@
     int sb = pair ? h_stage_bytes_pair(p.bn) : h_stage_bytes(p.bn);
     p.raw_stages = 3;
     if (const char* e = getenv("SGB_F16_RAW")) { int v = atoi(e); if (v >= 2 && v <= kHMaxRawStages) p.raw_stages = v; }
-    int st = (kHSmemBudget - kHBarBytes - kHEpiBytes - p.raw_stages * kHRawBytes - 1024) / sb;
+    const int aff_bytes = aff ? 3 * p.k_chunks * kHBK * 4 : 0;
+    int st = (kHSmemBudget - kHBarBytes - kHEpiBytes - aff_bytes - p.raw_stages * kHRawBytes - 1024) / sb;
     p.stages = st > kHMaxStages ? kHMaxStages : st;
     if (const char* e = getenv("SGB_F16_STAGES")) { int v = atoi(e); if (v >= 2 && v <= p.stages) p.stages = v; }
-    p.smem_bytes = (size_t)p.raw_stages * kHRawBytes + (size_t)p.stages * sb + kHBarBytes + kHEpiBytes;
+    p.smem_bytes = (size_t)p.raw_stages * kHRawBytes + (size_t)p.stages * sb + kHBarBytes + kHEpiBytes + aff_bytes;
     p.img_bytes = (size_t)p.n_tiles * p.k_chunks * 2 * h_b_tile_bytes(p.bn);
     p.acc_stride = (p.bn + 31) / 32 * 32;
     uint32_t cols = 32;
@@ -1056,8 +1158,16 @@
 
 size_t gemm_f16_workspace(int n, int k) { return h_plan(n, k).img_bytes + 512; }
 
+bool gemm_f16_prologue_ok(int k) { return k <= kHMaxAffK; }
+
 int gemm_f16_launch(const GemmArgs& g, const float* a_amax, void* ws, size_t ws_bytes, cudaStream_t stream) {
-    HPlan p = h_plan(g.n, g.k, h_pair_wanted(g.m, g.n));
+    const bool aff = g.a_scale != nullptr;
+    if (aff && !gemm_f16_prologue_ok(g.k)) {
+        set_error("sgb_gemm: the fp16-split engine applies the BatchNorm prologue for k <= %d (k=%d)", kHMaxAffK, g.k);
+        return SGB_ENOTSUP;
+    }
+    const AffinePrologue pro{g.a_mean, g.a_scale, g.a_shift, g.slope};
+    HPlan p = h_plan(g.n, g.k, h_pair_wanted(g.m, g.n), aff);
     if (!ws || ws_bytes < p.img_bytes + 512) {
         set_error("sgb_gemm: fp16-split engine needs %zu bytes of workspace, got %zu", p.img_bytes + 512, ws_bytes);
         return SGB_ENOSPC;
@@ -1070,16 +1180,16 @@
     float* hdr = reinterpret_cast<float*>(base);
     uint8_t* img = base + 256;
     if (!a_amax) {
-        int rc = amax_launch(g.a, g.lda, g.m, g.k, reinterpret_cast<uint32_t*>(hdr + 2), stream);
+        int rc = amax_launch(g.a, g.lda, g.m, g.k, reinterpret_cast<uint32_t*>(hdr + 2), stream, pro);
         if (rc != SGB_OK) return rc;
         a_amax = hdr + 2;
     }
     k_prep_weights_f16<<<num_sms(), 256, 0, stream>>>(g.b, g.ldb, g.transb, g.n, g.k, p.bn, p.n_tiles, p.k_chunks, reinterpret_cast<__half*>(img), hdr);
     SGB_CHECK_LAUNCH("k_prep_weights_f16");
+    void (*kern)(HArgs) = p.pair ? (aff ? k_gemm_f16<true, true> : k_gemm_f16<true, false>) : (aff ? k_gemm_f16<false, true> : k_gemm_f16<false, false>);
     {
-        static std::atomic<uint64_t> optin{0}, optin_pair{0};
-        int rc = p.pair ? smem_optin(reinterpret_cast<const void*>(k_gemm_f16<true>), kHSmemBudget, &optin_pair)
-                        : smem_optin(reinterpret_cast<const void*>(k_gemm_f16<false>), kHSmemBudget, &optin);
+        static std::atomic<uint64_t> optin[4];
+        int rc = smem_optin(reinterpret_cast<const void*>(kern), kHSmemBudget, &optin[(p.pair ? 2 : 0) + (aff ? 1 : 0)]);
         if (rc != SGB_OK) return rc;
     }
     HArgs t{};
@@ -1089,7 +1199,8 @@
     }
     t.a = g.a; t.lda = g.lda; t.wp = img; t.wscale = hdr; t.a_amax = a_amax; t.c = g.c; t.ldc = g.ldc; t.m = g.m; t.n = g.n; t.k = g.k;
     t.bn = p.bn; t.n_tiles = p.n_tiles; t.k_chunks = p.k_chunks; t.stages = p.stages; t.raw_stages = p.raw_stages;
-    t.bias = g.bias; t.accumulate = g.accumulate; t.stat_partials = g.stat_partials; t.tmem_cols = p.tmem_cols; t.acc_stride = p.acc_stride;
+    t.bias = g.bias; t.accumulate = g.accumulate; t.stat_partials = g.stat_partials; t.stat_ext = g.stat_ext; t.tmem_cols = p.tmem_cols; t.acc_stride = p.acc_stride;
+    t.pro = pro;
     const int64_t m_tiles = ceil_div(g.m, kHBM);
     int groups = num_sms() / p.n_tiles;
     if (groups < 1) groups = 1;
@@ -1105,6 +1216,7 @@
         const int rows = gemm_stat_rows(g.m), written = 4 * groups;
         if (rows > written)
             SGB_CUDA(cudaMemsetAsync(g.stat_partials + (size_t)written * 3 * g.n, 0, (size_t)(rows - written) * 3 * g.n * sizeof(float), stream));
+        if (g.stat_ext) SGB_CUDA(cudaMemsetAsync(g.stat_ext, 0x80, 2 * (size_t)g.n * sizeof(int32_t), stream));
     }
     if (p.pair) {
         cudaLaunchConfig_t cfg{};
@@ -1117,9 +1229,9 @@
         attr[0].val.clusterDim.x = 2; attr[0].val.clusterDim.y = 1; attr[0].val.clusterDim.z = 1;
         cfg.attrs = attr;
         cfg.numAttrs = 1;
-        SGB_CUDA(cudaLaunchKernelEx(&cfg, k_gemm_f16<true>, t));
+        SGB_CUDA(cudaLaunchKernelEx(&cfg, kern, t));
     } else {
-        k_gemm_f16<false><<<grid, kHThreads, p.smem_bytes, stream>>>(t);
+        kern<<<grid, kHThreads, p.smem_bytes, stream>>>(t);
     }
     SGB_CHECK_LAUNCH("k_gemm_f16");
     return SGB_OK;
@@ -1166,8 +1278,9 @@
 
 size_t gemm_tn_f16_workspace(int64_t m, int n, int k) { return t_plan(m, n, k).ws_bytes; }
 
-int gemm_tn_f16_launch(const float* g, int64_t ldg, const float* a, int64_t lda, const float* g_amax, const float* a_amax, float* d,
-                       int64_t ldd, int64_t m, int n, int k, int accumulate, void* ws, size_t ws_bytes, cudaStream_t stream) {
+int gemm_tn_f16_launch(const float* g, int64_t ldg, const float* a, int64_t lda, const float* g_amax, const float* a_amax, const AffinePrologue& pro,
+                       float* d, int64_t ldd, int64_t m, int n, int k, int accumulate, void* ws, size_t ws_bytes, cudaStream_t stream) {
+    const bool aff = pro.mean != nullptr;
     TPlan p = t_plan(m, n, k);
     if (!ws || ws_bytes < p.ws_bytes) {
         set_error("sgb_gemm_tn: fp16-split engine needs %zu bytes of workspace, got %zu", p.ws_bytes, ws_bytes);
@@ -1186,13 +1299,14 @@
         g_amax = hdr + 0;
     }
     if (!a_amax) {
-        int rc = amax_launch(a, lda, m, k, reinterpret_cast<uint32_t*>(hdr + 1), stream);
+        int rc = amax_launch(a, lda, m, k, reinterpret_cast<uint32_t*>(hdr + 1), stream, pro);
         if (rc != SGB_OK) return rc;
         a_amax = hdr + 1;
     }
+    void (*kern)(TArgs) = aff ? k_gemm_tn_f16<true> : k_gemm_tn_f16<false>;
     {
-        static std::atomic<uint64_t> optin{0};
-        int rc = smem_optin(reinterpret_cast<const void*>(k_gemm_tn_f16), kHSmemBudget, &optin);
+        static std::atomic<uint64_t> optin[2];
+        int rc = smem_optin(reinterpret_cast<const void*>(kern), kHSmemBudget, &optin[aff ? 1 : 0]);
         if (rc != SGB_OK) return rc;
     }
     TArgs t{};
@@ -1204,8 +1318,9 @@
     }
     t.g = g; t.ldg = ldg; t.a = a; t.lda = lda; t.g_amax = g_amax; t.a_amax = a_amax; t.partial = partial; t.m = m; t.n = n; t.k = k;
     t.bk = p.bk; t.k_tiles = p.k_tiles; t.stages = p.stages; t.raw_stages = p.raw_stages; t.conv_groups = p.conv_groups; t.m_per_split = p.m_per_split; t.tmem_cols = p.tmem_cols; t.acc_stride = p.acc_stride;
+    t.pro = pro;
     dim3 grid((unsigned)(p.n_tiles * p.k_tiles), (unsigned)p.splits);
-    k_gemm_tn_f16<<<grid, kTThreads, p.smem_bytes, stream>>>(t);
+    kern<<<grid, kTThreads, p.smem_bytes, stream>>>(t);
     SGB_CHECK_LAUNCH("k_gemm_tn_f16");
     return reduce_splits_launch(partial, p.splits, n, k, d, ldd, accumulate, stream);
 }
@@ -1247,8 +1362,9 @@
 
 size_t gemm_tn_pair_workspace(int64_t m, int n, int k) { return gemm_tn_pair_ok(m, n, k) ? p_plan(m, n, k).ws_bytes : 0; }
 
-int gemm_tn_pair_launch(const float* g, int64_t ldg, const float* a, int64_t lda, const float* g_amax, const float* a_amax, float* d,
-                        int64_t ldd, int64_t m, int n, int k, int accumulate, void* ws, size_t ws_bytes, cudaStream_t stream) {
+int gemm_tn_pair_launch(const float* g, int64_t ldg, const float* a, int64_t lda, const float* g_amax, const float* a_amax, const AffinePrologue& pro,
+                        float* d, int64_t ldd, int64_t m, int n, int k, int accumulate, void* ws, size_t ws_bytes, cudaStream_t stream) {
+    const bool aff = pro.mean != nullptr;
     PPlan p = p_plan(m, n, k);
     if (!ws || ws_bytes < p.ws_bytes) {
         set_error("sgb_gemm_tn: pair engine needs %zu bytes of workspace, got %zu", p.ws_bytes, ws_bytes);
@@ -1267,13 +1383,14 @@
         g_amax = hdr + 0;
     }
     if (!a_amax) {
-        int rc = amax_launch(a, lda, m, k, reinterpret_cast<uint32_t*>(hdr + 1), stream);
+        int rc = amax_launch(a, lda, m, k, reinterpret_cast<uint32_t*>(hdr + 1), stream, pro);
         if (rc != SGB_OK) return rc;
         a_amax = hdr + 1;
     }
+    void (*kern)(TPArgs) = aff ? k_gemm_tn_f16_pair<true> : k_gemm_tn_f16_pair<false>;
     {
-        static std::atomic<uint64_t> optin{0};
-        int rc = smem_optin(reinterpret_cast<const void*>(k_gemm_tn_f16_pair), kHSmemBudget, &optin);
+        static std::atomic<uint64_t> optin[2];
+        int rc = smem_optin(reinterpret_cast<const void*>(kern), kHSmemBudget, &optin[aff ? 1 : 0]);
         if (rc != SGB_OK) return rc;
     }
     TPArgs t{};
@@ -1284,8 +1401,9 @@
     }
     t.ah = p.ah; t.g_amax = g_amax; t.a_amax = a_amax; t.partial = partial; t.m = m; t.n = n; t.k = k;
     t.bk = p.bk; t.k_tiles = p.k_tiles; t.stages = p.stages; t.raw_stages = p.raw_stages; t.m_per_split = p.m_per_split; t.tmem_cols = p.tmem_cols; t.acc_stride = p.acc_stride;
+    t.pro = pro;
     dim3 grid((unsigned)(2 * p.pairs), (unsigned)p.splits);
-    k_gemm_tn_f16_pair<<<grid, kPThreads, p.smem_bytes, stream>>>(t);
+    kern<<<grid, kPThreads, p.smem_bytes, stream>>>(t);
     SGB_CHECK_LAUNCH("k_gemm_tn_f16_pair");
     return reduce_splits_launch(partial, p.splits, n, k, d, ldd, accumulate, stream);
 }
diff --git a/semigcn_b200/networks.py b/semigcn_b200/networks.py
--- a/semigcn_b200/networks.py
+++ b/semigcn_b200/networks.py
@@ -59,15 +59,18 @@
                 prep.close()
         skip_in = []
         nblk = len(self.blocks)
+        defer = self.comm is None and not self.skip and ops.defer_bn_enabled()
+        n = x.shape[0]
         for i, b in enumerate(self.blocks):
+            d = defer and i + 1 < nblk and self.blocks[i + 1].takes_deferred_input(n)
             if i <= 5:
-                x = b(x, edge_index)
+                x = b(x, edge_index, defer_out=d)
                 skip_in.append(x)
             elif i <= 7:
-                x = b(x, edge_index)
+                x = b(x, edge_index, defer_out=d)
             else:
                 if self.skip:
                     lin = self.skip_blocks[nblk - i]
                     x = ops.linear(torch.cat([skip_in[nblk - i], x], dim=1), lin.weight, lin.bias)
-                x = b(x, edge_index)
+                x = b(x, edge_index, defer_out=d)
         return x_pos + x
diff --git a/semigcn_b200/nn.py b/semigcn_b200/nn.py
--- a/semigcn_b200/nn.py
+++ b/semigcn_b200/nn.py
@@ -68,7 +68,7 @@
             raise SgbError("GCNConv: edge_weight is not supported (the reference never passes one)")
         _check_inputs(x, edge_index, self.in_channels)
         g = ops.graph_for(edge_index, x.shape[0], MODE_GCN)
-        return ConvBlockFn.apply(x, g, _BlockCfg("gcn", None, 1.0), self.bias, None, None, self.lin.weight)
+        return ConvBlockFn.apply(x, g, _BlockCfg("gcn", None, 1.0), self.bias, None, None, None, None, self.lin.weight)
 
     def __repr__(self) -> str:
         return f"GCNConv({self.in_channels}, {self.out_channels})"
@@ -105,23 +105,33 @@
             raise SgbError("ChebConv: edge_weight / batch / lambda_max are not supported (lambda_max is 2.0 for 'sym')")
         _check_inputs(x, edge_index, self.in_channels)
         g = ops.graph_for(edge_index, x.shape[0], MODE_CHEB)
-        return ConvBlockFn.apply(x, g, _BlockCfg("cheb", None, 1.0), self.bias, None, None, *[l.weight for l in self.lins])
+        return ConvBlockFn.apply(x, g, _BlockCfg("cheb", None, 1.0), self.bias, None, None, None, None, *[l.weight for l in self.lins])
 
     def __repr__(self) -> str:
         return f"ChebConv({self.in_channels}, {self.out_channels}, K={len(self.lins)}, normalization={self.normalization})"
 
 
 class _BlockCfg:
-    def __init__(self, kind: str, bn: Optional[nn.BatchNorm1d], slope: float, x_amax: Optional[Tensor] = None):
+    def __init__(self, kind: str, bn: Optional[nn.BatchNorm1d], slope: float, x_amax: Optional[Tensor] = None,
+                 defer_out: bool = False, x_src: Optional["_BlockCfg"] = None):
         self.kind, self.bn, self.slope = kind, bn, slope
         self.x_amax = x_amax
         self.out_amax = None
+        self.defer_out, self.x_src = defer_out, x_src
+        self.out_affine: Optional[Tuple[Tensor, Tensor, Tensor, Tensor]] = None
+        self.dy_amax: Optional[Tensor] = None
+
+
+class DeferredBnAct:
+
+    def __init__(self, y: Tensor, cfg: _BlockCfg, bn: nn.BatchNorm1d):
+        self.y, self.cfg, self.bn = y, cfg, bn
 
 
 class ConvBlockFn(torch.autograd.Function):
 
     @staticmethod
-    def forward(ctx, x, graph, cfg, bias, gamma, beta, *weights):
+    def forward(ctx, x, graph, cfg, bias, gamma, beta, x_gamma, x_beta, *weights):
         x = ops._f32c(x, "x")
         bn = cfg.bn
         training = bn is not None and (bn.training or bn.running_mean is None)
@@ -129,22 +139,36 @@
         saved_ops: List[Tensor] = []
         am = ops.new_amax(x.device, 4)
         x_amax = cfg.x_amax
+        x_aff = None
+        if cfg.x_src is not None:
+            mean_p, _, scale_p, shift_p = cfg.x_src.out_affine
+            x_aff = (mean_p, scale_p, shift_p, cfg.x_src.slope)
+            x_amax = cfg.x_src.out_amax
+        ctx.x_aff = x_aff
+        ext = None
         if cfg.kind == "gcn":
             (w,) = weights
             cout, cin = w.shape
             agg_first = cin <= cout
+            if x_aff is not None and agg_first:
+                raise SgbError("ConvBlockFn: a deferred input needs a transform-first GCN block")
             if agg_first:
                 p = ops.spmm(graph, x, amax_out=am[0:1])
-                r = ops.gemm(p, w, transb=True, bias=bias, want_stats=want_stats, a_amax=am[0:1])
+                if (cfg.defer_out and want_stats and graph.comm is None and cfg.slope >= 0.0
+                        and ops.gemm_on_f16_engine(p.shape[0], cout, cin)):
+                    ext = torch.empty((2, cout), dtype=torch.int32, device=x.device)
+                r = ops.gemm(p, w, transb=True, bias=bias, want_stats=want_stats, a_amax=am[0:1], extremes_out=ext)
                 saved_ops = [p]
                 ctx.op_amax = [am[0:1]]
             else:
-                h = ops.gemm(x, w, transb=True, a_amax=x_amax)
+                h = ops.gemm(x, w, transb=True, a_affine=x_aff, a_amax=x_amax)
                 r = ops.spmm(graph, h, bias=bias, want_stats=want_stats)
                 saved_ops = [x]
                 ctx.op_amax = [x_amax]
             ctx.agg_first = agg_first
         else:
+            if x_aff is not None:
+                raise SgbError("ConvBlockFn: a deferred input needs a transform-first GCN block")
             nw = len(weights)
             cin = x.shape[1]
             tcat = None
@@ -164,6 +188,7 @@
         y, partials = r if want_stats else (r, None)
 
         ctx.graph, ctx.cfg, ctx.nw, ctx.has_bias = graph, cfg, len(weights), bias is not None
+        ctx.deferred = False
         if bn is None:
             ctx.bn_mode = 0
             ctx.save_for_backward(*weights, *saved_ops)
@@ -176,10 +201,19 @@
                     momentum = 1.0 / float(bn.num_batches_tracked)
             rm = bn.running_mean if bn.track_running_stats else None
             rv = bn.running_var if bn.track_running_stats else None
+            defer = ext is not None
             mean, invstd, scale, shift = ops.bn_finalize(partials, graph.n_global, gamma, beta, bn.eps, momentum, rm, rv,
-                                                         comm=graph.comm)
+                                                         comm=graph.comm, extremes=ext, slope=cfg.slope,
+                                                         amax_out=am[2:3] if defer else None)
+            if defer:
+                cfg.out_affine = (mean, invstd, scale, shift)
+                cfg.out_amax = am[2:3]
+                ctx.bn_mode, ctx.deferred, ctx.has_affine = 2, True, gamma is not None
+                ctx.save_for_backward(*weights, *saved_ops)
+                return y
         else:
             mean, invstd, scale, shift = ops.eval_affine(bn.running_mean, bn.running_var, gamma, beta, bn.eps)
+        cfg.defer_out = False
         z = ops.bn_act_apply(y, mean, scale, shift, cfg.slope, amax_out=am[3:4])
         cfg.out_amax = am[3:4]
         ctx.bn_mode = 2 if training else 1
@@ -192,13 +226,15 @@
         cfg, graph, nw = ctx.cfg, ctx.graph, ctx.nw
         saved = ctx.saved_tensors
         weights = saved[:nw]
-        dgamma = dbeta = None
+        dgamma = dbeta = dxg = dxb = None
         dz = dz.contiguous()
-        am = ops.new_amax(dz.device, 2)
+        am = ops.new_amax(dz.device, 3)
         dy_amax = None
-        if ctx.bn_mode == 0:
+        if ctx.bn_mode == 0 or ctx.deferred:
             saved_ops = saved[nw:]
             dy = dz
+            if ctx.deferred:
+                dy_amax = cfg.dy_amax
         else:
             saved_ops = saved[nw:-5]
             y, scale, shift, mean, invstd = saved[-5:]
@@ -236,9 +272,15 @@
             else:
                 (x,) = saved_ops
                 dh = ops.spmm(graph, dy, transpose=True, amax_out=am[1:2])
-                dws[0] = ops.gemm_tn(dh, x, g_amax=am[1:2], a_amax=ctx.op_amax[0])
+                dws[0] = ops.gemm_tn(dh, x, g_amax=am[1:2], a_amax=ctx.op_amax[0], a_affine=ctx.x_aff)
                 if need_x:
                     dx = ops.gemm(dh, w, transb=False, a_amax=am[1:2])
+                    if ctx.x_aff is not None:
+                        src = cfg.x_src
+                        mean_p, invstd_p, scale_p, shift_p = src.out_affine
+                        src.dy_amax = am[2:3]
+                        dx, dxg, dxb = ops.bn_act_bwd(dx, x, scale_p, shift_p, mean_p, invstd_p, src.slope, True,
+                                                      amax_out=src.dy_amax)
         else:
             x = saved_ops[0]
             cin = x.shape[1]
@@ -263,7 +305,8 @@
                         d = ops.spmm(graph, gs[k + 1], transpose=True, alpha=2.0 if k >= 1 else 1.0, addend=d, beta=1.0)
                     gs[k] = d
                 dx = gs[0]
-        return (dx, None, None, db, dgamma, dbeta, *dws)
+        return (dx, None, None, db, dgamma, dbeta, dxg if ctx.needs_input_grad[6] else None,
+                dxb if ctx.needs_input_grad[7] else None, *dws)
 
 
 class _SparseHashModule(nn.Module):
@@ -362,7 +405,13 @@
                 return 3, 0.0
         return 2, 1.0
 
-    def forward(self, *args):
+    def takes_deferred_input(self, m: int) -> bool:
+        conv = self[0]
+        return (isinstance(conv, GCNConv) and self._fusable(0) is not None and self._descs[0][0][0] == self._in_names[0]
+                and conv.in_channels > conv.out_channels
+                and ops.bn_prologue_on_tensor_cores(m, conv.in_channels, conv.out_channels))
+
+    def forward(self, *args, defer_out: bool = False):
         env = dict(zip(self._in_names, args))
         out = None
         i = 0
@@ -374,16 +423,26 @@
                 consumed, slope = fuse
                 x, edge_index = env[ins[0]], env[ins[1]]
                 bn = self[i + 1]
+                src = None
+                if isinstance(x, DeferredBnAct):
+                    if not (i == 0 and self.takes_deferred_input(x.y.shape[0])):
+                        raise SgbError("Sequential: a deferred BatchNorm output reached a block that cannot apply it")
+                    src, x = x, x.y
                 _check_inputs(x, edge_index, mod.in_channels)
+                defer = defer_out and i + consumed == len(self)
                 if isinstance(mod, GCNConv):
                     g = ops.graph_for(edge_index, x.shape[0], MODE_GCN)
-                    cfg = _BlockCfg("gcn", bn, slope, ops.amax_of(x))
-                    out = ConvBlockFn.apply(x, g, cfg, mod.bias, bn.weight, bn.bias, mod.lin.weight)
+                    cfg = _BlockCfg("gcn", bn, slope, ops.amax_of(x) if src is None else None, defer_out=defer,
+                                    x_src=src.cfg if src is not None else None)
+                    out = ConvBlockFn.apply(x, g, cfg, mod.bias, bn.weight, bn.bias, src.bn.weight if src is not None else None,
+                                            src.bn.bias if src is not None else None, mod.lin.weight)
                 else:
                     g = ops.graph_for(edge_index, x.shape[0], MODE_CHEB)
-                    cfg = _BlockCfg("cheb", bn, slope, ops.amax_of(x))
-                    out = ConvBlockFn.apply(x, g, cfg, mod.bias, bn.weight, bn.bias, *[l.weight for l in mod.lins])
-                if cfg.out_amax is not None:
+                    cfg = _BlockCfg("cheb", bn, slope, ops.amax_of(x), defer_out=defer)
+                    out = ConvBlockFn.apply(x, g, cfg, mod.bias, bn.weight, bn.bias, None, None, *[l.weight for l in mod.lins])
+                if cfg.defer_out:
+                    out = DeferredBnAct(out, cfg, bn)
+                elif cfg.out_amax is not None:
                     ops.tag_amax(out, cfg.out_amax)
                 env[outs[0]] = out
                 i += consumed
diff --git a/semigcn_b200/ops.py b/semigcn_b200/ops.py
--- a/semigcn_b200/ops.py
+++ b/semigcn_b200/ops.py
@@ -202,7 +202,7 @@
 
 def gemm(a: Tensor, b: Tensor, transb: bool = True, a_affine: Affine = None, bias: Optional[Tensor] = None,
          out: Optional[Tensor] = None, accumulate: bool = False, want_stats: bool = False, engine: int = 0,
-         a_amax: Optional[Tensor] = None):
+         a_amax: Optional[Tensor] = None, extremes_out: Optional[Tensor] = None):
     lib = L.load()
     require_cuda(a, b, bias)
     a, b = _f32c(a, "a"), _f32c(b, "b")
@@ -222,7 +222,7 @@
     with torch.cuda.device(a.device):
         check(lib.sgb_gemm(1 if transb else 0, ptr(a), a.stride(0), ptr(b), b.stride(0), ptr(c), c.stride(0), m, n, k,
                            ptr(mu), ptr(sc), ptr(sh), float(slope), ptr(bias), 1 if accumulate else 0, ptr(partials),
-                           ptr(a_amax), ptr(ws), wsb, engine, stream_ptr(a.device)), "sgb_gemm")
+                           ptr(extremes_out), ptr(a_amax), ptr(ws), wsb, engine, stream_ptr(a.device)), "sgb_gemm")
     if sp is not None:
         sp.close()
     L.count(1)
@@ -230,7 +230,7 @@
 
 
 def gemm_tn(gmat: Tensor, a: Tensor, out: Optional[Tensor] = None, accumulate: bool = False, engine: int = 0,
-            g_amax: Optional[Tensor] = None, a_amax: Optional[Tensor] = None) -> Tensor:
+            g_amax: Optional[Tensor] = None, a_amax: Optional[Tensor] = None, a_affine: Affine = None) -> Tensor:
     lib = L.load()
     require_cuda(gmat, a)
     gmat, a = _f32c(gmat, "g"), _f32c(a, "a")
@@ -239,12 +239,14 @@
     if a.shape[0] != m:
         raise SgbError("gemm_tn: row counts differ")
     d = out if out is not None else torch.empty((n, k), dtype=torch.float32, device=a.device)
+    mu, sc, sh, slope = (a_affine if a_affine is not None else (None, None, None, 0.0))
     wsb = lib.sgb_gemm_tn_workspace_bytes(m, n, k)
     ws = _ws(wsb, a.device)
     sp = _prof.span(f"gemm_tn_n{n}_k{k}", 4.0 * (m * (k + n) + k * n), 2.0 * m * n * k) if _prof.ACTIVE is not None else None
     with torch.cuda.device(a.device):
         check(lib.sgb_gemm_tn(ptr(gmat), gmat.stride(0), ptr(a), a.stride(0), ptr(d), d.stride(0), m, n, k,
-                              1 if accumulate else 0, ptr(g_amax), ptr(a_amax), ptr(ws), wsb, engine, stream_ptr(a.device)), "sgb_gemm_tn")
+                              1 if accumulate else 0, ptr(g_amax), ptr(a_amax), ptr(mu), ptr(sc), ptr(sh), float(slope), ptr(ws), wsb,
+                              engine, stream_ptr(a.device)), "sgb_gemm_tn")
     if sp is not None:
         sp.close()
     L.count(2)
@@ -271,6 +273,18 @@
 
 def tensor_core_likely(m: int, cin: int, cout: int) -> bool:
     return m >= 2048 and ((cin >= 32 and cout >= 16) or (cout >= 32 and cin >= 16))
+
+
+def defer_bn_enabled() -> bool:
+    return os.environ.get("SGB_DEFER_BN", "1") != "0"
+
+
+def gemm_on_f16_engine(m: int, n: int, k: int) -> bool:
+    return m >= 2048 and n >= 32 and k >= 16 and n % 16 == 0 and k % 4 == 0
+
+
+def bn_prologue_on_tensor_cores(m: int, cin: int, cout: int) -> bool:
+    return m >= 4096 and cout >= 32 and 16 <= cin <= 512 and cout % 16 == 0 and cin % 4 == 0
 
 
 def amax(x: Tensor) -> Optional[Tensor]:
@@ -356,7 +370,8 @@
 
 
 def bn_finalize(partials: Tensor, count: int, gamma: Optional[Tensor], beta: Optional[Tensor], eps: float,
-                momentum: float, running_mean: Optional[Tensor], running_var: Optional[Tensor], comm=None):
+                momentum: float, running_mean: Optional[Tensor], running_var: Optional[Tensor], comm=None,
+                extremes: Optional[Tensor] = None, slope: float = 0.0, amax_out: Optional[Tensor] = None):
     lib = L.load()
     if comm is not None:
         partials = comm.all_gather_cat(merge_moment_rows(partials).contiguous())
@@ -367,7 +382,7 @@
     with torch.cuda.device(dev):
         check(lib.sgb_bn_finalize(ptr(partials), rows, c, count, ptr(gamma), ptr(beta), float(eps), float(momentum),
                                   ptr(running_mean), ptr(running_var), ptr(st[0]), ptr(st[1]), ptr(st[2]), ptr(st[3]),
-                                  stream_ptr(dev)), "sgb_bn_finalize")
+                                  ptr(extremes), float(slope), ptr(amax_out), stream_ptr(dev)), "sgb_bn_finalize")
     if sp is not None:
         sp.close()
     L.count(1)
```
